# xaskasdf/ntransformer

Measured on AMD Instinct MI355X. Metric: decode tokens/sec (Llama-3.1-8B Q8_0 class, resident weights, greedy, batch 1), higher is better.
Workload: dtype f32; 1 GPU; Llama-3.1-8B-shaped Q8_0 GGUF tensors (seed 20260925), resident in HBM, 16-token prompt, greedy decode; ctx=4096, replicas=1, hipgraph=True

## Files before the change

include/ntk_engine.h:

```cpp
#ifndef NTK_ENGINE_H
#define NTK_ENGINE_H

#include "ntk.h"

#if defined(__GNUC__)
#pragma GCC visibility push(default)
#endif
#ifdef __cplusplus
extern "C" {
#endif

int ntk_rope_kv_store(float* q, const float* k, const float* v, const int* positions, int seq_len, int n_heads, int n_kv_heads, int head_dim,
                      float theta_base, float freq_scale, int interleaved, void* k_cache, void* v_cache, int start_pos, int max_seq, void* stream);
int ntk_rope_tab(float* q, float* k, const int* positions, int batch_size, int seq_len, int n_heads, int n_kv_heads, int head_dim, float theta_base,
                 float freq_scale, int interleaved, const float* inv_freq, void* stream);
int ntk_rope_kv_store_tab(float* q, const float* k, const float* v, const int* positions, int seq_len, int n_heads, int n_kv_heads, int head_dim,
                          float theta_base, float freq_scale, int interleaved, void* k_cache, void* v_cache, int start_pos, int max_seq,
                          const float* inv_freq, void* stream);
typedef struct ntk_gemv_seg {
    const void* W;
    float*      y;
    int         rows;
    int         dtype;
} ntk_gemv_seg;

int ntk_gemv_fused(const ntk_gemv_seg* segs, int nseg, const float* x, int in_features, const float* norm_w,
                   float eps, const float* resid, int silu_pair, void* stream);

size_t ntk_q8l_bytes(int rows, int in_features);
int ntk_q8l_pack(void* dst, const void* raw, int rows, int in_features, void* stream);
int ntk_q8l_unpack(void* raw, const void* packed, int rows, int in_features, void* stream);

size_t ntk_rp_bytes(int dtype, int rows, int in_features);
int ntk_rp_pack(void* dst, const void* raw, int rows, int in_features, int dtype, void* stream);
int ntk_rp_dequant(float* out, const void* rp, int rows, int in_features, int dtype, void* stream);
int ntk_rp_unpack(void* raw, const void* rp, int rows, int in_features, int dtype, void* stream);
int ntk_gemv_rp(float* y, const void* rp, const float* x, int out_features, int in_features, int weight_dtype, void* stream);
int ntk_gemv_rp_fused(const ntk_gemv_seg* segs, int nseg, const float* x, int in_features, const float* norm_w, float eps,
                      const float* resid, int silu_pair, void* stream);
#define NTK_ARENA_HIDDEN 1
#define NTK_ARENA_ATTN_OUT 2
#define NTK_ARENA_GATE 3
#define NTK_ARENA_HIDDEN_FLOATS 8192
#define NTK_ARENA_ATTN_FLOATS 8192
#define NTK_ARENA_GATE_FLOATS 32768
int ntk_decode_arena_acquire(void);
void ntk_decode_arena_release(int device);
float* ntk_decode_arena_slot(int slot);
int ntk_debug_gemv_static_x(void);

int ntk_debug_rp_prologue(uint8_t* out, const float* x, const float* norm_w, float eps, int in_features, int nsub, int nwaves, void* stream);
int ntk_debug_mfma_i8_probe(int* D, const int8_t* A, const int8_t* B, void* stream);

int ntk_attention_decode_fused(float* output, const float* q, const float* k, const float* v, void* k_cache,
                               void* v_cache, const int* d_pos, const float* inv_freq, int n_heads, int n_kv_heads,
                               int head_dim, int max_seq, float scale, float theta_base, float freq_scale,
                               void* stream);

size_t ntk_attention_split_scratch_bytes(int n_heads, int head_dim, int nsplit);
int ntk_attention_decode_split(float* output, const float* q, const float* k, const float* v, void* k_cache,
                               void* v_cache, const int* d_pos, const float* inv_freq, int n_heads, int n_kv_heads,
                               int head_dim, int max_seq, float scale, float theta_base, float freq_scale, int nsplit,
                               float* scratch, void* stream);
int ntk_attention_split_scratch_init(float* scratch, int n_heads, void* stream);
int ntk_attention_decode_split_merged(float* output, const float* q, const float* k, const float* v, void* k_cache,
                                      void* v_cache, const int* d_pos, const float* inv_freq, int n_heads, int n_kv_heads,
                                      int head_dim, int max_seq, float scale, float theta_base, float freq_scale, int nsplit,
                                      float* scratch, void* stream);

#define NTK_ATTN_BATCH_MAX 16
typedef struct ntk_kv_batch {
    void* k[NTK_ATTN_BATCH_MAX];
    void* v[NTK_ATTN_BATCH_MAX];
} ntk_kv_batch;
int ntk_attention_decode_batch(float* output, const float* q, const float* k, const float* v, const ntk_kv_batch* caches, const int* positions,
                               int n_rows, const float* inv_freq, int n_heads, int n_kv_heads, int head_dim, int max_seq, float scale,
                               float theta_base, float freq_scale, int nsplit, float* scratch, void* stream);

typedef struct ntk_kv_segments {
    int   n_seg;
    int   row0[NTK_ATTN_BATCH_MAX];
    int   n_rows[NTK_ATTN_BATCH_MAX];
    int   start_pos[NTK_ATTN_BATCH_MAX];
    void* k[NTK_ATTN_BATCH_MAX];
    void* v[NTK_ATTN_BATCH_MAX];
} ntk_kv_segments;
int ntk_kv_segments_validate(const ntk_kv_segments* segs, int total_rows, int max_seq);
int ntk_rope_kv_store_segments(float* q, const float* k, const float* v, const ntk_kv_segments* segs, int n_heads, int n_kv_heads, int head_dim,
                               float theta_base, float freq_scale, int interleaved, int max_seq, void* stream);
int ntk_rope_kv_store_segments_tab(float* q, const float* k, const float* v, const ntk_kv_segments* segs, int n_heads, int n_kv_heads, int head_dim,
                                   float theta_base, float freq_scale, int interleaved, int max_seq, const float* inv_freq, void* stream);
int ntk_attention_prefill_segments(float* output, const float* Q, const ntk_kv_segments* segs, int n_heads, int n_kv_heads, int head_dim, int max_seq,
                                   float scale, void* stream);

size_t ntk_kv_q8_cache_bytes(int max_seq, int n_kv_heads, int head_dim);
int ntk_kv_store_q8(void* k_cache, void* v_cache, const float* k, const float* v, int seq_len, int n_kv_heads, int head_dim, int start_pos,
                    int max_seq, void* stream);
int ntk_rope_kv_store_q8(float* q, const float* k, const float* v, const int* positions, int seq_len, int n_heads, int n_kv_heads, int head_dim,
                         float theta_base, float freq_scale, int interleaved, void* k_cache, void* v_cache, int start_pos, int max_seq,
                         void* stream);
int ntk_rope_kv_store_q8_tab(float* q, const float* k, const float* v, const int* positions, int seq_len, int n_heads, int n_kv_heads, int head_dim,
                             float theta_base, float freq_scale, int interleaved, void* k_cache, void* v_cache, int start_pos, int max_seq,
                             const float* inv_freq, void* stream);
int ntk_attention_decode_q8(float* output, const float* q, const float* k, const float* v, void* k_cache, void* v_cache, const int* d_pos,
                            const float* inv_freq, int n_heads, int n_kv_heads, int head_dim, int max_seq, float scale, float theta_base,
                            float freq_scale, int nsplit, float* scratch, void* stream);
int ntk_kv_dequant_q8_f16(void* k_f16, void* v_f16, const void* k_cache, const void* v_cache, int n_rows, int n_kv_heads, int head_dim,
                          int max_seq, void* stream);
int ntk_attention_decode_q8_batch(float* output, const float* q, const float* k, const float* v, const ntk_kv_batch* caches, const int* positions,
                                  int n_rows, const float* inv_freq, int n_heads, int n_kv_heads, int head_dim, int max_seq, float scale,
                                  float theta_base, float freq_scale, int nsplit, float* scratch, void* stream);

int ntk_kv_shift(uint16_t* k_cache, uint16_t* v_cache, int n_layers, int max_seq, int n_kv_heads, int head_dim, int src0, int dst0, int n_rows,
                 const float* inv_freq, float theta_base, float freq_scale, int interleaved, void* stream);
int ntk_kv_shift_q8(void* k_cache_q8, void* v_cache_q8, int n_layers, int max_seq, int n_kv_heads, int head_dim, int src0, int dst0, int n_rows,
                    const float* inv_freq, float theta_base, float freq_scale, int interleaved, void* stream);

int ntk_debug_gemv_fused_form(const ntk_gemv_seg* segs, int nseg, const float* x, int in_features, const float* norm_w, float eps,
                              const float* resid, int silu_pair, int integer_activations, void* stream);

size_t   ntk_tp_comm_bytes(size_t max_floats);
void*    ntk_tp_comm_alloc(size_t bytes);
int      ntk_tp_comm_reset(void* comm, void* stream);
float*   ntk_tp_slot(void* comm, size_t max_floats, unsigned call_index);
int      ntk_tp_allreduce_add(float* hidden, void* const* peers, int rank, int world, size_t max_floats, unsigned call_index, int n, void* stream);
int      ntk_tp_advance_epoch(void* comm, void* stream);
unsigned ntk_tp_error(void* comm);
int      ntk_ipc_export(void* devptr, void* handle64);
int      ntk_ipc_open(const void* handle64, void** devptr);
int      ntk_ipc_close(void* devptr);

int ntk_gemm_quant(float* Y, const void* W, const float* X, int n_tokens, int out_features, int in_features,
                   int weight_dtype, const float* resid, void* stream);

typedef struct ntk_gemm_partials {
    const float* part[3];
    float*       y[3];
    int          rows[3];
    int          nseg, n_tokens, nsplit;
} ntk_gemm_partials;
typedef struct ntk_gemm_desc {
    const ntk_gemv_seg* segs;
    int                 nseg;
    const float*        X;
    int                 n_tokens, in_features;
    const float*        resid;
    void*               workspace;
    size_t              workspace_bytes;
    int                 reuse_x;
    const float*        row_max;
    ntk_gemm_partials*  partials;
    int                 weights_repacked;
    int                 full_form;
} ntk_gemm_desc;
size_t ntk_gemm_quant_workspace_bytes(int in_features, int out_features);
int ntk_gemm_quant_f16(const ntk_gemm_desc* desc, void* stream);
int ntk_reduce_rmsnorm_rowmax(float* hidden, const ntk_gemm_partials* partials, const float* weight, float eps, float* x_out, float* row_max,
                              float* zero_tokens, void* stream);
int ntk_reduce_silu_mul_rowmax(float* output, const ntk_gemm_partials* partials, float* row_max, void* stream);
int ntk_rmsnorm_rowmax(float* output, const float* input, const float* weight, int n_tokens, int hidden_size, float eps, float* row_max,
                       float* zero_tokens, void* stream);
int ntk_silu_mul_rowmax(float* output, const float* gate, const float* up, int n_tokens, int width, float* row_max, void* stream);
int ntk_gemm_prepare_x(const float* X, int n_tokens, int in_features, void* workspace, void* stream);
int ntk_rmsnorm_prepare_x(float* output, const float* input, const float* weight, int n_tokens, int hidden_size, float eps, void* workspace, void* stream);
int ntk_reduce_rmsnorm_prepare_x(float* hidden, const ntk_gemm_partials* partials, const float* weight, float eps, float* x_out, void* workspace, void* stream);
int ntk_silu_mul_prepare_x(float* output, const float* gate, const float* up, int n_tokens, int width, void* workspace, void* stream);
int ntk_reduce_silu_mul_prepare_x(float* output, const ntk_gemm_partials* partials, void* workspace, void* stream);

size_t ntk_gemm_dense16_workspace_bytes(int in_features, int out_features, int dtype);
int ntk_gemm_dense16(const ntk_gemm_desc* desc, void* stream);

int ntk_embed_rows(float* out, const void* table, const int* tokens, int n_tokens, int hidden, int dtype,
                   void* stream);

int ntk_argmax(const float* logits, int n, int* d_out_token, int* h_mirror, float* scratch, void* stream);

int ntk_logprob_rows(const float* logits, int n_rows, int vocab, int ld, const int* targets, float* logprob, int* top1, void* stream);

size_t ntk_sample_scratch_bytes(int n);
int ntk_sample_top_k(float* logits, int n, const int* d_recent, int n_recent, float repeat_penalty, float temperature,
                     int top_k, float top_p, float r, int* d_out_token, int* h_mirror, void* scratch, void* stream);
int ntk_repeat_penalty(float* logits, int n, const int* d_recent, int n_recent, float repeat_penalty, void* stream);

#define NTK_SAMPLE_ROWS_MAX 16
typedef struct ntk_sample_rows {
    float temperature[NTK_SAMPLE_ROWS_MAX], top_p[NTK_SAMPLE_ROWS_MAX], repeat_penalty[NTK_SAMPLE_ROWS_MAX], r[NTK_SAMPLE_ROWS_MAX];
    int   top_k[NTK_SAMPLE_ROWS_MAX], n_recent[NTK_SAMPLE_ROWS_MAX];
} ntk_sample_rows;
size_t ntk_sample_rows_scratch_bytes(int n_rows, int vocab);
int ntk_sample_rows_top_k(float* logits, int n_rows, int vocab, int ld, const int* d_recent, int recent_ld, const ntk_sample_rows* rows, int* d_out,
                          int* h_mirror, void* scratch, void* stream);

int ntk_argmax_advance(const float* logits, int n, int* d_out_token, int* h_mirror, unsigned long long* h_ring4, int* d_pos,
                       float* scratch, void* stream);

int ntk_debug_sclk(unsigned long long* d_out2, void* stream);
int ntk_debug_sclk_begin(unsigned* d_flag, unsigned long long* d_out2, void* side_stream);
int ntk_debug_sclk_end(unsigned* d_flag, void* other_stream);

void ntk_debug_malloc_budget(long long bytes);

int ntk_advance_pos(int* d_pos, void* stream);

int ntk_qkv_bias(float* q, float* k, float* v, const float* bq, const float* bk, const float* bv, int n_rows, int q_dim, int kv_dim, void* stream);

int ntk_qk_norm(float* q, float* k, const float* wq, const float* wk, int n_rows, int n_heads, int n_kv_heads, int head_dim, float eps, void* stream);

#ifdef __cplusplus
}
#endif
#if defined(__GNUC__)
#pragma GCC visibility pop
#endif
#endif
```

ntransformer_amd/_lib.py:

```python
from __future__ import annotations

import ctypes as C
import os

_HERE = os.path.dirname(os.path.abspath(__file__))
LIB_PATH = os.environ.get("NTK_LIB_PATH") or os.path.join(_HERE, "libntransformer_hip.so")

NTK_OK = 0
_STATUS = {0: "ok", -1: "unsupported dtype", -2: "bad shape", -3: "HIP launch/runtime error", -4: "misaligned pointer",
           -5: "null pointer", -6: "no usable GPU", -7: "out of memory", -8: "I/O error", -9: "malformed GGUF"}


class NtkError(RuntimeError):
    def __init__(self, status: int, what: str = ""):
        self.status = status
        super().__init__("ntk status %d (%s)%s" % (status, _STATUS.get(status, "?"), (": " + what) if what else ""))


def check(status: int, what: str = "") -> None:
    if status != NTK_OK:
        raise NtkError(status, what)


class KvBatch(C.Structure):
    _fields_ = [("k", C.c_void_p * 16), ("v", C.c_void_p * 16)]


class KvSegments(C.Structure):
    _fields_ = [("n_seg", C.c_int), ("row0", C.c_int * 16), ("n_rows", C.c_int * 16), ("start_pos", C.c_int * 16), ("k", C.c_void_p * 16),
                ("v", C.c_void_p * 16)]


class SampleRows(C.Structure):
    _fields_ = [("temperature", C.c_float * 16), ("top_p", C.c_float * 16), ("repeat_penalty", C.c_float * 16), ("r", C.c_float * 16),
                ("top_k", C.c_int * 16), ("n_recent", C.c_int * 16)]


class GemvSeg(C.Structure):
    _fields_ = [("W", C.c_void_p), ("y", C.c_void_p), ("rows", C.c_int), ("dtype", C.c_int)]


class GemmPartials(C.Structure):
    _fields_ = [("part", C.c_void_p * 3), ("y", C.c_void_p * 3), ("rows", C.c_int * 3), ("nseg", C.c_int), ("n_tokens", C.c_int), ("nsplit", C.c_int)]


class GemmDesc(C.Structure):
    _fields_ = [("segs", C.POINTER(GemvSeg)), ("nseg", C.c_int), ("X", C.c_void_p), ("n_tokens", C.c_int), ("in_features", C.c_int), ("resid", C.c_void_p),
                ("workspace", C.c_void_p), ("workspace_bytes", C.c_size_t), ("reuse_x", C.c_int), ("row_max", C.c_void_p),
                ("partials", C.POINTER(GemmPartials)), ("weights_repacked", C.c_int), ("full_form", C.c_int)]


_lib = None


def lib() -> C.CDLL:
    global _lib
    if _lib is not None:
        return _lib
    if not os.path.exists(LIB_PATH):
        raise ImportError("%s is missing: run `python -c 'import __graft_entry__ as g; g.build()'` "
                          "(hipcc --offload-arch=gfx950); there is no CPU fallback" % LIB_PATH)
    L = C.CDLL(LIB_PATH, mode=C.RTLD_GLOBAL)
    vp, i, f, sz = C.c_void_p, C.c_int, C.c_float, C.c_size_t
    sig = {
        "ntk_abi_version": (i, []),
        "ntk_status_string": (C.c_char_p, [i]),
        "ntk_row_bytes": (sz, [i, C.c_int64]),
        "ntk_device_count": (i, []),
        "ntk_device_init": (i, [i]),
        "ntk_device_name": (i, [C.c_char_p, sz]),
        "ntk_device_mem_info": (i, [C.POINTER(sz), C.POINTER(sz)]),
        "ntk_stream": (vp, [i]),
        "ntk_stream_synchronize": (i, [vp]),
        "ntk_device_synchronize": (i, []),
        "ntk_event_create": (vp, []),
        "ntk_event_destroy": (i, [vp]),
        "ntk_event_record": (i, [vp, vp]),
        "ntk_event_synchronize": (i, [vp]),
        "ntk_event_elapsed_ms": (i, [vp, vp, C.POINTER(f)]),
        "nt_hip_malloc": (vp, [sz]), "nt_hip_free": (None, [vp]),
        "nt_hip_memcpy_h2d": (None, [vp, vp, sz]), "nt_hip_memcpy_d2h": (None, [vp, vp, sz]),
        "nt_hip_memcpy_d2d": (None, [vp, vp, sz]), "nt_hip_memset": (None, [vp, i, sz]),
        "nt_hip_malloc_host": (vp, [sz]), "nt_hip_free_host": (None, [vp]),
        "ntk_memcpy_h2d_async": (i, [vp, vp, sz, vp]), "ntk_memcpy_d2h_async": (i, [vp, vp, sz, vp]),
        "nt_cuda_malloc": (vp, [sz]), "nt_cuda_free": (None, [vp]),
        "nt_cuda_memcpy_h2d": (None, [vp, vp, sz]), "nt_cuda_memcpy_d2h": (None, [vp, vp, sz]),
        "nt_cuda_memcpy_d2d": (None, [vp, vp, sz]), "nt_cuda_memset": (None, [vp, i, sz]),
        "nt_cuda_malloc_host": (vp, [sz]), "nt_cuda_free_host": (None, [vp]),
        "ntk_rmsnorm": (i, [vp, vp, vp, i, i, f, vp]),
        "ntk_rmsnorm_f16": (i, [vp, vp, vp, i, i, f, vp]),
        "ntk_rope": (i, [vp, vp, vp, i, i, i, i, i, f, f, i, vp]),
        "ntk_softmax": (i, [vp, vp, i, i, vp]),
        "ntk_masked_softmax": (i, [vp, vp, vp, i, i, vp]),
        "ntk_gemv": (i, [vp, vp, vp, i, i, i, vp]),
        "ntk_gemv_add": (i, [vp, vp, vp, i, i, i, vp]),
        "ntk_gemm_f32": (i, [vp, vp, vp, i, i, i, vp]),
        "ntk_silu_mul": (i, [vp, vp, vp, i, vp]),
        "ntk_rmsnorm_rowmax": (i, [vp, vp, vp, i, i, f, vp, vp, vp]),
        "ntk_rope_kv_store": (i, [vp, vp, vp, vp, i, i, i, i, f, f, i, vp, vp, i, i, vp]),
        "ntk_silu_mul_rowmax": (i, [vp, vp, vp, i, i, vp, vp]),
        "ntk_add_bias": (i, [vp, vp, i, vp]),
        "ntk_attention_decode": (i, [vp, vp, vp, vp, i, i, i, i, i, f, vp]),
        "ntk_attention_prefill": (i, [vp, vp, vp, vp, i, i, i, i, i, i, f, vp]),
        "ntk_copy_to_kv_cache": (i, [vp, vp, vp, vp, i, i, i, i, i, vp]),
        "ntk_add": (i, [vp, vp, vp, i, vp]),
        "ntk_add_inplace": (i, [vp, vp, i, vp]),
        "ntk_copy": (i, [vp, vp, i, vp]),
        "ntk_cosine_similarity": (i, [vp, vp, vp, i, vp]),
        "ntk_gemv_fused": (i, [C.POINTER(GemvSeg), i, vp, i, vp, f, vp, i, vp]),
        "ntk_debug_gemv_fused_form": (i, [C.POINTER(GemvSeg), i, vp, i, vp, f, vp, i, i, vp]),
        "ntk_q8l_bytes": (sz, [i, i]),
        "ntk_q8l_pack": (i, [vp, vp, i, i, vp]),
        "ntk_q8l_unpack": (i, [vp, vp, i, i, vp]),
        "ntk_rp_bytes": (sz, [i, i, i]),
        "ntk_rp_pack": (i, [vp, vp, i, i, i, vp]),
        "ntk_rp_dequant": (i, [vp, vp, i, i, i, vp]),
        "ntk_rp_unpack": (i, [vp, vp, i, i, i, vp]),
        "ntk_gemv_rp": (i, [vp, vp, vp, i, i, i, vp]),
        "ntk_gemv_rp_fused": (i, [C.POINTER(GemvSeg), i, vp, i, vp, f, vp, i, vp]),
        "ntk_decode_arena_acquire": (i, []), "ntk_decode_arena_release": (None, [i]),
        "ntk_decode_arena_slot": (vp, [i]), "ntk_debug_gemv_static_x": (i, []),
        "ntk_debug_rp_prologue": (i, [vp, vp, vp, f, i, i, i, vp]),
        "ntk_debug_mfma_i8_probe": (i, [vp, vp, vp, vp]),
        "ntk_gemm_quant": (i, [vp, vp, vp, i, i, i, i, vp, vp]),
        "ntk_gemm_dense16_workspace_bytes": (sz, [i, i, i]),
        "ntk_gemm_dense16": (i, [C.POINTER(GemmDesc), vp]),
        "ntk_attention_decode_split": (i, [vp, vp, vp, vp, vp, vp, vp, vp, i, i, i, i, f, f, f, i, vp, vp]),
        "ntk_attention_split_scratch_bytes": (C.c_size_t, [i, i, i]),
        "ntk_attention_split_scratch_init": (i, [vp, i, vp]),
        "ntk_attention_decode_split_merged": (i, [vp, vp, vp, vp, vp, vp, vp, vp, i, i, i, i, f, f, f, i, vp, vp]),
        "ntk_attention_decode_fused": (i, [vp, vp, vp, vp, vp, vp, vp, vp, i, i, i, i, f, f, f, vp]),
        "ntk_attention_decode_batch": (i, [vp, vp, vp, vp, vp, vp, i, vp, i, i, i, i, f, f, f, i, vp, vp]),
        "ntk_kv_segments_validate": (i, [vp, i, i]),
        "ntk_rope_kv_store_segments": (i, [vp, vp, vp, vp, i, i, i, f, f, i, i, vp]),
        "ntk_attention_prefill_segments": (i, [vp, vp, vp, i, i, i, i, f, vp]),
        "ntk_rope_tab": (i, [vp, vp, vp, i, i, i, i, i, f, f, i, vp, vp]),
        "ntk_rope_kv_store_tab": (i, [vp, vp, vp, vp, i, i, i, i, f, f, i, vp, vp, i, i, vp, vp]),
        "ntk_rope_kv_store_segments_tab": (i, [vp, vp, vp, vp, i, i, i, f, f, i, i, vp, vp]),
        "ntk_rope_kv_store_q8_tab": (i, [vp, vp, vp, vp, i, i, i, i, f, f, i, vp, vp, i, i, vp, vp]),
        "ntk_kv_q8_cache_bytes": (C.c_size_t, [i, i, i]),
        "ntk_kv_store_q8": (i, [vp, vp, vp, vp, i, i, i, i, i, vp]),
        "ntk_rope_kv_store_q8": (i, [vp, vp, vp, vp, i, i, i, i, f, f, i, vp, vp, i, i, vp]),
        "ntk_attention_decode_q8": (i, [vp, vp, vp, vp, vp, vp, vp, vp, i, i, i, i, f, f, f, i, vp, vp]),
        "ntk_kv_dequant_q8_f16": (i, [vp, vp, vp, vp, i, i, i, i, vp]),
        "ntk_attention_decode_q8_batch": (i, [vp, vp, vp, vp, vp, vp, i, vp, i, i, i, i, f, f, f, i, vp, vp]),
        "ntk_kv_shift": (i, [vp, vp, i, i, i, i, i, i, i, vp, f, f, i, vp]),
        "ntk_kv_shift_q8": (i, [vp, vp, i, i, i, i, i, i, i, vp, f, f, i, vp]),
        "ntk_embed_rows": (i, [vp, vp, vp, i, i, i, vp]),
        "ntk_argmax": (i, [vp, i, vp, vp, vp, vp]),
        "ntk_logprob_rows": (i, [vp, i, i, i, vp, vp, vp, vp]),
        "ntk_sample_rows_scratch_bytes": (C.c_size_t, [i, i]),
        "ntk_sample_rows_top_k": (i, [vp, i, i, i, vp, i, C.POINTER(SampleRows), vp, vp, vp, vp]),
        "ntk_advance_pos": (i, [vp, vp]),
        "ntk_qkv_bias": (i, [vp, vp, vp, vp, vp, vp, i, i, i, vp]),
        "ntk_qk_norm": (i, [vp, vp, vp, vp, i, i, i, i, f, vp]),
        "ntk_debug_sclk": (i, [vp, vp]),
        "ntk_debug_sclk_begin": (i, [vp, vp, vp]),
        "ntk_debug_sclk_end": (i, [vp, vp]),
    }
    for name, (res, args) in sig.items():
        fn = getattr(L, name)
        fn.restype = res
        fn.argtypes = args
    _lib = L
    return L


EXPORTS_NTK_H = None
```

ntransformer_amd/csrc/common.hip.h:

```cpp
#pragma once
#include <hip/hip_runtime.h>
#include <stdint.h>
#include "../../include/ntk_engine.h"

#define NTK_WAVE 64

#define NTK_HIP_TRY(expr)                                   \
    do {                                                    \
        hipError_t e__ = (expr);                            \
        if (e__ != hipSuccess) return NTK_E_LAUNCH;         \
    } while (0)

#define NTK_EXTRA_API extern "C" __attribute__((visibility("default")))
#ifdef NTK_TUNE
#include <cstdlib>
#define NTK_TUNE_ENV_INT(name, dflt) ([] { const char* e__ = getenv(name); return e__ ? atoi(e__) : (dflt); }())
#else
#define NTK_TUNE_ENV_INT(name, dflt) (dflt)
#endif

namespace ntk {

hipStream_t resolve_stream(void* s);
int         last_launch_status();
int         q8l_gemv_fused(const ntk_gemv_seg* segs, int nseg, const float* x, int in, const float* norm_w, float eps, const float* resid,
                           int silu_pair, hipStream_t st);
int         dense16_gemv_fused(const ntk_gemv_seg* segs, int nseg, const float* x, int in, const float* norm_w, float eps, const float* resid,
                               int silu_pair, hipStream_t st);

__device__ __forceinline__ float h2f(uint16_t bits) {
    _Float16 h;
    __builtin_memcpy(&h, &bits, 2);
    return (float)h;
}
__device__ __forceinline__ uint16_t f2h(float f) {
    _Float16 h = (_Float16)f;
    uint16_t bits;
    __builtin_memcpy(&bits, &h, 2);
    return bits;
}

__device__ __forceinline__ void rope_rotate(const float a, const float b, const float c, const float s, float& ra, float& rb) {
#pragma clang fp contract(off)
    ra = a * c - b * s;
    rb = b * c + a * s;
}

__device__ __forceinline__ float rope_freq(const float* __restrict__ inv_freq, const int i, const int head_dim, const float theta) {
    return inv_freq ? inv_freq[i] : 1.0f / (float)pow((double)theta, (double)((2.0f * i) / head_dim));
}

template <int CTRL, int ROW_MASK>
__device__ __forceinline__ float dpp_or_zero(float v) {
    return __int_as_float(__builtin_amdgcn_update_dpp(0, __float_as_int(v), CTRL, ROW_MASK, 0xF, false));
}
template <int CTRL, int ROW_MASK>
__device__ __forceinline__ float dpp_or_self(float v) {
    return __int_as_float(__builtin_amdgcn_update_dpp(__float_as_int(v), __float_as_int(v), CTRL, ROW_MASK, 0xF, false));
}
constexpr int DPP_QUAD_1032 = 0xB1, DPP_QUAD_2301 = 0x4E, DPP_ROW_HALF_MIRROR = 0x141, DPP_ROW_MIRROR = 0x140,
              DPP_ROW_BCAST15 = 0x142, DPP_ROW_BCAST31 = 0x143;

__device__ __forceinline__ float wave_sum_lane63(float v) {
    v += dpp_or_zero<DPP_QUAD_1032, 0xF>(v);
    v += dpp_or_zero<DPP_QUAD_2301, 0xF>(v);
    v += dpp_or_zero<DPP_ROW_HALF_MIRROR, 0xF>(v);
    v += dpp_or_zero<DPP_ROW_MIRROR, 0xF>(v);
    v += dpp_or_zero<DPP_ROW_BCAST15, 0xA>(v);
    v += dpp_or_zero<DPP_ROW_BCAST31, 0xC>(v);
    return v;
}
__device__ __forceinline__ float wave_sum(float v) {
    return __int_as_float(__builtin_amdgcn_readlane(__float_as_int(wave_sum_lane63(v)), 63));
}
__device__ __forceinline__ float wave_max(float v) {
    v = fmaxf(v, dpp_or_self<DPP_QUAD_1032, 0xF>(v));
    v = fmaxf(v, dpp_or_self<DPP_QUAD_2301, 0xF>(v));
    v = fmaxf(v, dpp_or_self<DPP_ROW_HALF_MIRROR, 0xF>(v));
    v = fmaxf(v, dpp_or_self<DPP_ROW_MIRROR, 0xF>(v));
    v = fmaxf(v, dpp_or_self<DPP_ROW_BCAST15, 0xA>(v));
    v = fmaxf(v, dpp_or_self<DPP_ROW_BCAST31, 0xC>(v));
    return __int_as_float(__builtin_amdgcn_readlane(__float_as_int(v), 63));
}

template <int N>
__device__ __forceinline__ float group_sum(float v) {
    static_assert(N == 1 || N == 2 || N == 4 || N == 8 || N == 16 || N == 32, "group size");
    if constexpr (N >= 2) v += dpp_or_zero<DPP_QUAD_1032, 0xF>(v);
    if constexpr (N >= 4) v += dpp_or_zero<DPP_QUAD_2301, 0xF>(v);
    if constexpr (N >= 8) v += dpp_or_zero<DPP_ROW_HALF_MIRROR, 0xF>(v);
    if constexpr (N >= 16) v += dpp_or_zero<DPP_ROW_MIRROR, 0xF>(v);
    if constexpr (N >= 32) v += __shfl_xor(v, 16, 64);
    return v;
}

__device__ __forceinline__ float block_sum(float v, float* red) {
    const int lane = threadIdx.x & 63, wave = threadIdx.x >> 6, nw = (blockDim.x + 63) >> 6;
    v = wave_sum(v);
    __syncthreads();
    if (lane == 0) red[wave] = v;
    __syncthreads();
    float t = 0.0f;
    for (int i = 0; i < nw; ++i) t += red[i];
    return t;
}
__device__ __forceinline__ float block_max(float v, float* red) {
    const int lane = threadIdx.x & 63, wave = threadIdx.x >> 6, nw = (blockDim.x + 63) >> 6;
    v = wave_max(v);
    __syncthreads();
    if (lane == 0) red[wave] = v;
    __syncthreads();
    float t = red[0];
    for (int i = 1; i < nw; ++i) t = fmaxf(t, red[i]);
    return t;
}

template <int N>
__device__ __forceinline__ void lds_read_dwords(uint32_t (&dst)[N], const uint8_t* base, int off) {
    const int a = off & ~3;
    const uint32_t sh = (uint32_t)(off & 3);
    uint32_t w[N + 1];
#pragma unroll
    for (int i = 0; i <= N; ++i) w[i] = *reinterpret_cast<const uint32_t*>(base + a + 4 * i);
#pragma unroll
    for (int i = 0; i < N; ++i) dst[i] = __builtin_amdgcn_alignbyte(w[i + 1], w[i], sh);
}
__device__ __forceinline__ uint16_t lds_u16_at(const uint8_t* base, int off) {
    return *reinterpret_cast<const uint16_t*>(base + off);
}

__device__ __forceinline__ float ub2f(uint32_t w, int k) { return (float)((w >> (8 * k)) & 0xFFu); }
__device__ __forceinline__ float sb2f(uint32_t w, int k) { return (float)(int)(int8_t)(w >> (8 * k)); }

__device__ __forceinline__ void kq_scale_min(uint32_t s0, uint32_t s1, uint32_t s2, int j, float& sc, float& mn) {
    const uint64_t lo = (uint64_t)s0 | ((uint64_t)s1 << 32);
    auto byte = [&](int n) -> uint32_t {
        return n < 8 ? (uint32_t)((lo >> (8 * n)) & 0xFFu) : ((s2 >> (8 * (n - 8))) & 0xFFu);
    };
    uint32_t s, m;
    if (j < 4) {
        s = byte(j) & 63u;
        m = byte(j + 4) & 63u;
    } else {
        s = (byte(j + 4) & 0xFu) | ((byte(j - 4) >> 6) << 4);
        m = (byte(j + 4) >> 4) | ((byte(j) >> 6) << 4);
    }
    sc = (float)s;
    mn = (float)m;
}

}
```

ntransformer_amd/csrc/gemv.hip:

```cpp
#include "gemv_core.hip.h"
#include <algorithm>
#include <atomic>
#include <cmath>
#include <cstddef>
#include <mutex>
#include <cstdio>
#include <cstdlib>

namespace ntk {

enum { NS_ANY = 0, NS_ONE = 1, NS_SPLIT = 2 };

enum { XS_NONE = 0, XS_HIDDEN = NTK_ARENA_HIDDEN, XS_ATTN = NTK_ARENA_ATTN_OUT, XS_GATE = NTK_ARENA_GATE };
struct DecodeArena {
    float hidden[NTK_ARENA_HIDDEN_FLOATS];
    float attn_out[NTK_ARENA_ATTN_FLOATS];
    float gate[NTK_ARENA_GATE_FLOATS];
};
__device__ __attribute__((aligned(256))) DecodeArena g_decode_arena;
template <int XS> struct XSlot { static constexpr int IN = XS == XS_GATE ? 14336 : 4096; };
template <int XS> __device__ __forceinline__ const float* xslot_ptr() {
    return XS == XS_HIDDEN ? g_decode_arena.hidden : XS == XS_ATTN ? g_decode_arena.attn_out : g_decode_arena.gate;
}

template <int DT, bool NORM, bool XFAST, bool A16, bool XI = false, bool LM = false, int NSF = NS_ANY, int XS = XS_NONE>
__device__ __forceinline__ void gemv_quant_body(const GemvParams& p, const int bid, const int nblk) {
    using F = Fmt<DT>;
    static_assert(!LM || (DT == NTK_DT_Q8_0 && !A16 && !XI), "lane-major rows: Q8_0");
    static_assert(NSF == NS_ANY || LM, "compile-time slice forms: the lane-major kernels");
    static_assert(XS == XS_NONE || (LM && XFAST && NSF != NS_ANY), "early-x forms: the lane-major kernels, fast prologue");
    constexpr int NL = LM ? 4 : F::NL;
    constexpr int STAGE = LM ? 0 : NL * 1024 + 64;
    extern __shared__ __attribute__((aligned(16))) uint8_t smem[];
#ifdef NTK_GEMV_TRACE
    unsigned long long gv_t[GT_EV] = {0, 0, 0, 0, 0, 0, 0, 0, 0, 0, 0, 0, 0, 0};
#endif
    GV_STAMP(0);
#ifndef NTK_GEMV_NO_KARG_PREFETCH
    const auto* ka = __builtin_amdgcn_kernarg_segment_ptr();
    unsigned d0, d1, d2, d3, d4;
    if constexpr (XS == XS_NONE) {
        asm volatile("s_load_dword %0, %5, 0x0\n\ts_load_dword %1, %5, 0x40\n\ts_load_dword %2, %5, 0x80\n\ts_load_dword %3, %5, 0xc0\n\t"
                     "s_load_dword %4, %5, 0x100\n\ts_waitcnt lgkmcnt(0)"
                     : "=&s"(d0), "=&s"(d1), "=&s"(d2), "=&s"(d3), "=&s"(d4) : "s"(ka) : "memory");
    } else {
        asm volatile("s_load_dword %0, %5, 0x0\n\ts_load_dword %1, %5, 0x40\n\ts_load_dword %2, %5, 0x80\n\ts_load_dword %3, %5, 0xc0\n\t"
                     "s_load_dword %4, %5, 0x100"
                     : "=&s"(d0), "=&s"(d1), "=&s"(d2), "=&s"(d3), "=&s"(d4) : "s"(ka) : "memory");
    }
    __builtin_amdgcn_sched_barrier(0);
#endif

    const int tid = threadIdx.x;
    constexpr int XIT = 8, WIT = 4;
    u32x4 xv[XIT], wv[WIT];
    if constexpr (XS != XS_NONE) {
        constexpr int IN = XSlot<XS>::IN, step0 = 512 * 4;
        const float* const xs = xslot_ptr<XS>();
#pragma unroll
        for (int i = 0; i < XIT; ++i) {
            xv[i] = u32x4{0u, 0u, 0u, 0u};
            if (i * step0 < IN) xv[i] = *reinterpret_cast<const u32x4*>(xs + min(tid * 4 + i * step0, IN - 4));
        }
        GV_STAMP(7);
        __builtin_amdgcn_sched_barrier(0);
#ifndef NTK_GEMV_NO_KARG_PREFETCH
        asm volatile("s_waitcnt lgkmcnt(0)" : "+s"(d0), "+s"(d1), "+s"(d2), "+s"(d3), "+s"(d4) : : "memory");
        __builtin_amdgcn_sched_barrier(0);
#endif
        if constexpr (NORM) {
#pragma unroll
            for (int i = 0; i < WIT; ++i) {
                wv[i] = u32x4{0u, 0u, 0u, 0u};
                if (i * step0 < IN) wv[i] = *reinterpret_cast<const u32x4*>(p.norm_w + min(tid * 4 + i * step0, IN - 4));
            }
        }
    } else
    if constexpr (XFAST) {
        const int step0 = (int)blockDim.x * 4;
#pragma unroll
        for (int i = 0; i < XIT; ++i) {
            xv[i] = u32x4{0u, 0u, 0u, 0u};
            if (i * step0 < p.in) xv[i] = *reinterpret_cast<const u32x4*>(p.x + min(tid * 4 + i * step0, p.in - 4));
        }
        if constexpr (NORM) {
#pragma unroll
            for (int i = 0; i < WIT; ++i) {
                wv[i] = u32x4{0u, 0u, 0u, 0u};
                if (i * step0 < p.in) wv[i] = *reinterpret_cast<const u32x4*>(p.norm_w + min(tid * 4 + i * step0, p.in - 4));
            }
        }
        GV_STAMP(7);
    }
    const int lane = tid & 63;
    const int wave = __builtin_amdgcn_readfirstlane(tid >> 6);
    const int ns = NSF == NS_ONE ? 1 : p.ns;
    const bool single = NSF == NS_ANY ? p.ns == 1 : NSF == NS_ONE;
    const int nwaves = ns * p.rw;
    const int s = wave % ns;
    const int g = wave / ns;
    constexpr bool norm = NORM;

    const size_t image_bytes = (size_t)std::min(ns, 4) * 64 * XPITCH * 4;
    const size_t stage0 = single ? image_bytes : 0;
    const size_t regionA = single ? image_bytes + (size_t)nwaves * STAGE : std::max((size_t)nwaves * STAGE, image_bytes);
    float* part = reinterpret_cast<float*>(smem + regionA);
    float* red = part + 2 * p.rw * ns * RB;
    const size_t lds_floats_total = regionA / 4 + (size_t)(2 * p.rw * ns * RB + 16 + 16);

    uint8_t* stage = smem + stage0 + (size_t)wave * STAGE;
    const int my_len = min(p.slice_cols, p.in - s * p.slice_cols);
    const int ncols = min(64, max(0, my_len - 64 * lane));
    const unsigned slice_byte0 = (unsigned)((size_t)s * p.slice_cols / F::BW * F::BB);
    const unsigned slice_bytes = (unsigned)(my_len / F::BW * F::BB);
    const int group = bid * p.rw + g;
    const int ngroups = nblk * p.rw;
    const int mats = p.silu_pair ? 2 : 1;
    const int n_my = (p.total_rows > group) ? ((p.total_rows - 1 - group) / ngroups + 1) * mats : 0;

    static_assert(MAX_SEG == 3, "locate / seg_y: unrolled for three segments");
    const int seg_rows0 = p.seg[0].rows, seg_rows1 = p.seg[1].rows;
    float* const seg_y0 = p.seg[0].y;
    float* const seg_y1 = p.seg[1].y;
    float* const seg_y2 = p.seg[2].y;
    auto locate = [&](int q, int& seg, int& row) {
        int r = group + (q >> (mats - 1)) * ngroups;
        if (p.silu_pair) { seg = q & 1; row = r; return; }
        seg = 0;
        if (p.nseg > 1 && r >= seg_rows0) {
            r -= seg_rows0; seg = 1;
            if (p.nseg > 2 && r >= seg_rows1) { r -= seg_rows1; seg = 2; }
        }
        row = r;
    };
    auto seg_y = [&](int seg) { return seg == 0 ? seg_y0 : seg == 1 ? seg_y1 : seg_y2; };
    int cu_seg = 0, cu_row = group, cu_rows = p.silu_pair ? 0x7fffffff : p.seg[0].rows;
    auto cursor_normalise = [&]() {
        while (cu_seg + 1 < p.nseg && cu_row >= cu_rows) { cu_row -= cu_rows; ++cu_seg; cu_rows = p.seg[cu_seg].rows; }
    };
    if (!p.silu_pair) cursor_normalise();
    auto cursor_advance = [&]() {
        if (p.silu_pair) {
            if (cu_seg == 0) { cu_seg = 1; } else { cu_seg = 0; cu_row += ngroups; }
        } else {
            cu_row += ngroups;
            cursor_normalise();
        }
    };

    u32x4 pf[NL], pf2[LM ? NL : 1];
    uint32_t pf_sc = 0u, pf2_sc = 0u;
    const int lm_nl = my_len >> 6, lm_lane = min(lane, max(lm_nl - 1, 0));
    unsigned pre_off[NL];
    if constexpr (A16) {
        const unsigned last0 = (slice_bytes - 1u) & ~15u;
#pragma unroll
        for (int j = 0; j < NL; ++j) pre_off[j] = min(16u * (unsigned)(lane + 64 * j), last0);
    }
    int pf_seg = 0, pf_row = 0, pf_shift = 0;
    float pf_res = 0.0f;
    auto issue = [&]() {
        pf_seg = cu_seg; pf_row = cu_row;
        if (p.resid != nullptr && single) {
            int idx = cu_row;
            asm volatile("" : "+v"(idx));
            pf_res = p.resid[idx];
        }
        if constexpr (LM) return;
        const unsigned rel = (unsigned)p.seg[cu_seg].delta + (unsigned)cu_row * p.row_bytes + slice_byte0;
        pf_shift = (int)(rel & 15u);
        const unsigned nbytes = (rel & 15u) + slice_bytes;
        const unsigned last = (nbytes - 1u) & ~15u;
        const uint8_t* a = p.seg[cu_seg].W + (rel & ~15u);
#pragma unroll
        for (int j = 0; j < NL; ++j) {
            unsigned off;
            if constexpr (A16) off = pre_off[j]; else off = min(16u * (unsigned)(lane + 64 * j), last);
            pf[j] = __builtin_nontemporal_load(reinterpret_cast<const u32x4*>(a + off));
        }
    };
    auto issue_lm = [&](u32x4 (&c)[NL], uint32_t& sc) {
        const uint8_t* a = p.seg[cu_seg].W + ((unsigned)cu_row * p.row_bytes + slice_byte0);
#pragma unroll
        for (int j = 0; j < NL; ++j)
            c[j] = __builtin_nontemporal_load(reinterpret_cast<const u32x4*>(a + 16u * (unsigned)(j * lm_nl + lm_lane)));
        sc = __builtin_nontemporal_load(reinterpret_cast<const uint32_t*>(a + 64u * (unsigned)lm_nl + 4u * (unsigned)lm_lane));
    };
    auto issue_first = [&]() { issue(); if constexpr (LM) issue_lm(pf, pf_sc); };
    if (n_my <= 0) { cu_seg = 0; cu_row = 0; }

    f32x2 x2[32];
    XInt xi;
    static_assert(!XI || (XFAST && ((DT == NTK_DT_Q4_K && A16) || DT == NTK_DT_Q6_K)), "integer activations: fast prologue, Q4_K (aligned rows) / Q6_K");
    {
        float* ximg = reinterpret_cast<float*>(smem);
        constexpr int GS = 4;
        auto img_index = [&](int c, int g0) {
            if (single) return (c >> 6) * XPITCH + (c & 63);
            const int sp = c / p.slice_cols, cc = c - sp * p.slice_cols;
            return ((sp - g0) * 64 + (cc >> 6)) * XPITCH + (cc & 63);
        };
        const int step = (int)blockDim.x * 4;
        const int dummy = (int)(lds_floats_total - 16);
        const bool have_lo = ncols > 0, have_hi = ncols > 32;
        auto read_own_row = [&](int g0) {
            const float* xrow = ximg + ((s - g0) * 64 + lane) * XPITCH;
            const float* xr0 = xrow, *xr1 = xrow + 32;
            if constexpr (DT == NTK_DT_Q6_K) {
                xr0 = ximg + ((s - g0) * 64 + (lane & ~1)) * XPITCH + 32 * (lane & 1);
                xr1 = xr0 + XPITCH;
            }
#pragma unroll
            for (int j = 0; j < 64; j += 4) {
                const float4 v = *reinterpret_cast<const float4*>((j < 32 ? xr0 : xr1 - 32) + j);
                const bool have = j < 32 ? have_lo : have_hi;
                x2[j / 2] = f32x2{have ? v.x : 0.0f, have ? v.y : 0.0f};
                x2[j / 2 + 1] = f32x2{have ? v.z : 0.0f, have ? v.w : 0.0f};
            }
        };
        if constexpr (XFAST) {
#ifndef NTK_GEMV_NO_XWAIT
            asm volatile("" : "+v"(xv[0]), "+v"(xv[1]), "+v"(xv[2]), "+v"(xv[3]), "+v"(xv[4]), "+v"(xv[5]), "+v"(xv[6]), "+v"(xv[7]));
            if constexpr (NORM) asm volatile("" : "+v"(wv[0]), "+v"(wv[1]), "+v"(wv[2]), "+v"(wv[3]));
#endif
            issue_first();
            GV_STAMP(8);
            __builtin_amdgcn_sched_barrier(0);
            GV_STAMP(1);
            float rms_inv = 1.0f;
            if constexpr (NORM) {
                float ssq = 0.0f;
#pragma unroll
                for (int i = 0; i < WIT; ++i) {
                    const float m = (tid * 4 + i * step < p.in) ? 1.0f : 0.0f;
                    const float x0 = __uint_as_float(xv[i].x), x1 = __uint_as_float(xv[i].y), x2_ = __uint_as_float(xv[i].z), x3 = __uint_as_float(xv[i].w);
                    ssq = fmaf(x0 * m, x0, ssq); ssq = fmaf(x1 * m, x1, ssq); ssq = fmaf(x2_ * m, x2_, ssq); ssq = fmaf(x3 * m, x3, ssq);
                }
                ssq = wave_sum(ssq);
                if (lane == 0) red[wave] = ssq;
                __syncthreads();
                float tot = 0.0f;
                for (int w = 0; w < nwaves; ++w) tot += red[w];
                rms_inv = 1.0f / sqrtf(tot / (float)p.in + p.eps);
#pragma unroll
                for (int i = 0; i < WIT; ++i) {
                    xv[i].x = __float_as_uint(__uint_as_float(xv[i].x) * rms_inv * __uint_as_float(wv[i].x));
                    xv[i].y = __float_as_uint(__uint_as_float(xv[i].y) * rms_inv * __uint_as_float(wv[i].y));
                    xv[i].z = __float_as_uint(__uint_as_float(xv[i].z) * rms_inv * __uint_as_float(wv[i].z));
                    xv[i].w = __float_as_uint(__uint_as_float(xv[i].w) * rms_inv * __uint_as_float(wv[i].w));
                }
            }
            if constexpr (XI) {
                uint8_t* dimg = smem;
                auto xi_store = [&](const u32x4 q, const int sp, const int cc, const bool live) {
                    const float v0 = live ? __uint_as_float(q.x) : 0.0f, v1 = live ? __uint_as_float(q.y) : 0.0f,
                                v2 = live ? __uint_as_float(q.z) : 0.0f, v3 = live ? __uint_as_float(q.w) : 0.0f;
                    float am = fmaxf(fmaxf(fabsf(v0), fabsf(v1)), fmaxf(fabsf(v2), fabsf(v3)));
                    am = fmaxf(am, dpp_or_self<DPP_QUAD_1032, 0xF>(am));
                    am = fmaxf(am, dpp_or_self<DPP_QUAD_2301, 0xF>(am));
                    am = fmaxf(am, dpp_or_self<DPP_ROW_HALF_MIRROR, 0xF>(am));
                    float sm = (v0 + v1) + (v2 + v3);
                    sm += dpp_or_zero<DPP_QUAD_1032, 0xF>(sm);
                    sm += dpp_or_zero<DPP_QUAD_2301, 0xF>(sm);
                    const int e = am > 0.0f ? __builtin_amdgcn_frexp_expf(am) : 0;
                    const float up = __builtin_ldexpf(1.0f, 22 - e), inv = __builtin_ldexpf(1.0f, e - 22);
                    const uint32_t x0 = __float_as_uint(fmaf(v0, up, 12582912.0f)) - 0x4B400000u, x1 = __float_as_uint(fmaf(v1, up, 12582912.0f)) - 0x4B400000u,
                                   x2i = __float_as_uint(fmaf(v2, up, 12582912.0f)) - 0x4B400000u, x3 = __float_as_uint(fmaf(v3, up, 12582912.0f)) - 0x4B400000u;
                    const uint32_t ta = __builtin_amdgcn_perm(x1, x0, 0x05010400u);
                    const uint32_t tb = __builtin_amdgcn_perm(x1, x0, 0x07030602u);
                    const uint32_t tc = __builtin_amdgcn_perm(x3, x2i, 0x05010400u);
                    const uint32_t td = __builtin_amdgcn_perm(x3, x2i, 0x07030602u);
                    const uint32_t p0 = __builtin_amdgcn_perm(tc, ta, 0x05040100u);
                    const uint32_t p1 = __builtin_amdgcn_perm(tc, ta, 0x07060302u);
                    const uint32_t p2 = __builtin_amdgcn_perm(td, tb, 0x05040100u);
                    if (live) {
                        uint8_t* row = dimg + (size_t)(sp * 64 + (cc >> 6)) * (XPITCH * 4);
                        *reinterpret_cast<uint32_t*>(row + (cc & 63)) = p0;
                        *reinterpret_cast<uint32_t*>(row + 64 + (cc & 63)) = p1;
                        *reinterpret_cast<uint32_t*>(row + 128 + (cc & 63)) = p2;
                        float* meta = reinterpret_cast<float*>(row + 192);
                        if ((cc & 31) == 0) meta[(cc >> 5) & 1] = inv;
                        if ((cc & 15) == 0) meta[2 + ((cc >> 4) & 3)] = sm;
                    }
                };
                auto xi_read = [&](const int g0) {
                    const bool have_lo_ = ncols > 0, have_hi_ = ncols > 32;
                    const uint8_t* rowA = dimg + (size_t)((s - g0) * 64 + lane) * (XPITCH * 4);
                    const uint8_t* rowB = rowA;
                    int offA = 0, offB = 32;
                    if constexpr (DT == NTK_DT_Q6_K) {
                        rowA = dimg + (size_t)((s - g0) * 64 + (lane & ~1)) * (XPITCH * 4);
                        rowB = rowA + XPITCH * 4;
                        offA = offB = 32 * (lane & 1);
                    }
#pragma unroll
                    for (int pl = 0; pl < 3; ++pl)
#pragma unroll
                        for (int k4 = 0; k4 < 4; ++k4) {
                            const uint8_t* src = (k4 < 2 ? rowA + offA : rowB + offB) + 64 * pl + 16 * (k4 & 1);
                            const u32x4 v = *reinterpret_cast<const u32x4*>(src);
                            const bool have = k4 < 2 ? have_lo_ : have_hi_;
                            xi.d[pl][4 * k4] = have ? v.x : 0u; xi.d[pl][4 * k4 + 1] = have ? v.y : 0u;
                            xi.d[pl][4 * k4 + 2] = have ? v.z : 0u; xi.d[pl][4 * k4 + 3] = have ? v.w : 0u;
                        }
                    const float* mA = reinterpret_cast<const float*>(rowA + 192);
                    const float* mB = reinterpret_cast<const float*>(rowB + 192);
                    xi.inv[0] = have_lo_ ? mA[offA >> 5] : 0.0f;
                    xi.inv[1] = have_hi_ ? mB[offB >> 5] : 0.0f;
                    xi.sx[0] = have_lo_ ? mA[2 + (offA >> 4)] : 0.0f; xi.sx[1] = have_lo_ ? mA[3 + (offA >> 4)] : 0.0f;
                    xi.sx[2] = have_hi_ ? mB[2 + (offB >> 4)] : 0.0f; xi.sx[3] = have_hi_ ? mB[3 + (offB >> 4)] : 0.0f;
                };
                int isp = 0, icc = tid * 4;
#pragma unroll
                for (int i = 0; i < XIT; ++i) {
                    if (i * step >= p.in) continue;
                    xi_store(xv[i], isp, icc, tid * 4 + i * step < p.in);
                    icc += step;
                    if (icc >= p.slice_cols) { icc -= p.slice_cols; ++isp; }
                }
                __syncthreads();
                xi_read(0);
            } else
            {
                const int cend = min(p.in, GS * p.slice_cols);
                int isp = 0, icc = tid * 4;
#pragma unroll
                for (int i = 0; i < XIT; ++i) {
                    if (i * step >= cend) continue;
                    const int c = tid * 4 + i * step;
                    *reinterpret_cast<u32x4*>(ximg + (c < cend ? (isp * 64 + (icc >> 6)) * XPITCH + (icc & 63) : dummy)) = xv[i];
                    icc += step;
                    if (icc >= p.slice_cols) { icc -= p.slice_cols; ++isp; }
                }
                for (int c = XIT * step + tid * 4; c < cend; c += step)
                    *reinterpret_cast<float4*>(ximg + img_index(c, 0)) = *reinterpret_cast<const float4*>(p.x + c);
                GV_STAMP(9);
                __syncthreads();
                GV_STAMP(10);
                if (s < GS) read_own_row(0);
#ifdef NTK_GEMV_TRACE
                asm volatile("s_waitcnt lgkmcnt(0)" ::: "memory");
                GV_STAMP(11);
#endif
            }
            if constexpr (!XI)
            for (int g0 = GS; g0 < ns; g0 += GS) {
                const int cbeg = g0 * p.slice_cols, cend = min(p.in, (g0 + GS) * p.slice_cols);
                __syncthreads();
                for (int c = cbeg + tid * 4; c < cend; c += step)
                    *reinterpret_cast<float4*>(ximg + img_index(c, g0)) = *reinterpret_cast<const float4*>(p.x + c);
                __syncthreads();
                if (s >= g0 && s < g0 + GS) read_own_row(g0);
            }
        } else {
            issue_first();
            float rms_inv = 1.0f;
            if (NORM && !(kAblate & 1)) {
                float ssq = 0.0f;
                for (int c = tid; c < p.in; c += blockDim.x) ssq = fmaf(p.x[c], p.x[c], ssq);
                ssq = wave_sum(ssq);
                if (lane == 0) red[wave] = ssq;
                __syncthreads();
                float tot = 0.0f;
                for (int w = 0; w < nwaves; ++w) tot += red[w];
                rms_inv = 1.0f / sqrtf(tot / (float)p.in + p.eps);
            }
            for (int g0 = 0; g0 < ns; g0 += GS) {
                const int cbeg = g0 * p.slice_cols, cend = min(p.in, (g0 + GS) * p.slice_cols);
                if (g0 > 0) __syncthreads();
                if (!(kAblate & 1)) {
                    for (int c = cbeg + tid; c < cend; c += blockDim.x)
                        ximg[img_index(c, g0)] = NORM ? p.x[c] * rms_inv * p.norm_w[c] : p.x[c];
                }
                __syncthreads();
                if (s >= g0 && s < g0 + GS) read_own_row(g0);
            }
        }
        if ((kAblate & 1) || XI) {
#pragma unroll
            for (int j = 0; j < 32; ++j) x2[j] = f32x2{1.0f, 1.0f};
        }
        if (!single && !LM) __syncthreads();
        GV_STAMP(2);
    }
    float sx16[4], sx32[2];
#pragma unroll
    for (int r = 0; r < 4; ++r) {
        float t = 0.0f;
#pragma unroll
        for (int j = 0; j < 8; ++j) t += x2[8 * r + j].x + x2[8 * r + j].y;
        sx16[r] = t;
    }
    sx32[0] = sx16[0] + sx16[1];
    sx32[1] = sx16[2] + sx16[3];
    if constexpr (DT == NTK_DT_Q4_K) {
#pragma unroll
        for (int j = 16; j < 32; ++j) x2[j] *= 0.0625f;
    }
    if constexpr (DT == NTK_DT_Q4_0) {
#pragma unroll
        for (int j = 0; j < 32; ++j) if ((j & 8) != 0) x2[j] *= 0.0625f;
    }
    float gate_carry = 0.0f;
    float pair_g = 0.0f, pair_u = 0.0f;
    auto silu_flush = [&](const int last_pair) {
        const int base = last_pair & ~63;
        if (lane <= last_pair - base) {
            const int row = group + (base + lane) * ngroups;
            p.seg[0].y[row] = pair_g / (1.0f + expf(-pair_g)) * pair_u;
        }
    };

    float res_pf = 0.0f;
    auto prefetch_resid = [&](int b) {
        if (p.resid == nullptr || s != 0 || lane >= RB || b * RB + lane >= n_my) return;
        int seg, row;
        locate(b * RB + lane, seg, row);
        res_pf = p.resid[row];
    };
    if (!single) prefetch_resid(0);
    auto combine = [&](int b, int cnt) {
        if (s != 0) return;
        const float* pg = part + (size_t)(b & 1) * p.rw * ns * RB + (size_t)(g * ns) * RB;
        float t = 0.0f;
        if (lane < cnt)
            for (int ss = 0; ss < ns; ++ss) t += pg[ss * RB + lane];
        const float nxt = __shfl_down(t, 1, 64);
        if (lane < cnt) {
            int seg, row;
            locate(b * RB + lane, seg, row);
            if (p.silu_pair) {
                if ((lane & 1) == 0) seg_y0[row] = t / (1.0f + expf(-t)) * nxt;
            } else {
                float v = t;
                if (p.resid != nullptr && seg == 0) v = res_pf + v;
                seg_y(seg)[row] = v;
            }
        }
        prefetch_resid(b + 1);
    };

    auto row_step = [&](const int q, u32x4 (&cur)[NL], uint32_t& cur_sc, u32x4 (&nxt)[LM ? NL : 1], uint32_t& nxt_sc) __attribute__((always_inline)) {
        const int seg = pf_seg, row = pf_row, shift = A16 ? 0 : pf_shift;
        const float res = pf_res;
        float acc;
        if constexpr (LM) {
            asm volatile("" : "+v"(cur[0]), "+v"(cur[1]), "+v"(cur[2]), "+v"(cur[3]), "+v"(cur_sc));
#ifdef NTK_GEMV_TRACE
            if (q == 0) GV_STAMP(3);
            if (q == n_my - 1) GV_STAMP(5);
#endif
            if (q + 1 < n_my) { cursor_advance(); issue(); issue_lm(nxt, nxt_sc); }
            __builtin_amdgcn_sched_barrier(0);
            acc = dot_q8_regs(cur, cur_sc, ncols, x2);
        } else {
#pragma unroll
            for (int j = 0; j < NL; ++j) {
                if (kAblate & 4) { asm volatile("" ::"v"(pf[j])); continue; }
                *reinterpret_cast<u32x4*>(stage + 16 * (lane + 64 * j)) = pf[j];
            }
            __builtin_amdgcn_wave_barrier();
#ifdef NTK_GEMV_TRACE
            if (q == 0) GV_STAMP(3);
            if (q == n_my - 1) GV_STAMP(5);
#endif
            if (q + 1 < n_my) { cursor_advance(); issue(); }
            if constexpr (XI && DT == NTK_DT_Q6_K) acc = DotI<DT>::run(stage, shift, lane, ncols, xi);
            else if constexpr (XI) acc = DotI<DT>::run(stage, lane, ncols, xi);
            else acc = (kAblate & 2) ? x2[0].x + (float)q : Dot<DT, A16>::run(stage, shift, lane, ncols, x2, sx16, sx32);
            __builtin_amdgcn_wave_barrier();
        }
        const float tot = wave_sum_lane63(acc);
#ifdef NTK_GEMV_TRACE
        if (q == 0) { asm volatile("" :: "v"(tot)); GV_STAMP(4); }
#endif

        if (single) {
            if (p.silu_pair) {
                const float t63 = __int_as_float(__builtin_amdgcn_readlane(__float_as_int(tot), 63));
                const int pi = (q >> 1) & 63;
                if ((q & 1) == 0) { if (lane == pi) pair_g = t63; }
                else {
                    if (lane == pi) pair_u = t63;
                    if (pi == 63 || q == n_my - 1) silu_flush(q >> 1);
                }
            } else if (lane == 63) {
                float v = tot;
                if (p.resid != nullptr && seg == 0) v = res + v;
                p.seg[seg].y[row] = v;
            }
        } else {
            const int b = q / RB, i = q % RB;
            if (lane == 63) part[(size_t)(b & 1) * p.rw * ns * RB + (size_t)(g * ns + s) * RB + i] = tot;
            if (i == RB - 1) {
                __syncthreads();
                combine(b, RB);
            }
        }
    };
    for (int q = 0; q < n_my; ++q) {
        row_step(q, pf, pf_sc, pf2, pf2_sc);
        if constexpr (LM) { if (++q < n_my) row_step(q, pf2, pf2_sc, pf, pf_sc); }
    }
    if (!single) {
        int done = n_my / RB;
        if (n_my % RB) {
            __syncthreads();
            combine(done, n_my % RB);
            ++done;
        }
        for (; done < p.nbatch; ++done) __syncthreads();
    }
#ifdef NTK_GEMV_TRACE
    GV_STAMP(6);
    if (tid == 0 && bid < GT_WG) {
        gv_t[13] = (unsigned long long)n_my;
        for (int e = 0; e < GT_EV; ++e) g_gemv_trace[p.trace_slot & (GT_SLOTS - 1)][bid][e] = gv_t[e];
    }
#endif
}

template <bool NORM, bool XFAST, int NSF, int XS = XS_NONE>
__global__ __launch_bounds__(512, Fmt<NTK_DT_Q8_0>::MINW) void gemv_q8l_kernel(const GemvParams p) {
    gemv_quant_body<NTK_DT_Q8_0, NORM, XFAST, false, false, true, NSF, XS>(p, (int)blockIdx.x, (int)gridDim.x);
}
template <bool UNPACK>
__global__ __launch_bounds__(256) void q8l_pack_kernel(uint8_t* __restrict__ dst, const uint8_t* __restrict__ src, const int rows, const int in,
                                                       const int slice_cols) {
    const int lanes_row = in >> 6;
    const size_t t = (size_t)blockIdx.x * blockDim.x + threadIdx.x;
    if (t >= (size_t)rows * lanes_row) return;
    const int row = (int)(t / lanes_row), gl = (int)(t % lanes_row);
    const int lanes_slice = slice_cols >> 6, sl = gl / lanes_slice, l = gl - sl * lanes_slice;
    const int nl = min(lanes_slice, lanes_row - sl * lanes_slice);
    const size_t row0 = (size_t)row * lanes_row * 68;
    uint32_t* file = reinterpret_cast<uint32_t*>(const_cast<uint8_t*>(UNPACK ? dst : src) + row0 + (size_t)gl * 68);
    uint8_t* slice = const_cast<uint8_t*>(UNPACK ? src : dst) + row0 + (size_t)sl * lanes_slice * 68;
    uint32_t w[17], q[16], sc;
    if constexpr (!UNPACK) {
#pragma unroll
        for (int k = 0; k < 17; ++k) w[k] = file[k];
#pragma unroll
        for (int k = 0; k < 8; ++k) { q[k] = (w[k] >> 16) | (w[k + 1] << 16); q[8 + k] = w[9 + k]; }
        sc = (w[0] & 0xFFFFu) | (w[8] & 0xFFFF0000u);
#pragma unroll
        for (int j = 0; j < 4; ++j) *reinterpret_cast<u32x4*>(slice + (size_t)(j * nl + l) * 16) = u32x4{q[4 * j], q[4 * j + 1], q[4 * j + 2], q[4 * j + 3]};
        *reinterpret_cast<uint32_t*>(slice + (size_t)64 * nl + 4 * l) = sc;
    } else {
#pragma unroll
        for (int j = 0; j < 4; ++j) {
            const u32x4 v = *reinterpret_cast<const u32x4*>(slice + (size_t)(j * nl + l) * 16);
            q[4 * j] = v.x; q[4 * j + 1] = v.y; q[4 * j + 2] = v.z; q[4 * j + 3] = v.w;
        }
        sc = *reinterpret_cast<const uint32_t*>(slice + (size_t)64 * nl + 4 * l);
        w[0] = (sc & 0xFFFFu) | (q[0] << 16);
#pragma unroll
        for (int k = 1; k < 8; ++k) w[k] = (q[k - 1] >> 16) | (q[k] << 16);
        w[8] = (q[7] >> 16) | (sc & 0xFFFF0000u);
#pragma unroll
        for (int k = 0; k < 8; ++k) w[9 + k] = q[8 + k];
#pragma unroll
        for (int k = 0; k < 17; ++k) file[k] = w[k];
    }
}

template <int DT, bool NORM, bool XFAST, bool A16>
__global__ __launch_bounds__(512, Fmt<DT>::MINW) void gemv_quant_kernel(const GemvParams p) {
    gemv_quant_body<DT, NORM, XFAST, A16>(p, (int)blockIdx.x, (int)gridDim.x);
}
template <int DT, bool NORM>
__global__ __launch_bounds__(512, Fmt<DT>::MINW) void gemv_quant_xi_kernel(const GemvParams p) {
    gemv_quant_body<DT, NORM, true, A16_OK<DT>, true>(p, (int)blockIdx.x, (int)gridDim.x);
}
template <int DTA, int DTB, bool NORM>
__global__ __launch_bounds__(512, 4) void gemv_quant_pair_kernel(const GemvParams pa, const GemvParams pb, const int split) {
    if ((int)blockIdx.x < split) gemv_quant_body<DTA, NORM, true, A16_OK<DTA>>(pa, (int)blockIdx.x, split);
    else gemv_quant_body<DTB, NORM, true, A16_OK<DTB>>(pb, (int)blockIdx.x - split, (int)gridDim.x - split);
}

template <bool BF> __device__ __forceinline__ float w16f(uint16_t bits) {
    if constexpr (BF) return __uint_as_float((uint32_t)bits << 16); else return h2f(bits);
}
template <typename T, bool ADD, bool BF = false>
__global__ __launch_bounds__(256) void gemv_dense_kernel(float* __restrict__ y, const T* __restrict__ W,
                                                         const float* __restrict__ x, int out, int in) {
    const int lane = threadIdx.x & 63;
    const int wave = blockIdx.x * (blockDim.x >> 6) + (threadIdx.x >> 6);
    const int nwaves = gridDim.x * (blockDim.x >> 6);
    constexpr int V = 16 / (int)sizeof(T);
    for (int r = wave; r < out; r += nwaves) {
        const T* w = W + (size_t)r * in;
        float acc = 0.0f;
        int done = 0;
        if ((reinterpret_cast<uintptr_t>(w) & 15) == 0 && (reinterpret_cast<uintptr_t>(x) & 15) == 0) {
            const int nv = in / V;
            for (int i = lane; i < nv; i += 64) {
                const u32x4 raw = __builtin_nontemporal_load(reinterpret_cast<const u32x4*>(w) + i);
                if constexpr (sizeof(T) == 4) {
                    const float4 xv = *reinterpret_cast<const float4*>(x + 4 * i);
                    acc = fmaf(__uint_as_float(raw.x), xv.x, acc); acc = fmaf(__uint_as_float(raw.y), xv.y, acc);
                    acc = fmaf(__uint_as_float(raw.z), xv.z, acc); acc = fmaf(__uint_as_float(raw.w), xv.w, acc);
                } else {
                    const float4 x0 = *reinterpret_cast<const float4*>(x + 8 * i);
                    const float4 x1 = *reinterpret_cast<const float4*>(x + 8 * i + 4);
                    acc = fmaf(w16f<BF>((uint16_t)(raw.x & 0xFFFF)), x0.x, acc); acc = fmaf(w16f<BF>((uint16_t)(raw.x >> 16)), x0.y, acc);
                    acc = fmaf(w16f<BF>((uint16_t)(raw.y & 0xFFFF)), x0.z, acc); acc = fmaf(w16f<BF>((uint16_t)(raw.y >> 16)), x0.w, acc);
                    acc = fmaf(w16f<BF>((uint16_t)(raw.z & 0xFFFF)), x1.x, acc); acc = fmaf(w16f<BF>((uint16_t)(raw.z >> 16)), x1.y, acc);
                    acc = fmaf(w16f<BF>((uint16_t)(raw.w & 0xFFFF)), x1.z, acc); acc = fmaf(w16f<BF>((uint16_t)(raw.w >> 16)), x1.w, acc);
                }
            }
            done = nv * V;
        }
        for (int i = done + lane; i < in; i += 64) {
            float wv;
            if constexpr (sizeof(T) == 4) wv = (float)w[i]; else wv = w16f<BF>((uint16_t)w[i]);
            acc = fmaf(wv, x[i], acc);
        }
        acc = wave_sum(acc);
        if (lane == 0) y[r] = ADD ? y[r] + acc : acc;
    }
}

static bool is_quant(int dt) {
    return dt == NTK_DT_Q8_0 || dt == NTK_DT_Q4_0 || dt == NTK_DT_Q4_K || dt == NTK_DT_Q5_K || dt == NTK_DT_Q6_K;
}

struct GemvLaunch {
    GemvParams p;
    int grid, nwaves;
    size_t lds;
    bool xfast, a16;
};

static bool raise_lds_limit(const void* fn) {
    return hipFuncSetAttribute(fn, hipFuncAttributeMaxDynamicSharedMemorySize, 160 * 1024) == hipSuccess;
}

template <int DT>
static int prepare_quant(const ntk_gemv_seg* segs, int nseg, const float* x, int in, const float* norm_w, float eps,
                         const float* resid, int silu_pair, int max_wg, GemvLaunch& L, bool lm = false) {
    using F = Fmt<DT>;
    if (in <= 0 || in % F::BW != 0) return NTK_E_SHAPE;
    GemvParams& p = L.p;
    p = GemvParams{};
    long total = 0;
    const size_t row_bytes = (size_t)in / F::BW * F::BB;
    for (int i = 0; i < nseg; ++i) {
        if (segs[i].rows < 0) return NTK_E_SHAPE;
        if (segs[i].rows > 0 && (!segs[i].W || !segs[i].y)) return NTK_E_NULL;
        if ((size_t)segs[i].rows * row_bytes > 0xFFFFFFF0ull) return NTK_E_SHAPE;
        const uintptr_t w = reinterpret_cast<uintptr_t>(segs[i].W);
        if (w & 1) return NTK_E_ALIGN;
        p.seg[i].W = reinterpret_cast<const uint8_t*>(w & ~(uintptr_t)15);
        p.seg[i].delta = (int)(w & 15);
        p.seg[i].y = segs[i].y;
        p.seg[i].rows = segs[i].rows;
        total += segs[i].rows;
    }
    if (silu_pair) {
        if (nseg != 2 || segs[0].rows != segs[1].rows || resid) return NTK_E_SHAPE;
        total = segs[0].rows;
    }
    p.nseg = nseg;
    p.total_rows = (int)total;
    p.x = x;
    p.in = in;
    if (!gemv_slices(in, F::BW == 256 ? 256 : 64, p.ns, p.slice_cols)) return NTK_E_SHAPE;
    static const int env_waves = std::max(1, NTK_TUNE_ENV_INT("NTK_GEMV_WAVES", 8));
    p.rw = std::max(1, env_waves / p.ns);
    L.nwaves = p.ns * p.rw;
    p.x_vec = ((reinterpret_cast<uintptr_t>(x) & 15) == 0 &&
               (!norm_w || (reinterpret_cast<uintptr_t>(norm_w) & 15) == 0) && (p.slice_cols % 4 == 0)) ? 1 : 0;
    p.norm_w = norm_w;
    p.eps = eps;
    p.resid = resid;
    p.silu_pair = silu_pair;
    p.row_bytes = (unsigned)row_bytes;
    const int mats = silu_pair ? 2 : 1;
    int grid = (int)std::min<long>((total + p.rw - 1) / p.rw, max_wg);
    grid = std::max(grid, 1);
    L.grid = grid;
    const long ngroups = (long)grid * p.rw;
    const long rows_per_group = (total + ngroups - 1) / ngroups;
    p.nbatch = (int)((rows_per_group * mats + RB - 1) / RB);
    const int STAGE = lm ? 0 : F::NL * 1024 + 64;
    const size_t image_bytes = (size_t)std::min(p.ns, 4) * 64 * XPITCH * 4;
    const size_t regionA = p.ns == 1 ? image_bytes + (size_t)L.nwaves * STAGE : std::max((size_t)L.nwaves * STAGE, image_bytes);
    L.lds = regionA + (size_t)(2 * p.rw * p.ns * RB + 16 + 16) * sizeof(float);
    L.xfast = p.x_vec && (in % 4 == 0) && in >= 4 && !(kAblate & 1) && (!norm_w || in <= 4 * 4 * 64 * L.nwaves) &&
              (p.ns == 1 || 4 * 64 * L.nwaves <= p.slice_cols);
    bool a16 = (DT == NTK_DT_Q4_K || DT == NTK_DT_Q5_K);
    for (int i = 0; i < nseg; ++i) a16 = a16 && p.seg[i].delta == 0;
    L.a16 = a16;
    return NTK_OK;
}

constexpr size_t kXiMinBytes = (size_t)48 << 20;
enum { XI_DEFAULT = -1, XI_NEVER = 0, XI_ALWAYS = 1 };

static int max_workgroups() {
    static const int max_wg = std::max(1, NTK_TUNE_ENV_INT("NTK_GEMV_MAX_WG", 512));
    return max_wg;
}

template <int DT>
static int launch_quant(const ntk_gemv_seg* segs, int nseg, const float* x, int in, const float* norm_w, float eps,
                        const float* resid, int silu_pair, hipStream_t st, int xi_mode = XI_DEFAULT) {
    GemvLaunch L;
    const int rc = prepare_quant<DT>(segs, nseg, x, in, norm_w, eps, resid, silu_pair, max_workgroups(), L);
    if (rc != NTK_OK) return rc;
    if (L.p.total_rows == 0) return NTK_OK;
    using KernelFn = void (*)(const GemvParams);
    static const KernelFn table[2][2][2] = {
        {{gemv_quant_kernel<DT, false, false, false>, gemv_quant_kernel<DT, false, false, A16_OK<DT>>},
         {gemv_quant_kernel<DT, false, true, false>, gemv_quant_kernel<DT, false, true, A16_OK<DT>>}},
        {{gemv_quant_kernel<DT, true, false, false>, gemv_quant_kernel<DT, true, false, A16_OK<DT>>},
         {gemv_quant_kernel<DT, true, true, false>, gemv_quant_kernel<DT, true, true, A16_OK<DT>>}}};
    if (L.lds > 64 * 1024) {
        static bool once = [] {
            bool ok = true;
            for (int a = 0; a < 2; ++a)
                for (int b = 0; b < 2; ++b)
                    for (int c = 0; c < 2; ++c)
                        ok = ok && hipFuncSetAttribute((const void*)table[a][b][c], hipFuncAttributeMaxDynamicSharedMemorySize,
                                                       160 * 1024) == hipSuccess;
            return ok;
        }();
        if (!once || L.lds > 160 * 1024) return NTK_E_SHAPE;
    }
    const dim3 g(L.grid), b(64 * L.nwaves);
#ifdef NTK_GEMV_TRACE
    static int trace_counter = 0;
    L.p.trace_slot = trace_counter++;
#endif
    if constexpr (DT == NTK_DT_Q4_K || DT == NTK_DT_Q6_K) {
        const size_t launch_bytes = (size_t)L.p.total_rows * (silu_pair ? 2 : 1) * L.p.row_bytes;
        const bool want = xi_mode == XI_ALWAYS || (xi_mode == XI_DEFAULT && launch_bytes >= kXiMinBytes);
        if (want && L.xfast && (L.a16 || DT == NTK_DT_Q6_K) && L.p.ns <= 2 && in <= 8 * 4 * 64 * L.nwaves) {
            using XFn = void (*)(const GemvParams);
            static const XFn xt[2] = {gemv_quant_xi_kernel<DT, false>, gemv_quant_xi_kernel<DT, true>};
            if (L.lds > 64 * 1024) {
                static bool once2 = hipFuncSetAttribute((const void*)xt[0], hipFuncAttributeMaxDynamicSharedMemorySize, 160 * 1024) == hipSuccess &&
                                    hipFuncSetAttribute((const void*)xt[1], hipFuncAttributeMaxDynamicSharedMemorySize, 160 * 1024) == hipSuccess;
                if (!once2) return NTK_E_SHAPE;
            }
            hipLaunchKernelGGL(xt[norm_w ? 1 : 0], g, b, L.lds, st, L.p);
            return last_launch_status();
        }
    }
    hipLaunchKernelGGL(table[norm_w ? 1 : 0][L.xfast ? 1 : 0][L.a16 ? 1 : 0], g, b, L.lds, st, L.p);
    return last_launch_status();
}

static size_t q8l_bytes(int rows, int in) {
    int ns, sc;
    return rows > 0 && q8l_layout(in, ns, sc) ? (size_t)rows * (size_t)(in / 32 * 34) : 0;
}

static int q8l_pack(void* dst, const void* raw, int rows, int in, bool unpack, hipStream_t st) {
    int ns, sc;
    if (rows <= 0 || !q8l_layout(in, ns, sc)) return NTK_E_SHAPE;
    if ((reinterpret_cast<uintptr_t>(unpack ? raw : dst) & 15) || (reinterpret_cast<uintptr_t>(unpack ? dst : raw) & 3)) return NTK_E_ALIGN;
    const size_t n = (size_t)rows * (in / 64);
    if ((n + 255) / 256 > 0x7FFFFFFFull) return NTK_E_SHAPE;
    const dim3 g((unsigned)((n + 255) / 256)), b(256);
    uint8_t* d = static_cast<uint8_t*>(dst);
    const uint8_t* r = static_cast<const uint8_t*>(raw);
    if (unpack) hipLaunchKernelGGL(q8l_pack_kernel<true>, g, b, 0, st, d, r, rows, in, sc);
    else hipLaunchKernelGGL(q8l_pack_kernel<false>, g, b, 0, st, d, r, rows, in, sc);
    return last_launch_status();
}

constexpr int kArenaDevices = 16;
struct ArenaDev {
    std::atomic<int> known{0};
    std::atomic<int> owned{0};
    const float* addr[4] = {nullptr, nullptr, nullptr, nullptr};
};
static ArenaDev g_arena_dev[kArenaDevices];
static std::mutex g_arena_mu;
static thread_local int t_last_static_x = XS_NONE;

static ArenaDev* arena_dev(bool lookup) {
    int dev = -1;
    if (hipGetDevice(&dev) != hipSuccess || dev < 0 || dev >= kArenaDevices) return nullptr;
    ArenaDev& a = g_arena_dev[dev];
    if (a.known.load(std::memory_order_acquire) == 0 && lookup) {
        std::lock_guard<std::mutex> lk(g_arena_mu);
        if (a.known.load(std::memory_order_relaxed) == 0) {
            void* base = nullptr;
            const bool ok = hipGetSymbolAddress(&base, HIP_SYMBOL(g_decode_arena)) == hipSuccess && base != nullptr;
            if (ok) {
                auto* f = static_cast<const float*>(base);
                a.addr[XS_HIDDEN] = f + offsetof(DecodeArena, hidden) / 4;
                a.addr[XS_ATTN] = f + offsetof(DecodeArena, attn_out) / 4;
                a.addr[XS_GATE] = f + offsetof(DecodeArena, gate) / 4;
            }
            a.known.store(ok ? 1 : -1, std::memory_order_release);
        }
    }
    return a.known.load(std::memory_order_acquire) == 1 ? &a : nullptr;
}
static int static_x_slot(const float* x, int in) {
    const ArenaDev* a = arena_dev(false);
    if (!a) return XS_NONE;
    if (x == a->addr[XS_HIDDEN] && in == XSlot<XS_HIDDEN>::IN) return XS_HIDDEN;
    if (x == a->addr[XS_ATTN] && in == XSlot<XS_ATTN>::IN) return XS_ATTN;
    if (x == a->addr[XS_GATE] && in == XSlot<XS_GATE>::IN) return XS_GATE;
    return XS_NONE;
}

int q8l_gemv_fused(const ntk_gemv_seg* segs, int nseg, const float* x, int in, const float* norm_w, float eps, const float* resid,
                   int silu_pair, hipStream_t st) {
    int ns, sc;
    t_last_static_x = XS_NONE;
    if (!q8l_layout(in, ns, sc)) return NTK_E_SHAPE;
    for (int i = 0; i < nseg; ++i)
        if (reinterpret_cast<uintptr_t>(segs[i].W) & 15) return NTK_E_ALIGN;
    GemvLaunch L;
    const int rc = prepare_quant<NTK_DT_Q8_0>(segs, nseg, x, in, norm_w, eps, resid, silu_pair, max_workgroups(), L, true);
    if (rc != NTK_OK) return rc;
    if (L.p.total_rows == 0) return NTK_OK;
    using KernelFn = void (*)(const GemvParams);
#define Q8L_FORMS(NORM, XFAST) {gemv_q8l_kernel<NORM, XFAST, NS_ONE>, gemv_q8l_kernel<NORM, XFAST, NS_SPLIT>}
    static const KernelFn table[2][2][2] = {{Q8L_FORMS(false, false), Q8L_FORMS(false, true)}, {Q8L_FORMS(true, false), Q8L_FORMS(true, true)}};
#undef Q8L_FORMS
    if (L.lds > 64 * 1024) {
        static const bool once = [] {
            bool ok = true;
            for (int a = 0; a < 2; ++a)
                for (int b = 0; b < 2; ++b)
                    for (int c = 0; c < 2; ++c) ok = ok && raise_lds_limit((const void*)table[a][b][c]);
            return ok;
        }();
        if (!once || L.lds > 160 * 1024) return NTK_E_SHAPE;
    }
#ifdef NTK_GEMV_TRACE
    static int trace_counter = 0;
    L.p.trace_slot = trace_counter++;
#endif
    KernelFn fn = table[norm_w ? 1 : 0][L.xfast ? 1 : 0][L.p.ns == 1 ? 0 : 1];
    if (L.xfast && L.nwaves == 8) {
        const int xs = static_x_slot(x, in);
        KernelFn early = nullptr;
        if (xs == XS_HIDDEN && L.p.ns == 1 && norm_w) early = gemv_q8l_kernel<true, true, NS_ONE, XS_HIDDEN>;
        else if (xs == XS_ATTN && L.p.ns == 1 && !norm_w) early = gemv_q8l_kernel<false, true, NS_ONE, XS_ATTN>;
        else if (xs == XS_GATE && L.p.ns > 1 && !norm_w) {
            static const bool raised = raise_lds_limit((const void*)gemv_q8l_kernel<false, true, NS_SPLIT, XS_GATE>);
            if (raised || L.lds <= 64 * 1024) early = gemv_q8l_kernel<false, true, NS_SPLIT, XS_GATE>;
        }
        if (early && L.lds <= 160 * 1024) { fn = early; t_last_static_x = xs; }
    }
    hipLaunchKernelGGL(fn, dim3(L.grid), dim3(64 * L.nwaves), L.lds, st, L.p);
    return last_launch_status();
}


template <int DTA, int DTB>
static int launch_pair(const ntk_gemv_seg* sa, int na, const ntk_gemv_seg* sb, int nb, const float* x, int in, const float* norm_w,
                       float eps, hipStream_t st) {
    const double ba = (double)Fmt<DTA>::BB / Fmt<DTA>::BW, bb = (double)Fmt<DTB>::BB / Fmt<DTB>::BW;
    long ra = 0, rb = 0;
    for (int i = 0; i < na; ++i) ra += sa[i].rows;
    for (int i = 0; i < nb; ++i) rb += sb[i].rows;
    if (ra <= 0 || rb <= 0) return NTK_E_SHAPE;
    const int total_wg = max_workgroups();
    int wa = (int)(total_wg * (ra * ba) / (ra * ba + rb * bb) + 0.5);
    wa = std::min(std::max(wa, 1), total_wg - 1);
    GemvLaunch A, B;
    int rc = prepare_quant<DTA>(sa, na, x, in, norm_w, eps, nullptr, 0, wa, A);
    if (rc == NTK_OK) rc = prepare_quant<DTB>(sb, nb, x, in, norm_w, eps, nullptr, 0, total_wg - wa, B);
    if (rc != NTK_OK) return rc;
    if (!A.xfast || !B.xfast || A.nwaves != B.nwaves || A.a16 != A16_OK<DTA> || B.a16 != A16_OK<DTB>) return NTK_E_ALIGN;
    for (int i = 0; i < na; ++i) if (A.p.seg[i].delta != 0 && A16_OK<DTA>) return NTK_E_ALIGN;
    using PairFn = void (*)(const GemvParams, const GemvParams, int);
    const size_t lds = std::max(A.lds, B.lds);
    static const PairFn table[2] = {gemv_quant_pair_kernel<DTA, DTB, false>, gemv_quant_pair_kernel<DTA, DTB, true>};
    if (lds > 64 * 1024) {
        static bool once = hipFuncSetAttribute((const void*)table[0], hipFuncAttributeMaxDynamicSharedMemorySize, 160 * 1024) == hipSuccess &&
                           hipFuncSetAttribute((const void*)table[1], hipFuncAttributeMaxDynamicSharedMemorySize, 160 * 1024) == hipSuccess;
        if (!once || lds > 160 * 1024) return NTK_E_SHAPE;
    }
    hipLaunchKernelGGL(table[norm_w ? 1 : 0], dim3(A.grid + B.grid), dim3(64 * A.nwaves), lds, st, A.p, B.p, A.grid);
    return last_launch_status();
}

static int dispatch_quant(int dt, const ntk_gemv_seg* segs, int nseg, const float* x, int in, const float* norm_w,
                          float eps, const float* resid, int silu_pair, hipStream_t st, int xi_mode = XI_DEFAULT) {
    switch (dt) {
        case NTK_DT_Q8_0: return launch_quant<NTK_DT_Q8_0>(segs, nseg, x, in, norm_w, eps, resid, silu_pair, st);
        case NTK_DT_Q4_0: return launch_quant<NTK_DT_Q4_0>(segs, nseg, x, in, norm_w, eps, resid, silu_pair, st);
        case NTK_DT_Q4_K: return launch_quant<NTK_DT_Q4_K>(segs, nseg, x, in, norm_w, eps, resid, silu_pair, st, xi_mode);
        case NTK_DT_Q5_K: return launch_quant<NTK_DT_Q5_K>(segs, nseg, x, in, norm_w, eps, resid, silu_pair, st);
        case NTK_DT_Q6_K: return launch_quant<NTK_DT_Q6_K>(segs, nseg, x, in, norm_w, eps, resid, silu_pair, st, xi_mode);
        default: return NTK_E_DTYPE;
    }
}

template <bool ADD>
static int launch_dense(float* y, const void* W, const float* x, int out, int in, int dt, hipStream_t st) {
    if (out == 0) return NTK_OK;
    const int grid = std::min((out + 3) / 4, 2048);
    if (dt == NTK_DT_F32)
        hipLaunchKernelGGL((gemv_dense_kernel<float, ADD>), dim3(grid), dim3(256), 0, st, y, (const float*)W, x, out, in);
    else if (dt == NTK_DT_BF16)
        hipLaunchKernelGGL((gemv_dense_kernel<uint16_t, ADD, true>), dim3(grid), dim3(256), 0, st, y, (const uint16_t*)W, x, out, in);
    else
        hipLaunchKernelGGL((gemv_dense_kernel<uint16_t, ADD>), dim3(grid), dim3(256), 0, st, y, (const uint16_t*)W, x, out, in);
    return last_launch_status();
}

}

extern "C" {

#ifdef NTK_GEMV_TRACE
NTK_EXTRA_API int ntk_debug_gemv_trace(unsigned long long* out, size_t n) {
    return hipMemcpyFromSymbol(out, HIP_SYMBOL(ntk::g_gemv_trace), n * sizeof(unsigned long long)) == hipSuccess ? 0 : -3;
}
#endif

int ntk_decode_arena_acquire(void) {
    ntk::ArenaDev* a = ntk::arena_dev(true);
    int free_ = 0;
    return a && a->owned.compare_exchange_strong(free_, 1) ? (int)(a - ntk::g_arena_dev) : -1;
}
void ntk_decode_arena_release(int device) {
    if (device >= 0 && device < ntk::kArenaDevices) ntk::g_arena_dev[device].owned.store(0);
}
float* ntk_decode_arena_slot(int slot) {
    const ntk::ArenaDev* a = ntk::arena_dev(true);
    return a && slot >= NTK_ARENA_HIDDEN && slot <= NTK_ARENA_GATE ? const_cast<float*>(a->addr[slot]) : nullptr;
}
int ntk_debug_gemv_static_x(void) { return ntk::t_last_static_x; }

size_t ntk_q8l_bytes(int rows, int in_features) { return ntk::q8l_bytes(rows, in_features); }
int ntk_q8l_pack(void* dst, const void* raw, int rows, int in_features, void* stream) {
    if (!dst || !raw) return NTK_E_NULL;
    return ntk::q8l_pack(dst, raw, rows, in_features, false, ntk::resolve_stream(stream));
}
int ntk_q8l_unpack(void* raw, const void* packed, int rows, int in_features, void* stream) {
    if (!raw || !packed) return NTK_E_NULL;
    return ntk::q8l_pack(raw, packed, rows, in_features, true, ntk::resolve_stream(stream));
}

int ntk_gemv(float* y, const void* W, const float* x, int out_features, int in_features, int weight_dtype, void* stream) {
    if (!y || !W || !x) return NTK_E_NULL;
    if (out_features < 0 || in_features <= 0) return NTK_E_SHAPE;
    hipStream_t st = ntk::resolve_stream(stream);
    if (weight_dtype == NTK_DT_F32 || weight_dtype == NTK_DT_F16 || weight_dtype == NTK_DT_BF16)
        return ntk::launch_dense<false>(y, W, x, out_features, in_features, weight_dtype, st);
    if (!ntk::is_quant(weight_dtype)) return NTK_E_DTYPE;
    ntk_gemv_seg seg{W, y, out_features, weight_dtype};
    return ntk::dispatch_quant(weight_dtype, &seg, 1, x, in_features, nullptr, 0.0f, nullptr, 0, st);
}

int ntk_gemv_add(float* y, const void* W, const float* x, int out_features, int in_features, int weight_dtype, void* stream) {
    if (!y || !W || !x) return NTK_E_NULL;
    if (out_features < 0 || in_features <= 0) return NTK_E_SHAPE;
    if (weight_dtype != NTK_DT_F16) return NTK_E_DTYPE;
    return ntk::launch_dense<true>(y, W, x, out_features, in_features, weight_dtype, ntk::resolve_stream(stream));
}


static int gemv_fused_form(const ntk_gemv_seg* segs, int nseg, const float* x, int in_features, const float* norm_w, float eps,
                           const float* resid, int silu_pair, void* stream, int xi_mode) {
    if (!segs || !x) return NTK_E_NULL;
    if (nseg < 1 || nseg > ntk::MAX_SEG) return NTK_E_SHAPE;
    if (segs[0].dtype == NTK_DT_F16 || segs[0].dtype == NTK_DT_BF16) {
        for (int i = 1; i < nseg; ++i)
            if (segs[i].dtype != segs[0].dtype) return NTK_E_DTYPE;
        return ntk::dense16_gemv_fused(segs, nseg, x, in_features, norm_w, eps, resid, silu_pair, ntk::resolve_stream(stream));
    }
    ntk_gemv_seg a[3], b[3];
    int na = 0, nb = 0;
    for (int i = 0; i < nseg; ++i) {
        if (!ntk::is_quant(segs[i].dtype)) return NTK_E_DTYPE;
        if (segs[i].dtype == segs[0].dtype) a[na++] = segs[i];
        else if (nb == 0 || segs[i].dtype == b[0].dtype) b[nb++] = segs[i];
        else return NTK_E_DTYPE;
    }
    hipStream_t st = ntk::resolve_stream(stream);
    if (nb == 0) return ntk::dispatch_quant(segs[0].dtype, segs, nseg, x, in_features, norm_w, eps, resid, silu_pair, st, xi_mode);
    if (resid || silu_pair) return NTK_E_DTYPE;
    const int da = a[0].dtype, db = b[0].dtype;
    if (da == NTK_DT_Q4_K && db == NTK_DT_Q6_K) return ntk::launch_pair<NTK_DT_Q4_K, NTK_DT_Q6_K>(a, na, b, nb, x, in_features, norm_w, eps, st);
    if (da == NTK_DT_Q6_K && db == NTK_DT_Q4_K) return ntk::launch_pair<NTK_DT_Q4_K, NTK_DT_Q6_K>(b, nb, a, na, x, in_features, norm_w, eps, st);
    if (da == NTK_DT_Q4_K && db == NTK_DT_Q5_K) return ntk::launch_pair<NTK_DT_Q4_K, NTK_DT_Q5_K>(a, na, b, nb, x, in_features, norm_w, eps, st);
    if (da == NTK_DT_Q5_K && db == NTK_DT_Q4_K) return ntk::launch_pair<NTK_DT_Q4_K, NTK_DT_Q5_K>(b, nb, a, na, x, in_features, norm_w, eps, st);
    return NTK_E_DTYPE;
}

int ntk_gemv_fused(const ntk_gemv_seg* segs, int nseg, const float* x, int in_features, const float* norm_w, float eps,
                   const float* resid, int silu_pair, void* stream) {
    return gemv_fused_form(segs, nseg, x, in_features, norm_w, eps, resid, silu_pair, stream, ntk::XI_DEFAULT);
}
int ntk_debug_gemv_fused_form(const ntk_gemv_seg* segs, int nseg, const float* x, int in_features, const float* norm_w, float eps,
                              const float* resid, int silu_pair, int integer_activations, void* stream) {
    if (integer_activations < -1 || integer_activations > 1) return NTK_E_SHAPE;
    return gemv_fused_form(segs, nseg, x, in_features, norm_w, eps, resid, silu_pair, stream, integer_activations);
}

}
```

ntransformer_amd/csrc/gemv_core.hip.h:

```cpp
#pragma once
#include "common.hip.h"
#include <algorithm>

namespace ntk {

typedef uint32_t u32x4 __attribute__((ext_vector_type(4)));

constexpr int RB = 4;
constexpr int XPITCH = 68;
constexpr int MAX_SEG = 3;
#ifndef NTK_GEMV_ABLATE
#define NTK_GEMV_ABLATE 0
#endif
constexpr int kAblate = NTK_GEMV_ABLATE;

#ifdef NTK_GEMV_TRACE
constexpr int GT_SLOTS = 64, GT_WG = 512, GT_EV = 14;
__device__ unsigned long long g_gemv_trace[GT_SLOTS][GT_WG][GT_EV];
#define GV_STAMP(ev) do { asm volatile("" ::: "memory"); gv_t[ev] = __builtin_amdgcn_s_memrealtime(); asm volatile("" ::: "memory"); } while (0)
#else
#define GV_STAMP(ev) do {} while (0)
#endif

template <int DT> struct Fmt;
template <> struct Fmt<NTK_DT_Q8_0> { static constexpr int BW = 32, BB = 34, NL = 5, MINW = 4; };
template <> struct Fmt<NTK_DT_Q4_0> { static constexpr int BW = 32, BB = 18, NL = 3, MINW = 4; };
template <> struct Fmt<NTK_DT_Q4_K> { static constexpr int BW = 256, BB = 144, NL = 3, MINW = 4; };
template <> struct Fmt<NTK_DT_Q5_K> { static constexpr int BW = 256, BB = 176, NL = 3, MINW = 4; };
template <> struct Fmt<NTK_DT_Q6_K> { static constexpr int BW = 256, BB = 210, NL = 4, MINW = 4; };

inline bool gemv_slices(int in, int align, int& ns, int& slice_cols) {
    ns = (in + 4095) / 4096;
    slice_cols = ((in + ns - 1) / ns + align - 1) / align * align;
    return ns <= 8 && (long)(ns - 1) * slice_cols < in;
}
inline bool q8l_layout(int in, int& ns, int& slice_cols) {
    if (in <= 0 || in % 256 != 0 || !gemv_slices(in, 64, ns, slice_cols)) return false;
    return slice_cols % 256 == 0 && (in - (ns - 1) * slice_cols) % 256 == 0;
}
template <int DT> constexpr bool A16_OK = (DT == NTK_DT_Q4_K || DT == NTK_DT_Q5_K);

struct GemvSeg {
    const uint8_t* W;
    float* y;
    int rows;
    int delta;
};

struct GemvParams {
    GemvSeg seg[MAX_SEG];
    int nseg;
    int total_rows;
    const float* x;
    int in;
    int ns;
    int rw;
    int slice_cols;
    int nbatch;
    int x_vec;
    const float* norm_w;
    float eps;
    const float* resid;
    int silu_pair;
    unsigned row_bytes;
#ifdef NTK_GEMV_TRACE
    int trace_slot;
#endif
};

template <int DT, bool A16> struct Dot;

typedef float f32x2 __attribute__((ext_vector_type(2)));
__device__ __forceinline__ f32x2 pkfma(f32x2 a, f32x2 b, f32x2 c) { return __builtin_elementwise_fma(a, b, c); }
__device__ __forceinline__ uint32_t opaque(uint32_t v) { asm("" : "+v"(v)); return v; }
__device__ __forceinline__ f32x2 ub01(uint32_t w) { return f32x2{ub2f(w, 0), ub2f(w, 1)}; }
__device__ __forceinline__ f32x2 ub23(uint32_t w) { return f32x2{ub2f(w, 2), ub2f(w, 3)}; }
__device__ __forceinline__ float hsum(f32x2 a, f32x2 b) { return (a.x + a.y) + (b.x + b.y); }


template <bool A16> struct Dot<NTK_DT_Q8_0, A16> {
    __device__ static float run(const uint8_t* st, int shift, int lane, int ncols, const f32x2 (&x2)[32],
                                const float (&)[4], const float (&)[2]) {
        float acc = 0.0f;
        const int o = shift + 68 * lane;
#pragma unroll
        for (int h = 0; h < 2; ++h) {
            if (ncols > 32 * h) {
                const int ob = o + 34 * h;
                const float d = h2f(lds_u16_at(st, ob));
                uint32_t q[8];
                lds_read_dwords<8>(q, st, ob + 2);
                f32x2 a0 = {0.0f, 0.0f}, a1 = {0.0f, 0.0f};
#pragma unroll
                for (int i = 0; i < 8; ++i) {
                    a0 = pkfma(f32x2{sb2f(q[i], 0), sb2f(q[i], 1)}, x2[16 * h + 2 * i], a0);
                    a1 = pkfma(f32x2{sb2f(q[i], 2), sb2f(q[i], 3)}, x2[16 * h + 2 * i + 1], a1);
                }
                acc = fmaf(d, hsum(a0, a1), acc);
            }
        }
        return acc;
    }
};

__device__ __forceinline__ float dot_q8_regs(const u32x4 (&c)[4], const uint32_t sc, const int ncols, const f32x2 (&x2)[32]) {
    float acc = 0.0f;
    if (ncols > 0) {
#pragma unroll
        for (int h = 0; h < 2; ++h) {
            const float d = h2f((uint16_t)(h ? sc >> 16 : sc & 0xFFFFu));
            const uint32_t q[8] = {c[2 * h].x, c[2 * h].y, c[2 * h].z, c[2 * h].w, c[2 * h + 1].x, c[2 * h + 1].y, c[2 * h + 1].z, c[2 * h + 1].w};
            f32x2 a0 = {0.0f, 0.0f}, a1 = {0.0f, 0.0f};
#pragma unroll
            for (int i = 0; i < 8; ++i) {
                a0 = pkfma(f32x2{sb2f(q[i], 0), sb2f(q[i], 1)}, x2[16 * h + 2 * i], a0);
                a1 = pkfma(f32x2{sb2f(q[i], 2), sb2f(q[i], 3)}, x2[16 * h + 2 * i + 1], a1);
            }
            acc = fmaf(d, hsum(a0, a1), acc);
        }
    }
    return acc;
}

template <bool A16> struct Dot<NTK_DT_Q4_0, A16> {
    __device__ static float run(const uint8_t* st, int shift, int lane, int ncols, const f32x2 (&x2)[32],
                                const float (&)[4], const float (&sx32)[2]) {
        float acc = 0.0f;
        const int o = shift + 36 * lane;
#pragma unroll
        for (int h = 0; h < 2; ++h) {
            if (ncols > 32 * h) {
                const int ob = o + 18 * h;
                const float d = h2f(lds_u16_at(st, ob));
                uint32_t q[4];
                lds_read_dwords<4>(q, st, ob + 2);
                f32x2 a0 = {0.0f, 0.0f}, a1 = {0.0f, 0.0f};
#pragma unroll
                for (int i = 0; i < 4; ++i) {
                    const uint32_t lo = opaque(q[i] & 0x0F0F0F0Fu), hi = opaque(q[i] & 0xF0F0F0F0u);
                    a0 = pkfma(ub01(lo), x2[16 * h + 2 * i], a0);
                    a1 = pkfma(ub23(lo), x2[16 * h + 2 * i + 1], a1);
                    a0 = pkfma(ub01(hi), x2[16 * h + 8 + 2 * i], a0);
                    a1 = pkfma(ub23(hi), x2[16 * h + 8 + 2 * i + 1], a1);
                }
                acc = fmaf(d, fmaf(-8.0f, sx32[h], hsum(a0, a1)), acc);
            }
        }
        return acc;
    }
};

template <bool A16>
__device__ __forceinline__ void kq_header(const uint8_t* st, int ob, int c, float& d1, float& m1, float& d2, float& m2) {
    uint32_t hd[4];
    if constexpr (A16) {
        const u32x4 v = *reinterpret_cast<const u32x4*>(st + ob);
        hd[0] = v.x; hd[1] = v.y; hd[2] = v.z; hd[3] = v.w;
    } else {
        lds_read_dwords<4>(hd, st, ob);
    }
    const float d = h2f((uint16_t)(hd[0] & 0xFFFFu)), dmin = h2f((uint16_t)(hd[0] >> 16));
    const uint32_t s0 = hd[1], s1 = hd[2], s2 = hd[3];
    const uint32_t sc_lo = s0 & 0x3F3F3F3Fu, mn_lo = s1 & 0x3F3F3F3Fu;
    const uint32_t sc_hi = (s2 & 0x0F0F0F0Fu) | ((s0 >> 2) & 0x30303030u);
    const uint32_t mn_hi = ((s2 >> 4) & 0x0F0F0F0Fu) | ((s1 >> 2) & 0x30303030u);
    const bool upper = c >= 2;
    const int sh = 16 * (c & 1);
    const uint32_t sc = (upper ? sc_hi : sc_lo) >> sh, mn = (upper ? mn_hi : mn_lo) >> sh;
    d1 = d * ub2f(sc, 0); m1 = dmin * ub2f(mn, 0);
    d2 = d * ub2f(sc, 1); m2 = dmin * ub2f(mn, 1);
}

template <int N, bool A16>
__device__ __forceinline__ void lds_read_q(uint32_t (&dst)[N], const uint8_t* st, int off) {
    if constexpr (A16) {
        static_assert(N % 4 == 0, "b128 reads");
#pragma unroll
        for (int i = 0; i < N / 4; ++i) {
            const u32x4 v = *reinterpret_cast<const u32x4*>(st + off + 16 * i);
            dst[4 * i] = v.x; dst[4 * i + 1] = v.y; dst[4 * i + 2] = v.z; dst[4 * i + 3] = v.w;
        }
    } else {
        lds_read_dwords<N>(dst, st, off);
    }
}

template <bool A16> struct Dot<NTK_DT_Q4_K, A16> {
    __device__ static float run(const uint8_t* st, int shift, int lane, int ncols, const f32x2 (&x2)[32],
                                const float (&)[4], const float (&sx32)[2]) {
        if (ncols <= 0) return 0.0f;
        const int c = lane & 3, ob = shift + 144 * (lane >> 2);
        float d1, m1, d2, m2;
        kq_header<A16>(st, ob, c, d1, m1, d2, m2);
        uint32_t q[8];
        lds_read_q<8, A16>(q, st, ob + 16 + 32 * c);
        f32x2 l0 = {0.0f, 0.0f}, l1 = {0.0f, 0.0f}, h0 = {0.0f, 0.0f}, h1 = {0.0f, 0.0f};
#pragma unroll
        for (int i = 0; i < 8; ++i) {
            const uint32_t lo = opaque(q[i] & 0x0F0F0F0Fu), hi = opaque(q[i] & 0xF0F0F0F0u);
            l0 = pkfma(ub01(lo), x2[2 * i], l0);
            l1 = pkfma(ub23(lo), x2[2 * i + 1], l1);
            h0 = pkfma(ub01(hi), x2[16 + 2 * i], h0);
            h1 = pkfma(ub23(hi), x2[16 + 2 * i + 1], h1);
        }
        float t = d1 * hsum(l0, l1);
        t = fmaf(-m1, sx32[0], t);
        t = fmaf(d2, hsum(h0, h1), t);
        t = fmaf(-m2, sx32[1], t);
        return t;
    }
};

struct XInt {
    uint32_t d[3][16];
    float inv[2];
    float sx[4];
};
template <int DT> struct DotI;

template <> struct DotI<NTK_DT_Q4_K> {
    __device__ static float run(const uint8_t* st, int lane, int ncols, const XInt& xi) {
        if (ncols <= 0) return 0.0f;
        const int c = lane & 3, ob = 144 * (lane >> 2);
        float d1, m1, d2, m2;
        kq_header<true>(st, ob, c, d1, m1, d2, m2);
        uint32_t q[8];
        lds_read_q<8, true>(q, st, ob + 16 + 32 * c);
        uint32_t a0 = 0, a1 = 0, b0 = 0, b1 = 0;
        int a2 = 0, b2 = 0;
#pragma unroll
        for (int i = 0; i < 8; ++i) {
            const uint32_t lo = q[i] & 0x0F0F0F0Fu, hi = (q[i] >> 4) & 0x0F0F0F0Fu;
            a0 = __builtin_amdgcn_udot4(lo, xi.d[0][i], a0, false);
            a1 = __builtin_amdgcn_udot4(lo, xi.d[1][i], a1, false);
            a2 = __builtin_amdgcn_sdot4((int)lo, (int)xi.d[2][i], a2, false);
            b0 = __builtin_amdgcn_udot4(hi, xi.d[0][8 + i], b0, false);
            b1 = __builtin_amdgcn_udot4(hi, xi.d[1][8 + i], b1, false);
            b2 = __builtin_amdgcn_sdot4((int)hi, (int)xi.d[2][8 + i], b2, false);
        }
        const float fa = (float)(int)(a0 + (a1 << 8) + ((uint32_t)a2 << 16)) * xi.inv[0];
        const float fb = (float)(int)(b0 + (b1 << 8) + ((uint32_t)b2 << 16)) * xi.inv[1];
        float t = d1 * fa;
        t = fmaf(-m1, xi.sx[0] + xi.sx[1], t);
        t = fmaf(d2, fb, t);
        t = fmaf(-m2, xi.sx[2] + xi.sx[3], t);
        return t;
    }
};

template <> struct DotI<NTK_DT_Q6_K> {
    __device__ static float run(const uint8_t* st, int shift, int lane, int ncols, const XInt& xi) {
        if (ncols <= 0) return 0.0f;
        const int t = lane & 1, hf = (lane >> 1) & 1, ob = shift + 210 * (lane >> 2);
        uint32_t scd[2];
        lds_read_dwords<2>(scd, st, ob + 192 + 8 * hf);
        const uint32_t sc_lo = scd[0] >> (16 * t), sc_hi = scd[1] >> (16 * t);
        const float d = h2f(lds_u16_at(st, ob + 208));
        float S[4];
#pragma unroll
        for (int is = 0; is < 2; ++is) {
            uint32_t A[4], H[4];
            lds_read_dwords<4>(A, st, ob + 64 * hf + 32 * t + 16 * is);
            lds_read_dwords<4>(H, st, ob + 128 + 32 * hf + 16 * is);
            uint32_t a0 = 0, a1 = 0, b0 = 0, b1 = 0;
            int a2 = 0, b2 = 0;
#pragma unroll
            for (int i = 0; i < 4; ++i) {
                const uint32_t hs = H[i] >> (2 * t);
                const uint32_t qa = (A[i] & 0x0F0F0F0Fu) | ((hs & 0x03030303u) << 4);
                const uint32_t qb = ((A[i] >> 4) & 0x0F0F0F0Fu) | (hs & 0x30303030u);
                a0 = __builtin_amdgcn_udot4(qa, xi.d[0][4 * is + i], a0, false);
                a1 = __builtin_amdgcn_udot4(qa, xi.d[1][4 * is + i], a1, false);
                a2 = __builtin_amdgcn_sdot4((int)qa, (int)xi.d[2][4 * is + i], a2, false);
                b0 = __builtin_amdgcn_udot4(qb, xi.d[0][8 + 4 * is + i], b0, false);
                b1 = __builtin_amdgcn_udot4(qb, xi.d[1][8 + 4 * is + i], b1, false);
                b2 = __builtin_amdgcn_sdot4((int)qb, (int)xi.d[2][8 + 4 * is + i], b2, false);
            }
            S[is] = fmaf(65536.0f, (float)a2, (float)(a0 + (a1 << 8))) * xi.inv[0];
            S[2 + is] = fmaf(65536.0f, (float)b2, (float)(b0 + (b1 << 8))) * xi.inv[1];
        }
        float bs = sb2f(sc_lo, 0) * fmaf(-32.0f, xi.sx[0], S[0]);
        bs = fmaf(sb2f(sc_lo, 1), fmaf(-32.0f, xi.sx[1], S[1]), bs);
        bs = fmaf(sb2f(sc_hi, 0), fmaf(-32.0f, xi.sx[2], S[2]), bs);
        bs = fmaf(sb2f(sc_hi, 1), fmaf(-32.0f, xi.sx[3], S[3]), bs);
        return d * bs;
    }
};

template <bool A16> struct Dot<NTK_DT_Q5_K, A16> {
    __device__ static float run(const uint8_t* st, int shift, int lane, int ncols, const f32x2 (&x2)[32],
                                const float (&)[4], const float (&sx32)[2]) {
        if (ncols <= 0) return 0.0f;
        const int c = lane & 3, ob = shift + 176 * (lane >> 2);
        float d1, m1, d2, m2;
        kq_header<A16>(st, ob, c, d1, m1, d2, m2);
        f32x2 l0 = {0.0f, 0.0f}, l1 = {0.0f, 0.0f}, h0 = {0.0f, 0.0f}, h1 = {0.0f, 0.0f};
#pragma unroll
        for (int hh = 0; hh < 2; ++hh) {
            uint32_t qh[4], ql[4];
            lds_read_q<4, A16>(qh, st, ob + 16 + 16 * hh);
            lds_read_q<4, A16>(ql, st, ob + 48 + 32 * c + 16 * hh);
#pragma unroll
            for (int i = 0; i < 4; ++i) {
                const uint32_t r = __builtin_amdgcn_alignbit(qh[i], qh[i], (uint32_t)((2 * c + 28) & 31));
                const uint32_t lo = opaque((ql[i] & 0x0F0F0F0Fu) | (r & 0x10101010u));
                const uint32_t hi = opaque(((ql[i] >> 4) & 0x0F0F0F0Fu) | ((r >> 1) & 0x10101010u));
                l0 = pkfma(ub01(lo), x2[8 * hh + 2 * i], l0);
                l1 = pkfma(ub23(lo), x2[8 * hh + 2 * i + 1], l1);
                h0 = pkfma(ub01(hi), x2[16 + 8 * hh + 2 * i], h0);
                h1 = pkfma(ub23(hi), x2[16 + 8 * hh + 2 * i + 1], h1);
            }
        }
        float t = d1 * hsum(l0, l1);
        t = fmaf(-m1, sx32[0], t);
        t = fmaf(d2, hsum(h0, h1), t);
        t = fmaf(-m2, sx32[1], t);
        return t;
    }
};

template <bool A16> struct Dot<NTK_DT_Q6_K, A16> {
    __device__ static float run(const uint8_t* st, int shift, int lane, int ncols, const f32x2 (&x2)[32],
                                const float (&sx16)[4], const float (&)[2]) {
        if (ncols <= 0) return 0.0f;
        const int t = lane & 1, hf = (lane >> 1) & 1, ob = shift + 210 * (lane >> 2);
        uint32_t scd[2];
        lds_read_dwords<2>(scd, st, ob + 192 + 8 * hf);
        const uint32_t sc_lo = scd[0] >> (16 * t), sc_hi = scd[1] >> (16 * t);
        const float d = h2f(lds_u16_at(st, ob + 208));
        float S[4];
#pragma unroll
        for (int is = 0; is < 2; ++is) {
            uint32_t A[4], H[4];
            lds_read_dwords<4>(A, st, ob + 64 * hf + 32 * t + 16 * is);
            lds_read_dwords<4>(H, st, ob + 128 + 32 * hf + 16 * is);
            f32x2 a0 = {0.0f, 0.0f}, a1 = {0.0f, 0.0f}, b0 = {0.0f, 0.0f}, b1 = {0.0f, 0.0f};
#pragma unroll
            for (int i = 0; i < 4; ++i) {
                const uint32_t hs = H[i] >> (2 * t);
                const uint32_t qa = opaque((A[i] & 0x0F0F0F0Fu) | ((hs & 0x03030303u) << 4));
                const uint32_t qb = opaque(((A[i] >> 4) & 0x0F0F0F0Fu) | (hs & 0x30303030u));
                a0 = pkfma(ub01(qa), x2[8 * is + 2 * i], a0);
// ... 18 lines not shown
```

ntransformer_amd/csrc/gemv_rp.hip:

```cpp
#include "common.hip.h"
#include <algorithm>
#include <cstdio>
#include <cstdlib>
#include <cstring>

namespace ntk {

typedef int v4i __attribute__((ext_vector_type(4)));
typedef uint32_t u4 __attribute__((ext_vector_type(4)));
typedef uint32_t u2 __attribute__((ext_vector_type(2)));

template <int DT> struct Rp;
template <> struct Rp<NTK_DT_Q4_K> { static constexpr int S1 = 1024, S2 = 320, BB = 144, NSUB = 8; };
template <> struct Rp<NTK_DT_Q5_K> { static constexpr int S1 = 1280, S2 = 320, BB = 176, NSUB = 8; };
template <> struct Rp<NTK_DT_Q6_K> { static constexpr int S1 = 1536, S2 = 288, BB = 210, NSUB = 16; };

static bool rp_supported(int dt) { return dt == NTK_DT_Q4_K || dt == NTK_DT_Q5_K || dt == NTK_DT_Q6_K; }
static size_t rp_s1(int dt) { return dt == NTK_DT_Q4_K ? 1024 : dt == NTK_DT_Q5_K ? 1280 : 1536; }
static size_t rp_s2(int dt) { return dt == NTK_DT_Q6_K ? 288 : 320; }

template <int DT> __device__ __forceinline__ int raw_q(const uint8_t* blk, int cc) {
    if constexpr (DT == NTK_DT_Q4_K || DT == NTK_DT_Q5_K) {
        const int chunk = cc >> 6, l = cc & 31, hi = (cc >> 5) & 1;
        const uint8_t* qs = blk + (DT == NTK_DT_Q4_K ? 16 : 48);
// ... 479 lines not shown
#pragma unroll
                for (int k = 0; k < 4; ++k) {
                    const uint32_t h0 = k < 2 ? (hh[0] << (4 - 2 * k)) : (hh[0] >> (2 * k - 4));
                    const uint32_t h1 = k < 2 ? (hh[1] << (4 - 2 * k)) : (hh[1] >> (2 * k - 4));
                    b0[k] = (int)((h0 & 0x30303030u) | (raw[k] & 0x0F0F0F0Fu));
                    b1[k] = (int)((h1 & 0x30303030u) | ((raw[k] >> 4) & 0x0F0F0F0Fu));
                }
            }
        }
        v4i bc;
        if constexpr (NSUB == 8) bc = v4i{kg == 0 ? (int)it.rec[2] : 0, kg == 0 ? (int)it.rec[3] : 0, 0, 0};
        else bc = v4i{kg == 0 ? (int)it.rec[0] : 0, kg == 0 ? (int)it.rec[1] : 0, kg == 0 ? (int)it.rec[2] : 0, kg == 0 ? (int)it.rec[3] : 0};
        const v4i a0 = *reinterpret_cast<const v4i*>(xa), a1 = *reinterpret_cast<const v4i*>(xa + 64);
        const v4i a2 = *reinterpret_cast<const v4i*>(xa + 128), a3 = *reinterpret_cast<const v4i*>(xa + 192);
        const v4i ac = *reinterpret_cast<const v4i*>(smem + cbase + cstride * (uint32_t)sbk);
        const float inv = invt[sbk];
        const v4i c0 = __builtin_amdgcn_mfma_i32_16x16x64_i8(a0, b[0], z4, 0, 0, 0);
        const v4i c1 = __builtin_amdgcn_mfma_i32_16x16x64_i8(a1, b[1], z4, 0, 0, 0);
        const v4i c2 = __builtin_amdgcn_mfma_i32_16x16x64_i8(a2, b[2], z4, 0, 0, 0);
        const v4i c3 = __builtin_amdgcn_mfma_i32_16x16x64_i8(a3, b[3], z4, 0, 0, 0);
        const v4i cc = __builtin_amdgcn_mfma_i32_16x16x64_i8(ac, bc, z4, 0, 0, 0);
        int s0, s1, s2, s3;
        if constexpr (NSUB == 8) {
            s0 = (int)__builtin_amdgcn_ubfe(it.rec[0], o0, 8u); s1 = (int)__builtin_amdgcn_ubfe(it.rec[0], o1, 8u);
            s2 = (int)__builtin_amdgcn_ubfe(it.rec[1], o0, 8u); s3 = (int)__builtin_amdgcn_ubfe(it.rec[1], o1, 8u);
        } else {
            s0 = __builtin_amdgcn_sbfe((int)it.rec[0], o0, 8u); s1 = __builtin_amdgcn_sbfe((int)it.rec[1], o0, 8u);
            s2 = __builtin_amdgcn_sbfe((int)it.rec[2], o0, 8u); s3 = __builtin_amdgcn_sbfe((int)it.rec[3], o0, 8u);
        }
        const int i0 = __mul24(c0[0], s0) + __mul24(c1[0], s1) + __mul24(c2[0], s2) + __mul24(c3[0], s3);
        const int i1 = __mul24(c0[1], s0) + __mul24(c1[1], s1) + __mul24(c2[1], s2) + __mul24(c3[1], s3);
        const int i2 = __mul24(c0[2], s0) + __mul24(c1[2], s1) + __mul24(c2[2], s2) + __mul24(c3[2], s3);
        const float d = h2f((uint16_t)(it.dd & 0xFFFFu));
        const float S = fmaf(fmaf((float)i2, 256.0f, (float)i1), 256.0f, (float)i0);
        racc = fmaf(S, d * inv, racc);
        const float corr = fmaf(fmaf(fmaf((float)cc[3], 256.0f, (float)cc[2]), 256.0f, (float)cc[1]), 256.0f, (float)cc[0]);
        float fneg;
        if constexpr (NSUB == 8) fneg = -h2f((uint16_t)(it.dd >> 16)) * inv; else fneg = -32.0f * d * inv;
        racc = fmaf(corr, fneg, racc);
    };

    while (p_idx + (2 * RP_DEPTH - 1) * NW < N) {
#pragma unroll
        for (int u = 0; u < RP_DEPTH; ++u) { process(ring[u]); load_item(ring[u]); }
    }
    RP_STAMP(4);
#pragma unroll
    for (int u = 0; u < RP_DEPTH; ++u)
        if (p_idx < N) { process(ring[u]); if (p_idx + (RP_DEPTH - 1) * NW < N) load_item(ring[u]); }
#pragma unroll
    for (int u = 0; u < RP_DEPTH; ++u)
        if (p_idx < N) process(ring[u]);
#ifdef NTK_GEMV_TRACE
    asm volatile("" :: "v"(racc));
#endif
    RP_STAMP(5);
#ifndef NTK_RP_RESID_EPILOGUE
    float res_late = 0.0f;
    {
        const bool res_l = !silu && p.resid != nullptr && sg.wg0 == p.seg[0].wg0;
        const int row_l = (u0 + (tid >> 4)) * 16 + (tid & 15);
        if (res_l && tid < ntl * 16 && row_l < sg.rows) res_late = p.resid[row_l];
    }
#endif
    while (p_tl < ntl) flush();
    __syncthreads();
    RP_STAMP(6);

    auto tile_sum = [&](const int tl, const int r) {
        const float* q = part + (size_t)tl * NW * 64 + r;
        float t = 0.0f;
        int w = 0;
#ifndef NTK_RP_EPILOGUE_ROLLED
        for (; w + 8 <= NW; w += 8) {
            float a[8][4];
#pragma unroll
            for (int k = 0; k < 8; ++k) { a[k][0] = q[(w + k) * 64]; a[k][1] = q[(w + k) * 64 + 16]; a[k][2] = q[(w + k) * 64 + 32]; a[k][3] = q[(w + k) * 64 + 48]; }
#pragma unroll
            for (int k = 0; k < 8; ++k) t += (a[k][0] + a[k][1]) + (a[k][2] + a[k][3]);
        }
#endif
        for (; w < NW; ++w) t += (q[w * 64] + q[w * 64 + 16]) + (q[w * 64 + 32] + q[w * 64 + 48]);
        return t;
    };
    if (silu) {
        for (int e = tid; e < (u1 - u0) * 16; e += (int)blockDim.x) {
            const int pl = e >> 4, r = e & 15, row = (u0 + pl) * 16 + r;
            if (row < sg.rows) {
                const float gv = tile_sum(2 * pl, r), uv = tile_sum(2 * pl + 1, r);
                sg.y[row] = gv / (1.0f + expf(-gv)) * uv;
            }
        }
    } else {
        const bool res = p.resid != nullptr && sg.wg0 == p.seg[0].wg0;
        for (int e = tid; e < ntl * 16; e += (int)blockDim.x) {
            const int tl = e >> 4, r = e & 15, row = (u0 + tl) * 16 + r;
            if (row < sg.rows) {
                float v = tile_sum(tl, r);
#ifndef NTK_RP_RESID_EPILOGUE
                if (res) v = (e == tid ? res_late : p.resid[row]) + v;
#else
                if (res) v = p.resid[row] + v;
#endif
                sg.y[row] = v;
            }
        }
    }
    RP_STAMP(7);
#ifdef NTK_GEMV_TRACE
    if (tid == 0 && bid < RT_WG) {
        rp_t[8] = (unsigned long long)N; rp_t[9] = (unsigned long long)NW;
        for (int e = 0; e < RT_EV; ++e) g_rp_trace[p.trace_slot & (RT_SLOTS - 1)][bid][e] = rp_t[e];
    }
#endif
}

template <int DTA, int DTB, bool NORM>
__global__ __launch_bounds__(1024) void rp_gemv_kernel(const RpParams p) {
    extern __shared__ __attribute__((aligned(16))) uint8_t rp_smem[];
#ifndef NTK_RP_NO_KERNARG_TOUCH
    {
        const auto* ka = __builtin_amdgcn_kernarg_segment_ptr();
        unsigned d0, d1, d2, d3;
        asm volatile("s_load_dword %0, %4, 0x0\n\ts_load_dword %1, %4, 0x40\n\ts_load_dword %2, %4, 0x80\n\ts_load_dword %3, %4, 0xc0\n\t"
                     "s_waitcnt lgkmcnt(0)"
                     : "=&s"(d0), "=&s"(d1), "=&s"(d2), "=&s"(d3) : "s"(ka) : "memory");
        __builtin_amdgcn_sched_barrier(0);
    }
#endif
    if constexpr (DTA == DTB) {
        rp_body<DTA, NORM>(p, 0, p.nseg, rp_smem);
    } else {
        if ((int)blockIdx.x < p.seg[p.nseg_a].wg0) rp_body<DTA, NORM>(p, 0, p.nseg_a, rp_smem);
        else rp_body<DTB, NORM>(p, p.nseg_a, p.nseg, rp_smem);
    }
}

template <int NSUB, bool NORM>
__global__ __launch_bounds__(1024) void rp_prologue_dump_kernel(uint8_t* out, const float* x, const float* norm_w, float eps, int in, int nsb) {
    extern __shared__ __attribute__((aligned(16))) uint8_t rp_smem[];
    const int tid = threadIdx.x, lane = tid & 63, wave = tid >> 6, NW = blockDim.x >> 6;
    float* red = reinterpret_cast<float*>(rp_smem + 4 * (size_t)in + 68 * (size_t)nsb);
    float rms_inv = 1.0f;
    if (NORM) {
        float ssq = 0.0f;
        for (int c = tid; c < in; c += blockDim.x) ssq = fmaf(x[c], x[c], ssq);
        ssq = wave_sum(ssq);
        if (lane == 0) red[wave] = ssq;
        __syncthreads();
        float tot = 0.0f;
        for (int w = 0; w < NW; ++w) tot += red[w];
        rms_inv = 1.0f / sqrtf(tot / (float)in + eps);
    }
    for (int sb = wave; sb < nsb; sb += NW) {
        float4 v = *reinterpret_cast<const float4*>(x + 256 * sb + 4 * lane);
        if (NORM) {
            const float4 w = *reinterpret_cast<const float4*>(norm_w + 256 * sb + 4 * lane);
            v.x = v.x * rms_inv * w.x; v.y = v.y * rms_inv * w.y; v.z = v.z * rms_inv * w.z; v.w = v.w * rms_inv * w.w;
        }
        rp_convert_quad<NSUB>(rp_smem, in, nsb, sb, lane, v.x, v.y, v.z, v.w);
    }
    __syncthreads();
    const size_t n = 4 * (size_t)in + 68 * (size_t)nsb;
    for (size_t k = tid; k < n; k += blockDim.x) out[k] = rp_smem[k];
}

__global__ __launch_bounds__(64) void rp_mfma_probe_kernel(int* D, const int8_t* A, const int8_t* B) {
    const int lane = threadIdx.x, i = lane & 15, kg = lane >> 4;
    v4i a, b;
    int8_t ta[16], tb[16];
    for (int k = 0; k < 16; ++k) { ta[k] = A[i * 64 + 16 * kg + k]; tb[k] = B[(16 * kg + k) * 16 + i]; }
    __builtin_memcpy(&a, ta, 16);
    __builtin_memcpy(&b, tb, 16);
    const v4i z = {0, 0, 0, 0};
    const v4i c = __builtin_amdgcn_mfma_i32_16x16x64_i8(a, b, z, 0, 0, 0);
    for (int r = 0; r < 4; ++r) D[(4 * kg + r) * 16 + i] = c[r];
}

struct RpPlan { int nw, grid; size_t lds; int nwg[3]; };

static bool rp_plan_try(const int* tiles, const int* dts, int nsegw, int mult, int nsb, int in, int nw, int per_cu, RpPlan& out, int* max_cu_units) {
    if ((nsb + nw - 1) / nw > RP_MAXQ || per_cu < 1 || per_cu * nw > 16) return false;
    const int gmax = 256 * per_cu;
    double wsum = 0.0;
    for (int i = 0; i < nsegw; ++i) wsum += (double)tiles[i] * (double)(2 * rp_s1(dts[i]) + rp_s2(dts[i]));
    int grid = 0, max_ntl = 0, kmax = 0;
    for (int i = 0; i < nsegw; ++i) {
        const double wi = (double)tiles[i] * (double)(2 * rp_s1(dts[i]) + rp_s2(dts[i]));
        int gi = std::max(1, (int)(gmax * wi / wsum));
        gi = std::min(gi, tiles[i]);
        const int k = (tiles[i] + gi - 1) / gi;
        gi = (tiles[i] + k - 1) / k;
        out.nwg[i] = gi;
        grid += gi;
        kmax = std::max(kmax, k);
        max_ntl = std::max(max_ntl, k * mult);
    }
    if (grid > gmax) return false;
    const size_t lds = rp_lds_bytes(in, nsb, nw, max_ntl);
    if (lds > 160 * 1024 || (size_t)per_cu * lds > 160 * 1024) return false;
    out.nw = nw; out.grid = grid; out.lds = lds;
    *max_cu_units = kmax * ((grid + 255) / 256);
    return true;
}

static bool rp_plan(const int* tiles, const int* dts, int nseg, int nsb, int in, int silu_pair, int force_nw, int force_per_cu, RpPlan& best) {
    const int mult = silu_pair ? 2 : 1;
    const int nsegw = silu_pair ? 1 : nseg;
    double bytes = 0.0;
    for (int i = 0; i < nsegw; ++i) bytes += (double)tiles[i] * mult * nsb * (double)(2 * rp_s1(dts[i]) + rp_s2(dts[i]));
    int m = 0;
    if (force_nw > 0 || force_per_cu > 0) {
        for (int nw : {16, 14, 12, 10, 8, 7, 6, 5, 4}) for (int pc = 4; pc >= 1; --pc) {
            if ((force_nw > 0 && nw != force_nw) || (force_per_cu > 0 && pc != force_per_cu)) continue;
            if (rp_plan_try(tiles, dts, nsegw, mult, nsb, in, nw, pc, best, &m)) return true;
        }
        return false;
    }
    const int nw = nsb > 32 ? 16 : 8;
    RpPlan one, two;
    int m1 = 0, m2 = 0;
    const bool ok1 = rp_plan_try(tiles, dts, nsegw, mult, nsb, in, nw, 1, one, &m1);
    const bool ok2 = nw == 8 && rp_plan_try(tiles, dts, nsegw, mult, nsb, in, nw, 2, two, &m2);
    if (ok1 && ok2) { best = (m2 <= m1 && one.grid < 240 && bytes >= 48e6) ? two : one; return true; }
    if (ok1) { best = one; return true; }
    if (ok2) { best = two; return true; }
    for (int w : {16, 14, 12, 10, 8, 7, 6, 5, 4}) for (int pc = 1; pc <= 4; ++pc)
        if (rp_plan_try(tiles, dts, nsegw, mult, nsb, in, w, pc, best, &m)) return true;
    return false;
}

static int g_rp_force_nw = 0, g_rp_force_per_cu = 0;
static int g_rp_last_nw = 0, g_rp_last_grid = 0, g_rp_last_lds = 0;

using RpFn = void (*)(const RpParams);
template <int DTA, int DTB> static RpFn rp_fn(bool norm) {
    static const RpFn t[2] = {rp_gemv_kernel<DTA, DTB, false>, rp_gemv_kernel<DTA, DTB, true>};
    static const bool ok = hipFuncSetAttribute((const void*)t[0], hipFuncAttributeMaxDynamicSharedMemorySize, 160 * 1024) == hipSuccess &&
                           hipFuncSetAttribute((const void*)t[1], hipFuncAttributeMaxDynamicSharedMemorySize, 160 * 1024) == hipSuccess;
    return ok ? t[norm ? 1 : 0] : nullptr;
}

}

extern "C" {

size_t ntk_rp_bytes(int dtype, int rows, int in_features) {
    if (!ntk::rp_supported(dtype) || rows <= 0 || in_features <= 0 || in_features % 256 != 0) return 0;
    const size_t tiles = ((size_t)rows + 15) / 16, nsb = (size_t)in_features / 256;
    return tiles * nsb * (2 * ntk::rp_s1(dtype) + ntk::rp_s2(dtype));
}

int ntk_rp_pack(void* dst, const void* raw, int rows, int in_features, int dtype, void* stream) {
    if (!dst || !raw) return NTK_E_NULL;
    if (!ntk::rp_supported(dtype)) return NTK_E_DTYPE;
    if (rows <= 0 || in_features <= 0 || in_features % 256 != 0) return NTK_E_SHAPE;
    if (reinterpret_cast<uintptr_t>(dst) & 15) return NTK_E_ALIGN;
    const int tiles = (rows + 15) / 16, nsb = in_features / 256;
    if ((long)tiles * nsb > 0x7FFFFFFFl) return NTK_E_SHAPE;
    const size_t p2 = (size_t)tiles * nsb * 2 * ntk::rp_s1(dtype);
    hipStream_t st = ntk::resolve_stream(stream);
    const dim3 g((unsigned)(tiles * nsb)), b(128);
    uint8_t* d = static_cast<uint8_t*>(dst);
    const uint8_t* r = static_cast<const uint8_t*>(raw);
    if (dtype == NTK_DT_Q4_K) hipLaunchKernelGGL(ntk::rp_pack_kernel<NTK_DT_Q4_K>, g, b, 0, st, d, r, rows, nsb, p2);
    else if (dtype == NTK_DT_Q5_K) hipLaunchKernelGGL(ntk::rp_pack_kernel<NTK_DT_Q5_K>, g, b, 0, st, d, r, rows, nsb, p2);
    else hipLaunchKernelGGL(ntk::rp_pack_kernel<NTK_DT_Q6_K>, g, b, 0, st, d, r, rows, nsb, p2);
    return ntk::last_launch_status();
}

int ntk_rp_unpack(void* raw, const void* rp, int rows, int in_features, int dtype, void* stream) {
    if (!raw || !rp) return NTK_E_NULL;
    if (!ntk::rp_supported(dtype)) return NTK_E_DTYPE;
    if (rows <= 0 || in_features <= 0 || in_features % 256 != 0) return NTK_E_SHAPE;
    if ((reinterpret_cast<uintptr_t>(rp) & 15) || (reinterpret_cast<uintptr_t>(raw) & (dtype == NTK_DT_Q6_K ? 1 : 3))) return NTK_E_ALIGN;
    const int tiles = (rows + 15) / 16, nsb = in_features / 256;
    if ((long)tiles * nsb > 0x7FFFFFFFl) return NTK_E_SHAPE;
    const size_t p2 = (size_t)tiles * nsb * 2 * ntk::rp_s1(dtype);
    hipStream_t st = ntk::resolve_stream(stream);
    const dim3 g((unsigned)(tiles * nsb)), b(256);
    uint8_t* d = static_cast<uint8_t*>(raw);
    const uint8_t* r = static_cast<const uint8_t*>(rp);
    if (dtype == NTK_DT_Q4_K) hipLaunchKernelGGL(ntk::rp_unpack_kernel<NTK_DT_Q4_K>, g, b, 0, st, d, r, rows, nsb, p2);
    else if (dtype == NTK_DT_Q5_K) hipLaunchKernelGGL(ntk::rp_unpack_kernel<NTK_DT_Q5_K>, g, b, 0, st, d, r, rows, nsb, p2);
    else hipLaunchKernelGGL(ntk::rp_unpack_kernel<NTK_DT_Q6_K>, g, b, 0, st, d, r, rows, nsb, p2);
    return ntk::last_launch_status();
}

int ntk_rp_dequant(float* out, const void* rp, int rows, int in_features, int dtype, void* stream) {
    if (!out || !rp) return NTK_E_NULL;
    if (!ntk::rp_supported(dtype)) return NTK_E_DTYPE;
    if (rows <= 0 || in_features <= 0 || in_features % 256 != 0) return NTK_E_SHAPE;
    const int tiles = (rows + 15) / 16, nsb = in_features / 256;
    const size_t p2 = (size_t)tiles * nsb * 2 * ntk::rp_s1(dtype);
    hipStream_t st = ntk::resolve_stream(stream);
    const dim3 g((unsigned)rows), b(256);
    const uint8_t* r = static_cast<const uint8_t*>(rp);
    if (dtype == NTK_DT_Q4_K) hipLaunchKernelGGL(ntk::rp_dequant_kernel<NTK_DT_Q4_K>, g, b, 0, st, out, r, rows, in_features, nsb, p2);
    else if (dtype == NTK_DT_Q5_K) hipLaunchKernelGGL(ntk::rp_dequant_kernel<NTK_DT_Q5_K>, g, b, 0, st, out, r, rows, in_features, nsb, p2);
    else hipLaunchKernelGGL(ntk::rp_dequant_kernel<NTK_DT_Q6_K>, g, b, 0, st, out, r, rows, in_features, nsb, p2);
    return ntk::last_launch_status();
}

int ntk_gemv_rp_fused(const ntk_gemv_seg* segs, int nseg, const float* x, int in_features, const float* norm_w, float eps,
                      const float* resid, int silu_pair, void* stream) {
    using namespace ntk;
    if (!segs || !x) return NTK_E_NULL;
    if (nseg < 1 || nseg > 3) return NTK_E_SHAPE;
    if (in_features <= 0 || in_features % 256 != 0 || in_features > 32768) return NTK_E_SHAPE;
    if ((reinterpret_cast<uintptr_t>(x) & 15) || (norm_w && (reinterpret_cast<uintptr_t>(norm_w) & 15))) return NTK_E_ALIGN;
    if (silu_pair && (nseg != 2 || segs[0].rows != segs[1].rows || segs[0].dtype != segs[1].dtype || resid)) return NTK_E_SHAPE;
    {
        bool q8 = true;
        for (int i = 0; i < nseg; ++i) q8 = q8 && segs[i].dtype == NTK_DT_Q8_0;
        if (q8) {
            for (int i = 0; i < nseg; ++i) {
                if (segs[i].rows <= 0) return NTK_E_SHAPE;
                if (!segs[i].W || !segs[i].y) return NTK_E_NULL;
            }
            return q8l_gemv_fused(segs, nseg, x, in_features, norm_w, eps, resid, silu_pair, resolve_stream(stream));
        }
    }
    ntk_gemv_seg ord[3];
    int na = 0, nb = 0, dtb = -1;
    for (int i = 0; i < nseg; ++i) {
        if (!rp_supported(segs[i].dtype)) return NTK_E_DTYPE;
        if (segs[i].rows <= 0) return NTK_E_SHAPE;
        if (!segs[i].W || !segs[i].y) return NTK_E_NULL;
        if (reinterpret_cast<uintptr_t>(segs[i].W) & 15) return NTK_E_ALIGN;
    }
    for (int i = 0; i < nseg; ++i) if (segs[i].dtype == segs[0].dtype) ord[na++] = segs[i];
    for (int i = 0; i < nseg; ++i) if (segs[i].dtype != segs[0].dtype) {
        if (dtb < 0) dtb = segs[i].dtype; else if (segs[i].dtype != dtb) return NTK_E_DTYPE;
        ord[na + nb++] = segs[i];
    }
    if (resid && ord[0].W != segs[0].W) return NTK_E_SHAPE;
    const int dta = segs[0].dtype;
    if (dtb < 0) dtb = dta;
    RpParams p;
    memset(&p, 0, sizeof p);
    const int nsb = in_features / 256;
    int tiles[3] = {0, 0, 0}, dts[3] = {0, 0, 0};
    for (int i = 0; i < nseg; ++i) { tiles[i] = (ord[i].rows + 15) / 16; dts[i] = ord[i].dtype; }
    RpPlan plan;
    if (!rp_plan(tiles, dts, nseg, nsb, in_features, silu_pair, g_rp_force_nw, g_rp_force_per_cu, plan)) return NTK_E_SHAPE;
    int wg = 0;
    for (int i = 0; i < nseg; ++i) {
        RpSeg& s = p.seg[i];
        s.rp = static_cast<const uint8_t*>(ord[i].W);
        s.y = ord[i].y;
        s.rows = ord[i].rows;
        s.tiles = tiles[i];
        s.p2_off = (size_t)tiles[i] * nsb * 2 * rp_s1(dts[i]);
        if (s.p2_off + (size_t)tiles[i] * nsb * rp_s2(dts[i]) > 0xFFFFFFF0ull) return NTK_E_SHAPE;
        if (silu_pair && i == 1) { const RpSeg& g0 = p.seg[0]; s.wg0 = g0.wg0; s.nwg = g0.nwg; s.kb = g0.kb; s.krem = g0.krem; continue; }
        s.wg0 = wg; s.nwg = plan.nwg[i];
        s.kb = tiles[i] / s.nwg; s.krem = tiles[i] % s.nwg;
        wg += plan.nwg[i];
    }
    p.nseg = nseg; p.nseg_a = na;
    p.x = x; p.in = in_features; p.nsb = nsb;
    p.norm_w = norm_w; p.eps = eps; p.resid = resid; p.silu_pair = silu_pair;
    RpFn fn = nullptr;
    const bool nm = norm_w != nullptr;
    if (dta == dtb) {
        fn = dta == NTK_DT_Q4_K ? rp_fn<NTK_DT_Q4_K, NTK_DT_Q4_K>(nm) : dta == NTK_DT_Q5_K ? rp_fn<NTK_DT_Q5_K, NTK_DT_Q5_K>(nm) : rp_fn<NTK_DT_Q6_K, NTK_DT_Q6_K>(nm);
    } else if (dta == NTK_DT_Q4_K && dtb == NTK_DT_Q6_K) fn = rp_fn<NTK_DT_Q4_K, NTK_DT_Q6_K>(nm);
    else if (dta == NTK_DT_Q4_K && dtb == NTK_DT_Q5_K) fn = rp_fn<NTK_DT_Q4_K, NTK_DT_Q5_K>(nm);
    else if (dta == NTK_DT_Q6_K && dtb == NTK_DT_Q4_K) fn = rp_fn<NTK_DT_Q6_K, NTK_DT_Q4_K>(nm);
    else if (dta == NTK_DT_Q5_K && dtb == NTK_DT_Q4_K) fn = rp_fn<NTK_DT_Q5_K, NTK_DT_Q4_K>(nm);
    else return NTK_E_DTYPE;
    if (!fn) return NTK_E_LAUNCH;
#ifdef NTK_TUNE
    g_rp_last_nw = plan.nw; g_rp_last_grid = plan.grid; g_rp_last_lds = (int)plan.lds;
#endif
#ifdef NTK_GEMV_TRACE
    static int trace_counter = 0;
    p.trace_slot = trace_counter++;
#endif
    hipLaunchKernelGGL(fn, dim3((unsigned)plan.grid), dim3((unsigned)(64 * plan.nw)), plan.lds, resolve_stream(stream), p);
    return last_launch_status();
}

int ntk_gemv_rp(float* y, const void* rp, const float* x, int out_features, int in_features, int weight_dtype, void* stream) {
    if (!ntk::rp_supported(weight_dtype)) return NTK_E_DTYPE;
    ntk_gemv_seg seg{rp, y, out_features, weight_dtype};
    return ntk_gemv_rp_fused(&seg, 1, x, in_features, nullptr, 0.0f, nullptr, 0, stream);
}

#ifdef NTK_TUNE
NTK_EXTRA_API void ntk_tune_rp_plan(int nw, int per_cu) { ntk::g_rp_force_nw = nw; ntk::g_rp_force_per_cu = per_cu; }
NTK_EXTRA_API void ntk_tune_rp_waves(int nw) { ntk_tune_rp_plan(nw, 0); }
NTK_EXTRA_API void ntk_tune_rp_last_plan(int* out3) { out3[0] = ntk::g_rp_last_nw; out3[1] = ntk::g_rp_last_grid; out3[2] = ntk::g_rp_last_lds; }
#endif

#ifdef NTK_GEMV_TRACE
NTK_EXTRA_API int ntk_debug_rp_trace(unsigned long long* out, size_t n) {
    return hipMemcpyFromSymbol(out, HIP_SYMBOL(ntk::g_rp_trace), n * sizeof(unsigned long long)) == hipSuccess ? 0 : -3;
}
#endif

int ntk_debug_rp_prologue(uint8_t* out, const float* x, const float* norm_w, float eps, int in_features, int nsub, int nwaves, void* stream) {
    if (!out || !x) return NTK_E_NULL;
    if (in_features <= 0 || in_features % 256 != 0 || (nsub != 8 && nsub != 16) || nwaves < 1 || nwaves > 16) return NTK_E_SHAPE;
    const int nsb = in_features / 256;
    const size_t lds = ntk::rp_lds_bytes(in_features, nsb, nwaves, 1);
    if (lds > 160 * 1024) return NTK_E_SHAPE;
    using Fn = void (*)(uint8_t*, const float*, const float*, float, int, int);
    Fn fn = nsub == 8 ? (norm_w ? ntk::rp_prologue_dump_kernel<8, true> : ntk::rp_prologue_dump_kernel<8, false>)
                      : (norm_w ? ntk::rp_prologue_dump_kernel<16, true> : ntk::rp_prologue_dump_kernel<16, false>);
    if (hipFuncSetAttribute((const void*)fn, hipFuncAttributeMaxDynamicSharedMemorySize, 160 * 1024) != hipSuccess) return NTK_E_LAUNCH;
    hipLaunchKernelGGL(fn, dim3(1), dim3((unsigned)(64 * nwaves)), lds, ntk::resolve_stream(stream), out, x, norm_w, eps, in_features, nsb);
    return ntk::last_launch_status();
}

int ntk_debug_mfma_i8_probe(int* D, const int8_t* A, const int8_t* B, void* stream) {
    if (!D || !A || !B) return NTK_E_NULL;
    hipLaunchKernelGGL(ntk::rp_mfma_probe_kernel, dim3(1), dim3(64), 0, ntk::resolve_stream(stream), D, A, B);
    return ntk::last_launch_status();
}

}
```

ntransformer_amd/ops.py:

```python
from __future__ import annotations

import ctypes as C
from typing import Optional, Sequence

import numpy as np

from . import _lib
from ._lib import GemvSeg, check


class DeviceBuffer:

    def __init__(self, nbytes: int):
        self.nbytes = int(nbytes)
        self.ptr = _lib.lib().nt_hip_malloc(max(self.nbytes, 1))
        if not self.ptr:
            raise _lib.NtkError(-7, "hipMalloc(%d)" % nbytes)

    @classmethod
    def from_numpy(cls, a: np.ndarray) -> "DeviceBuffer":
        a = np.ascontiguousarray(a)
        b = cls(a.nbytes)
        if a.nbytes:
            _lib.lib().nt_hip_memcpy_h2d(b.ptr, a.ctypes.data_as(C.c_void_p), a.nbytes)
        return b

    @classmethod
    def zeros(cls, nbytes: int) -> "DeviceBuffer":
        b = cls(nbytes)
        _lib.lib().nt_hip_memset(b.ptr, 0, nbytes)
        return b

    def upload(self, a: np.ndarray, offset: int = 0) -> None:
        a = np.ascontiguousarray(a)
        assert offset + a.nbytes <= self.nbytes
        _lib.lib().nt_hip_memcpy_h2d(self.ptr + offset, a.ctypes.data_as(C.c_void_p), a.nbytes)

    def numpy(self, dtype=np.float32, count: Optional[int] = None, offset: int = 0) -> np.ndarray:
        dt = np.dtype(dtype)
        n = (self.nbytes - offset) // dt.itemsize if count is None else count
        out = np.empty(n, dt)
        check(_lib.lib().ntk_stream_synchronize(None), "stream sync")
        if n:
            _lib.lib().nt_hip_memcpy_d2h(out.ctypes.data_as(C.c_void_p), self.ptr + offset, out.nbytes)
        return out

    def at(self, byte_offset: int) -> int:
        return self.ptr + byte_offset

    def free(self) -> None:
        if self.ptr:
            _lib.lib().nt_hip_free(self.ptr)
            self.ptr = None

    def __del__(self):
        try:
            self.free()
        except Exception:
            pass


def _p(x) -> Optional[int]:
    if x is None:
        return None
    return x.ptr if isinstance(x, DeviceBuffer) else int(x)


def init(device_id: int = 0) -> None:
    check(_lib.lib().ntk_device_init(device_id), "ntk_device_init")


def synchronize(stream=None) -> None:
    check(_lib.lib().ntk_stream_synchronize(stream), "stream sync")


def launch_rmsnorm(output, input, weight, batch_size, hidden_size, eps, stream=None):
    check(_lib.lib().ntk_rmsnorm(_p(output), _p(input), _p(weight), batch_size, hidden_size, eps, stream), "rmsnorm")


def launch_rmsnorm_f16(output, input, weight, batch_size, hidden_size, eps, stream=None):
    check(_lib.lib().ntk_rmsnorm_f16(_p(output), _p(input), _p(weight), batch_size, hidden_size, eps, stream), "rmsnorm_f16")


def launch_rope(q, k, positions, batch_size, seq_len, n_heads, n_kv_heads, head_dim, theta_base, freq_scale,
                interleaved, stream=None):
    check(_lib.lib().ntk_rope(_p(q), _p(k), _p(positions), batch_size, seq_len, n_heads, n_kv_heads, head_dim,
                              theta_base, freq_scale, int(bool(interleaved)), stream), "rope")


def rope_tab(q, k, positions, seq_len, n_heads, n_kv_heads, head_dim, theta_base, freq_scale, interleaved, inv_freq=None, stream=None):
    check(_lib.lib().ntk_rope_tab(_p(q), _p(k), _p(positions), 1, seq_len, n_heads, n_kv_heads, head_dim, theta_base, freq_scale,
                                  int(bool(interleaved)), _p(inv_freq), stream), "rope_tab")


def launch_softmax(output, input, rows, cols, stream=None):
    check(_lib.lib().ntk_softmax(_p(output), _p(input), rows, cols, stream), "softmax")


def launch_masked_softmax(output, input, mask, rows, cols, stream=None):
    check(_lib.lib().ntk_masked_softmax(_p(output), _p(input), _p(mask), rows, cols, stream), "masked_softmax")


def launch_gemv(y, W, x, out_features, in_features, weight_dtype, stream=None):
    check(_lib.lib().ntk_gemv(_p(y), _p(W), _p(x), out_features, in_features, int(weight_dtype), stream), "gemv")


def launch_gemv_add(y, W, x, out_features, in_features, weight_dtype, stream=None):
    check(_lib.lib().ntk_gemv_add(_p(y), _p(W), _p(x), out_features, in_features, int(weight_dtype), stream), "gemv_add")


def launch_gemm_f32(Cm, A, B, M, N, K, stream=None):
    check(_lib.lib().ntk_gemm_f32(_p(Cm), _p(A), _p(B), M, N, K, stream), "gemm_f32")


def launch_silu_mul(output, gate, up, size, stream=None):
    check(_lib.lib().ntk_silu_mul(_p(output), _p(gate), _p(up), size, stream), "silu_mul")


def launch_add_bias(y, bias, size, stream=None):
    check(_lib.lib().ntk_add_bias(_p(y), _p(bias), size, stream), "add_bias")


def launch_attention_decode(output, q, k_cache, v_cache, seq_len, n_heads, n_kv_heads, head_dim, max_seq, scale, stream=None):
    check(_lib.lib().ntk_attention_decode(_p(output), _p(q), _p(k_cache), _p(v_cache), seq_len, n_heads, n_kv_heads,
                                          head_dim, max_seq, scale, stream), "attention_decode")


def launch_attention_prefill(output, Q, k_cache, v_cache, seq_len, start_pos, n_heads, n_kv_heads, head_dim, max_seq,
                             scale, stream=None):
    check(_lib.lib().ntk_attention_prefill(_p(output), _p(Q), _p(k_cache), _p(v_cache), seq_len, start_pos, n_heads,
                                           n_kv_heads, head_dim, max_seq, scale, stream), "attention_prefill")


def launch_copy_to_kv_cache(k_cache, v_cache, k, v, seq_len, n_kv_heads, head_dim, start_pos, max_seq, stream=None):
    check(_lib.lib().ntk_copy_to_kv_cache(_p(k_cache), _p(v_cache), _p(k), _p(v), seq_len, n_kv_heads, head_dim,
                                          start_pos, max_seq, stream), "copy_to_kv_cache")


def launch_add(out, a, b, size, stream=None):
    check(_lib.lib().ntk_add(_p(out), _p(a), _p(b), size, stream), "add")


def launch_add_inplace(a, b, size, stream=None):
    check(_lib.lib().ntk_add_inplace(_p(a), _p(b), size, stream), "add_inplace")


def launch_copy(dst, src, size, stream=None):
    check(_lib.lib().ntk_copy(_p(dst), _p(src), size, stream), "copy")


def launch_cosine_similarity(result, a, b, size, stream=None):
    check(_lib.lib().ntk_cosine_similarity(_p(result), _p(a), _p(b), size, stream), "cosine_similarity")


def gemv_fused(segs: Sequence[tuple], x, in_features, norm_w=None, eps=0.0, resid=None, silu_pair=False, stream=None,
               integer_activations=None):
    arr = (GemvSeg * len(segs))()
    for i, (W, y, rows, dt) in enumerate(segs):
        arr[i].W, arr[i].y, arr[i].rows, arr[i].dtype = _p(W), _p(y), rows, int(dt)
    if integer_activations is None:
        check(_lib.lib().ntk_gemv_fused(arr, len(segs), _p(x), in_features, _p(norm_w), eps, _p(resid), int(silu_pair),
                                        stream), "gemv_fused")
    else:
        check(_lib.lib().ntk_debug_gemv_fused_form(arr, len(segs), _p(x), in_features, _p(norm_w), eps, _p(resid), int(silu_pair),
                                                   1 if integer_activations else 0, stream), "gemv_fused_form")


def qkv_bias(q, k, v, bq, bk, bv, n_rows, q_dim, kv_dim, stream=None):
    check(_lib.lib().ntk_qkv_bias(_p(q), _p(k), _p(v), _p(bq), _p(bk), _p(bv), n_rows, q_dim, kv_dim, stream), "qkv_bias")


def qk_norm(q, k, wq, wk, n_rows, n_heads, n_kv_heads, head_dim, eps, stream=None):
    check(_lib.lib().ntk_qk_norm(_p(q), _p(k), _p(wq), _p(wk), n_rows, n_heads, n_kv_heads, head_dim, eps, stream), "qk_norm")


def q8l_bytes(rows, in_features) -> int:
    return int(_lib.lib().ntk_q8l_bytes(rows, in_features))


def q8l_pack(raw, rows, in_features, stream=None) -> "DeviceBuffer":
    n = q8l_bytes(rows, in_features)
    if n == 0:
        raise _lib.NtkError(-2, "q8l_pack: shape without a lane-major form")
    dst = DeviceBuffer(n + 256)
    check(_lib.lib().ntk_q8l_pack(_p(dst), _p(raw), rows, in_features, stream), "q8l_pack")
    synchronize(stream)
    return dst


def q8l_unpack(packed, rows, in_features, nbytes, stream=None) -> "DeviceBuffer":
    dst = DeviceBuffer(nbytes + 256)
    check(_lib.lib().ntk_q8l_unpack(_p(dst), _p(packed), rows, in_features, stream), "q8l_unpack")
    synchronize(stream)
    return dst


def rp_bytes(dtype, rows, in_features) -> int:
    return int(_lib.lib().ntk_rp_bytes(int(dtype), rows, in_features))


def rp_pack(raw, rows, in_features, dtype, stream=None) -> "DeviceBuffer":
    n = rp_bytes(dtype, rows, in_features)
    if n == 0:
        raise _lib.NtkError(-1, "rp_pack: dtype / shape without a repacked form")
    dst = DeviceBuffer(n + 256)
    check(_lib.lib().ntk_rp_pack(_p(dst), _p(raw), rows, in_features, int(dtype), stream), "rp_pack")
    synchronize(stream)
    return dst


def rp_unpack(rp, rows, in_features, dtype, nbytes, stream=None) -> "DeviceBuffer":
    dst = DeviceBuffer(nbytes + 256)
    check(_lib.lib().ntk_rp_unpack(_p(dst), _p(rp), rows, in_features, int(dtype), stream), "rp_unpack")
    synchronize(stream)
    return dst


def gemv_rp_fused(segs: Sequence[tuple], x, in_features, norm_w=None, eps=0.0, resid=None, silu_pair=False, stream=None):
    arr = (GemvSeg * len(segs))()
    for i, (W, y, rows, dt) in enumerate(segs):
        arr[i].W, arr[i].y, arr[i].rows, arr[i].dtype = _p(W), _p(y), rows, int(dt)
    check(_lib.lib().ntk_gemv_rp_fused(arr, len(segs), _p(x), in_features, _p(norm_w), eps, _p(resid), int(silu_pair),
                                       stream), "gemv_rp_fused")


ARENA_HIDDEN, ARENA_ATTN_OUT, ARENA_GATE = 1, 2, 3


def decode_arena_slot(slot: int) -> int:
    p = _lib.lib().ntk_decode_arena_slot(int(slot))
    if not p:
        raise _lib.NtkError(-1, "ntk_decode_arena_slot(%d)" % slot)
    return int(p)


def upload_to(ptr: int, a: np.ndarray) -> None:
    a = np.ascontiguousarray(a)
    _lib.lib().nt_hip_memcpy_h2d(ptr, a.ctypes.data_as(C.c_void_p), a.nbytes)


def gemv_static_x() -> int:
    return int(_lib.lib().ntk_debug_gemv_static_x())


def _gemm_quant_f16(segs, X, n_tokens, in_features, resid=None, row_max=None, partials=None, stream=None, keep=None, repacked=False, workspace=None,
                    reuse_x=0, full_form=False):
    L = _lib.lib()
    L.ntk_gemm_quant_workspace_bytes.restype = C.c_size_t
    n = int(L.ntk_gemm_quant_workspace_bytes(C.c_int(in_features), C.c_int(sum(r for _, _, r, _ in segs))))
    ws = workspace if workspace is not None else DeviceBuffer(n)
    arr = (GemvSeg * len(segs))()
    for i, (W, y, rows, dt) in enumerate(segs):
        arr[i].W, arr[i].y, arr[i].rows, arr[i].dtype = _p(W), _p(y), rows, int(dt)
    d = _lib.GemmDesc()
    d.segs, d.nseg, d.X, d.n_tokens, d.in_features, d.resid = arr, len(segs), _p(X), n_tokens, in_features, _p(resid)
    d.workspace, d.workspace_bytes, d.reuse_x, d.row_max = ws.ptr, n, int(reuse_x), _p(row_max)
    d.partials = C.pointer(partials) if partials is not None else None
    d.weights_repacked = 1 if repacked else 0
    d.full_form = 1 if full_form else 0
    L.ntk_gemm_quant_f16.argtypes = [C.POINTER(_lib.GemmDesc), C.c_void_p]
    st = L.ntk_gemm_quant_f16(C.byref(d), stream)
    if keep is not None:
        keep.append(ws)
    else:
        synchronize()
    return st


def gemm_quant_f16_prepared(segs, X, n_tokens, in_features, resid=None, row_max=None, stream=None):
    L = _lib.lib()
    L.ntk_gemm_quant_workspace_bytes.restype = C.c_size_t
    n = int(L.ntk_gemm_quant_workspace_bytes(C.c_int(in_features), C.c_int(sum(r for _, _, r, _ in segs))))
    ws = DeviceBuffer(n)
    arr = (GemvSeg * len(segs))()
    for i, (W, y, rows, dt) in enumerate(segs):
        arr[i].W, arr[i].y, arr[i].rows, arr[i].dtype = _p(W), _p(y), rows, int(dt)
    d = _lib.GemmDesc()
    d.segs, d.nseg, d.X, d.n_tokens, d.in_features, d.resid = arr, len(segs), _p(X), n_tokens, in_features, _p(resid)
    d.workspace, d.workspace_bytes, d.reuse_x, d.row_max = ws.ptr, n, 0, _p(row_max)
    L.ntk_gemm_quant_f16.argtypes = [C.POINTER(_lib.GemmDesc), C.c_void_p]

    def call(_keep=(ws, arr, d)):
        return L.ntk_gemm_quant_f16(C.byref(d), stream)
    return call


def gemm_dense16_workspace(in_features, rows, dtype) -> "DeviceBuffer":
    n = int(_lib.lib().ntk_gemm_dense16_workspace_bytes(in_features, rows, int(dtype)))
    if n == 0:
        raise _lib.NtkError(-1, "ntk_gemm_dense16_workspace_bytes: not a 16-bit dtype")
    return DeviceBuffer(n)


def gemm_dense16(segs, X, n_tokens, in_features, resid=None, workspace=None, reuse_x=0, repacked=False, stream=None) -> int:
    ws = workspace if workspace is not None else DeviceBuffer(max(int(_lib.lib().ntk_gemm_dense16_workspace_bytes(in_features, sum(r for _, _, r, _ in segs), int(segs[0][3]))), 256))
    arr = (GemvSeg * len(segs))()
    for i, (W, y, rows, dt) in enumerate(segs):
        arr[i].W, arr[i].y, arr[i].rows, arr[i].dtype = _p(W), _p(y), rows, int(dt)
    d = _lib.GemmDesc()
    d.segs, d.nseg, d.X, d.n_tokens, d.in_features, d.resid = arr, len(segs), _p(X), n_tokens, in_features, _p(resid)
    d.workspace, d.workspace_bytes, d.reuse_x = _p(ws), ws.nbytes if isinstance(ws, DeviceBuffer) else (1 << 40), int(reuse_x)
    d.weights_repacked = 1 if repacked else 0
    st = _lib.lib().ntk_gemm_dense16(C.byref(d), stream)
    synchronize()
    return st


def gemm_quant_ws_multi(segs, X, n_tokens, in_features, stream=None, repacked=False):
    return _gemm_quant_f16(segs, X, n_tokens, in_features, stream=stream, repacked=repacked)


def gemm_quant_ws(Y, W, X, n_tokens, out_features, in_features, dtype, resid=None, stream=None, repacked=False):
    st = _gemm_quant_f16([(W, Y, out_features, dtype)], X, n_tokens, in_features, resid=resid, stream=stream, repacked=repacked)
    synchronize()
    return st


def gemm_quant_ws_rm(Y, W, X, n_tokens, out_features, in_features, dtype, row_max, resid=None, stream=None):
    st = _gemm_quant_f16([(W, Y, out_features, dtype)], X, n_tokens, in_features, resid=resid, row_max=row_max, stream=stream)
    synchronize()
    return st


def gemm_deferred_then_consumer(kind, W, X, n_tokens, rows, in_features, dtype, row_max=None, **kw):
    L = _lib.lib()
    pt = _lib.GemmPartials()
    keep = []
    if kind == "norm":
        y = DeviceBuffer(n_tokens * rows * 4)
        in_place = kw.get("in_place", True)
        check(_gemm_quant_f16([(W, kw["hidden"] if in_place else y, rows, dtype)], X, n_tokens, in_features, resid=kw["hidden"] if in_place else None,
                              row_max=row_max, partials=pt, keep=keep), "gemm deferred")
        L.ntk_reduce_rmsnorm_rowmax.argtypes = [C.c_void_p, C.POINTER(_lib.GemmPartials), C.c_void_p, C.c_float, C.c_void_p, C.c_void_p, C.c_void_p, C.c_void_p]
        check(L.ntk_reduce_rmsnorm_rowmax(_p(kw["hidden"]), C.byref(pt), _p(kw["weight"]), kw["eps"], _p(kw["x_out"]), _p(kw["row_max_out"]), _p(kw.get("zero")), None),
              "reduce_rmsnorm_rowmax")
    else:
        yg, yu = DeviceBuffer(n_tokens * rows * 4), DeviceBuffer(n_tokens * rows * 4)
        check(_gemm_quant_f16([(W[0], yg, rows, dtype), (W[1], yu, rows, dtype)], X, n_tokens, in_features, row_max=row_max, partials=pt, keep=keep),
              "gemm multi deferred")
        L.ntk_reduce_silu_mul_rowmax.argtypes = [C.c_void_p, C.POINTER(_lib.GemmPartials), C.c_void_p, C.c_void_p]
        check(L.ntk_reduce_silu_mul_rowmax(_p(kw["output"]), C.byref(pt), _p(kw["row_max_out"]), None), "reduce_silu_mul_rowmax")
    synchronize()
    return int(pt.nsplit)


def rope_kv_store(q, k, v, positions, seq_len, n_heads, n_kv_heads, head_dim, theta_base, freq_scale, interleaved, k_cache, v_cache, start_pos, max_seq):
    check(_lib.lib().ntk_rope_kv_store(_p(q), _p(k), _p(v), _p(positions), seq_len, n_heads, n_kv_heads, head_dim, theta_base, freq_scale,
                                       int(bool(interleaved)), _p(k_cache), _p(v_cache), start_pos, max_seq, None), "rope_kv_store")


def rope_kv_store_tab(q, k, v, positions, seq_len, n_heads, n_kv_heads, head_dim, theta_base, freq_scale, interleaved, k_cache, v_cache, start_pos, max_seq,
                      inv_freq=None):
    check(_lib.lib().ntk_rope_kv_store_tab(_p(q), _p(k), _p(v), _p(positions), seq_len, n_heads, n_kv_heads, head_dim, theta_base, freq_scale,
                                           int(bool(interleaved)), _p(k_cache), _p(v_cache), start_pos, max_seq, _p(inv_freq), None), "rope_kv_store_tab")


def gemm_workspace(in_features, rows):
    L = _lib.lib()
    L.ntk_gemm_quant_workspace_bytes.restype = C.c_size_t
    return DeviceBuffer(int(L.ntk_gemm_quant_workspace_bytes(C.c_int(in_features), C.c_int(rows))))


def prepare_x(kind, workspace, n_tokens, width, **kw):
    L = _lib.lib()
    vp, i, f = C.c_void_p, C.c_int, C.c_float
    if kind == "x":
        L.ntk_gemm_prepare_x.argtypes = [vp, i, i, vp, vp]
        st = L.ntk_gemm_prepare_x(_p(kw["X"]), n_tokens, width, workspace.ptr, None)
    elif kind == "rmsnorm":
        L.ntk_rmsnorm_prepare_x.argtypes = [vp, vp, vp, i, i, f, vp, vp]
        st = L.ntk_rmsnorm_prepare_x(_p(kw["output"]), _p(kw["input"]), _p(kw["weight"]), n_tokens, width, kw["eps"], workspace.ptr, None)
    elif kind == "silu":
        L.ntk_silu_mul_prepare_x.argtypes = [vp, vp, vp, i, i, vp, vp]
        st = L.ntk_silu_mul_prepare_x(_p(kw["output"]), _p(kw["gate"]), _p(kw["up"]), n_tokens, width, workspace.ptr, None)
    elif kind == "reduce_rmsnorm":
        L.ntk_reduce_rmsnorm_prepare_x.argtypes = [vp, C.POINTER(_lib.GemmPartials), vp, f, vp, vp, vp]
        st = L.ntk_reduce_rmsnorm_prepare_x(_p(kw["hidden"]), C.byref(kw["partials"]), _p(kw["weight"]), kw["eps"], _p(kw["x_out"]), workspace.ptr, None)
    else:
        L.ntk_reduce_silu_mul_prepare_x.argtypes = [vp, C.POINTER(_lib.GemmPartials), vp, vp]
        st = L.ntk_reduce_silu_mul_prepare_x(_p(kw["output"]), C.byref(kw["partials"]), workspace.ptr, None)
    synchronize()
    return st


def launch_rmsnorm_rowmax(output, input, weight, n_tokens, hidden_size, eps, row_max, zero_tokens=None, stream=None):
    check(_lib.lib().ntk_rmsnorm_rowmax(_p(output), _p(input), _p(weight), n_tokens, hidden_size, eps, _p(row_max), _p(zero_tokens), stream), "rmsnorm_rowmax")


def launch_silu_mul_rowmax(output, gate, up, n_tokens, width, row_max, stream=None):
    check(_lib.lib().ntk_silu_mul_rowmax(_p(output), _p(gate), _p(up), n_tokens, width, _p(row_max), stream), "silu_mul_rowmax")


def sample_top_k(logits, n, recent, n_recent, repeat_penalty, temperature, top_k, top_p, r, d_out, stream=None):
    L = _lib.lib()
    L.ntk_sample_scratch_bytes.restype = C.c_size_t
    scratch = DeviceBuffer(int(L.ntk_sample_scratch_bytes(C.c_int(n))))
    L.ntk_sample_top_k.argtypes = [C.c_void_p, C.c_int, C.c_void_p, C.c_int, C.c_float, C.c_float, C.c_int, C.c_float, C.c_float,
                                   C.c_void_p, C.c_void_p, C.c_void_p, C.c_void_p]
    st = L.ntk_sample_top_k(_p(logits), n, _p(recent), n_recent, repeat_penalty, temperature, top_k, top_p, r, _p(d_out), None,
                            _p(scratch), stream)
    synchronize()
    return st


def sample_rows_top_k(logits, n_rows, vocab, ld, recent, recent_ld, rows, d_out, stream=None, null=()):
    L = _lib.lib()
    if not isinstance(rows, _lib.SampleRows):
        sr = _lib.SampleRows()
        for b, (temperature, top_k, top_p, repeat_penalty, r, n_recent) in enumerate(rows):
            sr.temperature[b], sr.top_k[b], sr.top_p[b], sr.repeat_penalty[b], sr.r[b], sr.n_recent[b] = temperature, top_k, top_p, repeat_penalty, r, n_recent
        rows = sr
    scratch = DeviceBuffer(int(L.ntk_sample_rows_scratch_bytes(min(max(n_rows, 1), 16), min(max(vocab, 1), 1 << 20))))
    arg = lambda name, v: None if name in null else v
    st = L.ntk_sample_rows_top_k(arg("logits", _p(logits)), n_rows, vocab, ld, _p(recent), recent_ld, arg("rows", C.pointer(rows)), arg("d_out", _p(d_out)), None,
                                 arg("scratch", _p(scratch)), stream)
    synchronize()
    return st


def gemm_quant(Y, W, X, n_tokens, out_features, in_features, dtype, resid=None, stream=None):
    check(_lib.lib().ntk_gemm_quant(_p(Y), _p(W), _p(X), n_tokens, out_features, in_features, int(dtype), _p(resid),
                                    stream), "gemm_quant")


def attention_decode_fused(output, q, k, v, k_cache, v_cache, d_pos, n_heads, n_kv_heads, head_dim, max_seq, scale,
                           theta_base, freq_scale=1.0, inv_freq=None, stream=None):
    check(_lib.lib().ntk_attention_decode_fused(_p(output), _p(q), _p(k), _p(v), _p(k_cache), _p(v_cache), _p(d_pos),
                                                _p(inv_freq), n_heads, n_kv_heads, head_dim, max_seq, scale, theta_base,
                                                freq_scale, stream), "attention_decode_fused")


def attention_decode_split(output, q, k, v, k_cache, v_cache, d_pos, n_heads, n_kv_heads, head_dim, max_seq, scale,
                           theta_base, nsplit, freq_scale=1.0, inv_freq=None, stream=None):
    scratch = DeviceBuffer(int(_lib.lib().ntk_attention_split_scratch_bytes(n_heads, head_dim, nsplit)))
    check(_lib.lib().ntk_attention_decode_split(_p(output), _p(q), _p(k), _p(v), _p(k_cache), _p(v_cache), _p(d_pos),
                                                _p(inv_freq), n_heads, n_kv_heads, head_dim, max_seq, scale, theta_base,
                                                freq_scale, nsplit, _p(scratch), stream), "attention_decode_split")
    synchronize()
    return None


def attention_decode_split_merged(output, q, k, v, k_cache, v_cache, d_pos, n_heads, n_kv_heads, head_dim, max_seq, scale,
                                  theta_base, nsplit, freq_scale=1.0, inv_freq=None, stream=None, launches=1):
    scratch = DeviceBuffer(int(_lib.lib().ntk_attention_split_scratch_bytes(n_heads, head_dim, nsplit)))
    check(_lib.lib().ntk_attention_split_scratch_init(_p(scratch), n_heads, stream), "attention_split_scratch_init")
    for _ in range(launches):
        check(_lib.lib().ntk_attention_decode_split_merged(_p(output), _p(q), _p(k), _p(v), _p(k_cache), _p(v_cache), _p(d_pos),
                                                           _p(inv_freq), n_heads, n_kv_heads, head_dim, max_seq, scale, theta_base,
                                                           freq_scale, nsplit, _p(scratch), stream), "attention_decode_split_merged")
    synchronize()
    return None


def attention_decode_batch(output, q, k, v, k_caches, v_caches, positions, n_rows, n_heads, n_kv_heads, head_dim, max_seq, scale,
                           theta_base, nsplit=1, freq_scale=1.0, inv_freq=None, stream=None, table=True):
    L = _lib.lib()
    kv = _lib.KvBatch()
    for b, (kc, vc) in enumerate(zip(k_caches, v_caches)):
        kv.k[b], kv.v[b] = _p(kc), _p(vc)
    scratch = DeviceBuffer(max(n_rows, 1) * int(L.ntk_attention_split_scratch_bytes(n_heads, head_dim, nsplit)))
    check(L.ntk_attention_decode_batch(_p(output), _p(q), _p(k), _p(v), C.addressof(kv) if table else None, _p(positions), n_rows, _p(inv_freq),
                                       n_heads, n_kv_heads, head_dim, max_seq, scale, theta_base, freq_scale, nsplit, _p(scratch), stream),
          "attention_decode_batch")
    synchronize()
    return None


def kv_segments(segments, k_caches=None, v_caches=None, n_seg=None, row0=None):
    d = _lib.KvSegments()
    d.n_seg = len(segments) if n_seg is None else n_seg
    row = 0
    for s, (n, start) in enumerate(segments[:16]):
        d.row0[s], d.n_rows[s], d.start_pos[s] = (row if row0 is None else row0[s]), n, start
        row += n
        for side, caches in ((d.k, k_caches), (d.v, v_caches)):
            c = caches[s] if caches is not None else None
            side[s] = c if c is None or isinstance(c, int) else _p(c)
    return d


def kv_segments_validate(desc, total_rows, max_seq) -> int:
    return int(_lib.lib().ntk_kv_segments_validate(C.addressof(desc) if desc is not None else None, int(total_rows), int(max_seq)))


def rope_kv_store_segments(q, k, v, desc, n_heads, n_kv_heads, head_dim, theta_base, max_seq, freq_scale=1.0, interleaved=False, stream=None) -> int:
    return int(_lib.lib().ntk_rope_kv_store_segments(_p(q), _p(k), _p(v), C.addressof(desc) if desc is not None else None, n_heads, n_kv_heads, head_dim,
                                                     theta_base, freq_scale, int(interleaved), max_seq, stream))


def rope_kv_store_segments_tab(q, k, v, desc, n_heads, n_kv_heads, head_dim, theta_base, max_seq, freq_scale=1.0, interleaved=False, inv_freq=None,
                               stream=None) -> int:
    return int(_lib.lib().ntk_rope_kv_store_segments_tab(_p(q), _p(k), _p(v), C.addressof(desc) if desc is not None else None, n_heads, n_kv_heads,
                                                         head_dim, theta_base, freq_scale, int(interleaved), max_seq, _p(inv_freq), stream))


def attention_prefill_segments(output, Q, desc, n_heads, n_kv_heads, head_dim, max_seq, scale, stream=None) -> int:
    return int(_lib.lib().ntk_attention_prefill_segments(_p(output), _p(Q), C.addressof(desc) if desc is not None else None, n_heads, n_kv_heads, head_dim,
                                                         max_seq, scale, stream))


def embed_rows(out, table, tokens, n_tokens, hidden, dtype, stream=None, allow_unsupported=False):
    st = _lib.lib().ntk_embed_rows(_p(out), _p(table), _p(tokens), n_tokens, hidden, int(dtype), stream)
    if not (allow_unsupported and st == -1):
        check(st, "embed_rows")
    return st


def argmax(logits, n, d_out_token, scratch, h_mirror=None, stream=None):
    check(_lib.lib().ntk_argmax(_p(logits), n, _p(d_out_token), _p(h_mirror), _p(scratch), stream), "argmax")


def logprob_rows(logits, n_rows, vocab, ld, targets, logprob, top1=None, stream=None):
    check(_lib.lib().ntk_logprob_rows(_p(logits), n_rows, vocab, ld, _p(targets), _p(logprob), _p(top1), stream), "logprob_rows")


def advance_pos(d_pos, stream=None):
    check(_lib.lib().ntk_advance_pos(_p(d_pos), stream), "advance_pos")


def sclk_mhz(stream=None) -> float:
    import numpy as np
    b = DeviceBuffer.zeros(24)
    check(_lib.lib().ntk_debug_sclk(_p(b), stream), "sclk probe")
    synchronize(stream)
    v = b.numpy(np.uint64)
    return 100.0 * float(v[0]) / max(float(v[1]), 1.0)
# ... 22 lines not shown
```

Baseline: 560.5 tokens/s.

## Add six-wave canonical Q8 lane-major GEMV form chosen by an even-split planner

The GEMV launch planning moves into a shared gemv_plan helper. When eight waves do not divide the row count evenly but six do (for example, a fused QKV projection on a single slice), the planner now picks a six-wave layout. New canonical kernel instantiations (256/384/448 threads) emulate the 512-thread prologue by having each thread load two quads, for x and for the RMSNorm weights, at virtual-thread offsets. The goal is to remove tail imbalance across workgroups and waves. The cost is smaller workgroups, extra kernel variants and more complex prologue code. A debug entry point that forces a given wave count is also exposed.

```diff
diff --git a/include/ntk_engine.h b/include/ntk_engine.h
--- a/include/ntk_engine.h
+++ b/include/ntk_engine.h
@@ -118,6 +118,9 @@
 
 int ntk_debug_gemv_fused_form(const ntk_gemv_seg* segs, int nseg, const float* x, int in_features, const float* norm_w, float eps,
                               const float* resid, int silu_pair, int integer_activations, void* stream);
+
+int ntk_debug_gemv_rp_fused_waves(const ntk_gemv_seg* segs, int nseg, const float* x, int in_features, const float* norm_w, float eps,
+                                  const float* resid, int silu_pair, int waves, void* stream);
 
 size_t   ntk_tp_comm_bytes(size_t max_floats);
 void*    ntk_tp_comm_alloc(size_t bytes);
diff --git a/ntransformer_amd/_lib.py b/ntransformer_amd/_lib.py
--- a/ntransformer_amd/_lib.py
+++ b/ntransformer_amd/_lib.py
@@ -118,6 +118,7 @@
         "ntk_rp_unpack": (i, [vp, vp, i, i, i, vp]),
         "ntk_gemv_rp": (i, [vp, vp, vp, i, i, i, vp]),
         "ntk_gemv_rp_fused": (i, [C.POINTER(GemvSeg), i, vp, i, vp, f, vp, i, vp]),
+        "ntk_debug_gemv_rp_fused_waves": (i, [C.POINTER(GemvSeg), i, vp, i, vp, f, vp, i, i, vp]),
         "ntk_decode_arena_acquire": (i, []), "ntk_decode_arena_release": (None, [i]),
         "ntk_decode_arena_slot": (vp, [i]), "ntk_debug_gemv_static_x": (i, []),
         "ntk_debug_rp_prologue": (i, [vp, vp, vp, f, i, i, i, vp]),
diff --git a/ntransformer_amd/csrc/common.hip.h b/ntransformer_amd/csrc/common.hip.h
--- a/ntransformer_amd/csrc/common.hip.h
+++ b/ntransformer_amd/csrc/common.hip.h
@@ -24,7 +24,7 @@
 hipStream_t resolve_stream(void* s);
 int         last_launch_status();
 int         q8l_gemv_fused(const ntk_gemv_seg* segs, int nseg, const float* x, int in, const float* norm_w, float eps, const float* resid,
-                           int silu_pair, hipStream_t st);
+                           int silu_pair, hipStream_t st, int waves = 0);
 int         dense16_gemv_fused(const ntk_gemv_seg* segs, int nseg, const float* x, int in, const float* norm_w, float eps, const float* resid,
                                int silu_pair, hipStream_t st);
 
diff --git a/ntransformer_amd/csrc/gemv.hip b/ntransformer_amd/csrc/gemv.hip
--- a/ntransformer_amd/csrc/gemv.hip
+++ b/ntransformer_amd/csrc/gemv.hip
@@ -23,12 +23,14 @@
     return XS == XS_HIDDEN ? g_decode_arena.hidden : XS == XS_ATTN ? g_decode_arena.attn_out : g_decode_arena.gate;
 }
 
-template <int DT, bool NORM, bool XFAST, bool A16, bool XI = false, bool LM = false, int NSF = NS_ANY, int XS = XS_NONE>
+template <int DT, bool NORM, bool XFAST, bool A16, bool XI = false, bool LM = false, int NSF = NS_ANY, int XS = XS_NONE, int TC = 0>
 __device__ __forceinline__ void gemv_quant_body(const GemvParams& p, const int bid, const int nblk) {
     using F = Fmt<DT>;
     static_assert(!LM || (DT == NTK_DT_Q8_0 && !A16 && !XI), "lane-major rows: Q8_0");
     static_assert(NSF == NS_ANY || LM, "compile-time slice forms: the lane-major kernels");
     static_assert(XS == XS_NONE || (LM && XFAST && NSF != NS_ANY), "early-x forms: the lane-major kernels, fast prologue");
+    static_assert(TC == 0 || (LM && XFAST && NSF == NS_ONE && TC % 64 == 0 && TC < GV_VTHREADS && 2 * TC >= GV_VTHREADS), "canonical forms: lane-major rows of one slice, 256 .. 448 threads");
+    static_assert(TC == 0 || XS == XS_NONE || XSlot<XS>::IN <= GV_CANON_MAX_IN, "canonical forms: two quads per virtual thread");
     constexpr int NL = LM ? 4 : F::NL;
     constexpr int STAGE = LM ? 0 : NL * 1024 + 64;
     extern __shared__ __attribute__((aligned(16))) uint8_t smem[];
@@ -52,15 +54,29 @@
 #endif
 
     const int tid = threadIdx.x;
-    constexpr int XIT = 8, WIT = 4;
+    constexpr int XIT = GV_XIT, WIT = GV_WIT;
     u32x4 xv[XIT], wv[WIT];
+    constexpr int QV = TC ? 2 : XIT, QW = TC ? 2 : WIT;
+    static_assert(TC == 0 || (2 * QV <= XIT && 2 * QW <= WIT && QV == QW), "register budget of the fast prologue");
+    const bool vt2 = TC && tid + TC < GV_VTHREADS;
+    if constexpr (TC != 0) {
+#pragma unroll
+        for (int i = QV; i < XIT; ++i) xv[i] = u32x4{0u, 0u, 0u, 0u};
+#pragma unroll
+        for (int i = QW; i < WIT; ++i) wv[i] = u32x4{0u, 0u, 0u, 0u};
+    }
     if constexpr (XS != XS_NONE) {
-        constexpr int IN = XSlot<XS>::IN, step0 = 512 * 4;
+        constexpr int IN = XSlot<XS>::IN, step0 = GV_VTHREADS * 4;
         const float* const xs = xslot_ptr<XS>();
 #pragma unroll
-        for (int i = 0; i < XIT; ++i) {
+        for (int i = 0; i < QV; ++i) {
             xv[i] = u32x4{0u, 0u, 0u, 0u};
             if (i * step0 < IN) xv[i] = *reinterpret_cast<const u32x4*>(xs + min(tid * 4 + i * step0, IN - 4));
+        }
+        if constexpr (TC != 0) {
+#pragma unroll
+            for (int i = 0; i < QV; ++i)
+                if (i * step0 < IN && vt2) xv[QV + i] = *reinterpret_cast<const u32x4*>(xs + min((tid + TC) * 4 + i * step0, IN - 4));
         }
         GV_STAMP(7);
         __builtin_amdgcn_sched_barrier(0);
@@ -70,24 +86,39 @@
 #endif
         if constexpr (NORM) {
 #pragma unroll
-            for (int i = 0; i < WIT; ++i) {
+            for (int i = 0; i < QW; ++i) {
                 wv[i] = u32x4{0u, 0u, 0u, 0u};
                 if (i * step0 < IN) wv[i] = *reinterpret_cast<const u32x4*>(p.norm_w + min(tid * 4 + i * step0, IN - 4));
             }
+            if constexpr (TC != 0) {
+#pragma unroll
+                for (int i = 0; i < QW; ++i)
+                    if (i * step0 < IN && vt2) wv[QW + i] = *reinterpret_cast<const u32x4*>(p.norm_w + min((tid + TC) * 4 + i * step0, IN - 4));
+            }
         }
     } else
     if constexpr (XFAST) {
-        const int step0 = (int)blockDim.x * 4;
-#pragma unroll
-        for (int i = 0; i < XIT; ++i) {
+        const int step0 = TC ? GV_VTHREADS * 4 : (int)blockDim.x * 4;
+#pragma unroll
+        for (int i = 0; i < QV; ++i) {
             xv[i] = u32x4{0u, 0u, 0u, 0u};
             if (i * step0 < p.in) xv[i] = *reinterpret_cast<const u32x4*>(p.x + min(tid * 4 + i * step0, p.in - 4));
         }
+        if constexpr (TC != 0) {
+#pragma unroll
+            for (int i = 0; i < QV; ++i)
+                if (i * step0 < p.in && vt2) xv[QV + i] = *reinterpret_cast<const u32x4*>(p.x + min((tid + TC) * 4 + i * step0, p.in - 4));
+        }
         if constexpr (NORM) {
 #pragma unroll
-            for (int i = 0; i < WIT; ++i) {
+            for (int i = 0; i < QW; ++i) {
                 wv[i] = u32x4{0u, 0u, 0u, 0u};
                 if (i * step0 < p.in) wv[i] = *reinterpret_cast<const u32x4*>(p.norm_w + min(tid * 4 + i * step0, p.in - 4));
+            }
+            if constexpr (TC != 0) {
+#pragma unroll
+                for (int i = 0; i < QW; ++i)
+                    if (i * step0 < p.in && vt2) wv[QW + i] = *reinterpret_cast<const u32x4*>(p.norm_w + min((tid + TC) * 4 + i * step0, p.in - 4));
             }
         }
         GV_STAMP(7);
@@ -200,7 +231,7 @@
             const int sp = c / p.slice_cols, cc = c - sp * p.slice_cols;
             return ((sp - g0) * 64 + (cc >> 6)) * XPITCH + (cc & 63);
         };
-        const int step = (int)blockDim.x * 4;
+        const int step = TC ? GV_VTHREADS * 4 : (int)blockDim.x * 4;
         const int dummy = (int)(lds_floats_total - 16);
         const bool have_lo = ncols > 0, have_hi = ncols > 32;
         auto read_own_row = [&](int g0) {
@@ -231,16 +262,30 @@
             if constexpr (NORM) {
                 float ssq = 0.0f;
 #pragma unroll
-                for (int i = 0; i < WIT; ++i) {
+                for (int i = 0; i < QW; ++i) {
                     const float m = (tid * 4 + i * step < p.in) ? 1.0f : 0.0f;
                     const float x0 = __uint_as_float(xv[i].x), x1 = __uint_as_float(xv[i].y), x2_ = __uint_as_float(xv[i].z), x3 = __uint_as_float(xv[i].w);
                     ssq = fmaf(x0 * m, x0, ssq); ssq = fmaf(x1 * m, x1, ssq); ssq = fmaf(x2_ * m, x2_, ssq); ssq = fmaf(x3 * m, x3, ssq);
                 }
                 ssq = wave_sum(ssq);
                 if (lane == 0) red[wave] = ssq;
+                if constexpr (TC != 0) {
+                    if (wave + TC / 64 < GV_VTHREADS / 64) {
+                        float ssq2 = 0.0f;
+#pragma unroll
+                        for (int i = 0; i < QW; ++i) {
+                            const u32x4 q = xv[QV + i];
+                            const float m = ((tid + TC) * 4 + i * step < p.in) ? 1.0f : 0.0f;
+                            const float x0 = __uint_as_float(q.x), x1 = __uint_as_float(q.y), x2_ = __uint_as_float(q.z), x3 = __uint_as_float(q.w);
+                            ssq2 = fmaf(x0 * m, x0, ssq2); ssq2 = fmaf(x1 * m, x1, ssq2); ssq2 = fmaf(x2_ * m, x2_, ssq2); ssq2 = fmaf(x3 * m, x3, ssq2);
+                        }
+                        ssq2 = wave_sum(ssq2);
+                        if (lane == 0) red[wave + TC / 64] = ssq2;
+                    }
+                }
                 __syncthreads();
                 float tot = 0.0f;
-                for (int w = 0; w < nwaves; ++w) tot += red[w];
+                for (int w = 0; w < (TC ? GV_VTHREADS / 64 : nwaves); ++w) tot += red[w];
                 rms_inv = 1.0f / sqrtf(tot / (float)p.in + p.eps);
 #pragma unroll
                 for (int i = 0; i < WIT; ++i) {
@@ -323,6 +368,16 @@
             } else
             {
                 const int cend = min(p.in, GS * p.slice_cols);
+                if constexpr (TC != 0) {
+#pragma unroll
+                    for (int k = 0; k < 2; ++k)
+#pragma unroll
+                    for (int i = 0; i < QV; ++i) {
+                        if (i * step >= cend || (k > 0 && !vt2)) continue;
+                        const int c = (tid + k * TC) * 4 + i * step;
+                        *reinterpret_cast<u32x4*>(ximg + (c < cend ? (c >> 6) * XPITCH + (c & 63) : dummy)) = xv[k * QV + i];
+                    }
+                } else {
                 int isp = 0, icc = tid * 4;
 #pragma unroll
                 for (int i = 0; i < XIT; ++i) {
@@ -331,6 +386,7 @@
                     *reinterpret_cast<u32x4*>(ximg + (c < cend ? (isp * 64 + (icc >> 6)) * XPITCH + (icc & 63) : dummy)) = xv[i];
                     icc += step;
                     if (icc >= p.slice_cols) { icc -= p.slice_cols; ++isp; }
+                }
                 }
                 for (int c = XIT * step + tid * 4; c < cend; c += step)
                     *reinterpret_cast<float4*>(ximg + img_index(c, 0)) = *reinterpret_cast<const float4*>(p.x + c);
@@ -523,6 +579,10 @@
 template <bool NORM, bool XFAST, int NSF, int XS = XS_NONE>
 __global__ __launch_bounds__(512, Fmt<NTK_DT_Q8_0>::MINW) void gemv_q8l_kernel(const GemvParams p) {
     gemv_quant_body<NTK_DT_Q8_0, NORM, XFAST, false, false, true, NSF, XS>(p, (int)blockIdx.x, (int)gridDim.x);
+}
+template <bool NORM, int TC, int XS = XS_NONE>
+__global__ __launch_bounds__(512, Fmt<NTK_DT_Q8_0>::MINW) void gemv_q8l_canon_kernel(const GemvParams p) {
+    gemv_quant_body<NTK_DT_Q8_0, NORM, true, false, false, true, NS_ONE, XS, TC>(p, (int)blockIdx.x, (int)gridDim.x);
 }
 template <bool UNPACK>
 __global__ __launch_bounds__(256) void q8l_pack_kernel(uint8_t* __restrict__ dst, const uint8_t* __restrict__ src, const int rows, const int in,
@@ -630,6 +690,7 @@
     int grid, nwaves;
     size_t lds;
     bool xfast, a16;
+    bool canon;
 };
 
 static bool raise_lds_limit(const void* fn) {
@@ -638,7 +699,7 @@
 
 template <int DT>
 static int prepare_quant(const ntk_gemv_seg* segs, int nseg, const float* x, int in, const float* norm_w, float eps,
-                         const float* resid, int silu_pair, int max_wg, GemvLaunch& L, bool lm = false) {
+                         const float* resid, int silu_pair, int max_wg, GemvLaunch& L, bool lm = false, int waves = 0) {
     using F = Fmt<DT>;
     if (in <= 0 || in % F::BW != 0) return NTK_E_SHAPE;
     GemvParams& p = L.p;
@@ -665,30 +726,27 @@
     p.total_rows = (int)total;
     p.x = x;
     p.in = in;
-    if (!gemv_slices(in, F::BW == 256 ? 256 : 64, p.ns, p.slice_cols)) return NTK_E_SHAPE;
-    static const int env_waves = std::max(1, NTK_TUNE_ENV_INT("NTK_GEMV_WAVES", 8));
-    p.rw = std::max(1, env_waves / p.ns);
-    L.nwaves = p.ns * p.rw;
-    p.x_vec = ((reinterpret_cast<uintptr_t>(x) & 15) == 0 &&
-               (!norm_w || (reinterpret_cast<uintptr_t>(norm_w) & 15) == 0) && (p.slice_cols % 4 == 0)) ? 1 : 0;
+    const bool aligned = (reinterpret_cast<uintptr_t>(x) & 15) == 0 && (!norm_w || (reinterpret_cast<uintptr_t>(norm_w) & 15) == 0);
+    const int mats = silu_pair ? 2 : 1;
+    GemvShape shape{};
+    shape.total_rows = total; shape.mats = mats; shape.in = in;
+    shape.align = F::BW == 256 ? 256 : 64;
+    shape.stage = lm ? 0 : F::NL * 1024 + 64;
+    shape.lm = lm; shape.norm = norm_w != nullptr;
+    shape.x_ok = aligned && !(kAblate & 1);
+    static const int env_waves = std::max(0, NTK_TUNE_ENV_INT("NTK_GEMV_WAVES", 0));
+    const GemvPlan g = gemv_plan(shape, waves > 0 ? waves : env_waves, max_wg, waves > 0);
+    if (g.status != NTK_OK) return g.status;
+    p.ns = g.ns; p.slice_cols = g.slice_cols;
+    p.rw = g.rw;
+    p.nbatch = g.nbatch;
+    L.nwaves = g.nwaves; L.grid = g.grid; L.lds = g.lds; L.xfast = g.xfast; L.canon = g.canon;
+    p.x_vec = (aligned && (p.slice_cols % 4 == 0)) ? 1 : 0;
     p.norm_w = norm_w;
     p.eps = eps;
     p.resid = resid;
     p.silu_pair = silu_pair;
     p.row_bytes = (unsigned)row_bytes;
-    const int mats = silu_pair ? 2 : 1;
-    int grid = (int)std::min<long>((total + p.rw - 1) / p.rw, max_wg);
-    grid = std::max(grid, 1);
-    L.grid = grid;
-    const long ngroups = (long)grid * p.rw;
-    const long rows_per_group = (total + ngroups - 1) / ngroups;
-    p.nbatch = (int)((rows_per_group * mats + RB - 1) / RB);
-    const int STAGE = lm ? 0 : F::NL * 1024 + 64;
-    const size_t image_bytes = (size_t)std::min(p.ns, 4) * 64 * XPITCH * 4;
-    const size_t regionA = p.ns == 1 ? image_bytes + (size_t)L.nwaves * STAGE : std::max((size_t)L.nwaves * STAGE, image_bytes);
-    L.lds = regionA + (size_t)(2 * p.rw * p.ns * RB + 16 + 16) * sizeof(float);
-    L.xfast = p.x_vec && (in % 4 == 0) && in >= 4 && !(kAblate & 1) && (!norm_w || in <= 4 * 4 * 64 * L.nwaves) &&
-              (p.ns == 1 || 4 * 64 * L.nwaves <= p.slice_cols);
     bool a16 = (DT == NTK_DT_Q4_K || DT == NTK_DT_Q5_K);
     for (int i = 0; i < nseg; ++i) a16 = a16 && p.seg[i].delta == 0;
     L.a16 = a16;
@@ -811,14 +869,14 @@
 }
 
 int q8l_gemv_fused(const ntk_gemv_seg* segs, int nseg, const float* x, int in, const float* norm_w, float eps, const float* resid,
-                   int silu_pair, hipStream_t st) {
+                   int silu_pair, hipStream_t st, int waves) {
     int ns, sc;
     t_last_static_x = XS_NONE;
     if (!q8l_layout(in, ns, sc)) return NTK_E_SHAPE;
     for (int i = 0; i < nseg; ++i)
         if (reinterpret_cast<uintptr_t>(segs[i].W) & 15) return NTK_E_ALIGN;
     GemvLaunch L;
-    const int rc = prepare_quant<NTK_DT_Q8_0>(segs, nseg, x, in, norm_w, eps, resid, silu_pair, max_workgroups(), L, true);
+    const int rc = prepare_quant<NTK_DT_Q8_0>(segs, nseg, x, in, norm_w, eps, resid, silu_pair, max_workgroups(), L, true, waves);
     if (rc != NTK_OK) return rc;
     if (L.p.total_rows == 0) return NTK_OK;
     using KernelFn = void (*)(const GemvParams);
@@ -840,10 +898,19 @@
     L.p.trace_slot = trace_counter++;
 #endif
     KernelFn fn = table[norm_w ? 1 : 0][L.xfast ? 1 : 0][L.p.ns == 1 ? 0 : 1];
-    if (L.xfast && L.nwaves == 8) {
+    if (L.canon) {
+#define Q8L_CANON(TC) {gemv_q8l_canon_kernel<false, TC>, gemv_q8l_canon_kernel<true, TC>}
+        static const KernelFn canon[3][2] = {Q8L_CANON(256), Q8L_CANON(384), Q8L_CANON(448)};
+#undef Q8L_CANON
+        static_assert(gv_canon_waves(4) && gv_canon_waves(6) && gv_canon_waves(7) && !gv_canon_waves(5), "one instantiation per wave count of the plan");
+        fn = canon[L.nwaves == 4 ? 0 : L.nwaves == 6 ? 1 : 2][norm_w ? 1 : 0];
+    }
+    if (L.xfast && (L.nwaves == 8 || (L.canon && L.nwaves == 6))) {
         const int xs = static_x_slot(x, in);
         KernelFn early = nullptr;
-        if (xs == XS_HIDDEN && L.p.ns == 1 && norm_w) early = gemv_q8l_kernel<true, true, NS_ONE, XS_HIDDEN>;
+        if (xs == XS_HIDDEN && L.p.ns == 1 && norm_w)
+            early = L.nwaves == 8 ? gemv_q8l_kernel<true, true, NS_ONE, XS_HIDDEN> : gemv_q8l_canon_kernel<true, 384, XS_HIDDEN>;
+        else if (L.nwaves != 8) {}
         else if (xs == XS_ATTN && L.p.ns == 1 && !norm_w) early = gemv_q8l_kernel<false, true, NS_ONE, XS_ATTN>;
         else if (xs == XS_GATE && L.p.ns > 1 && !norm_w) {
             static const bool raised = raise_lds_limit((const void*)gemv_q8l_kernel<false, true, NS_SPLIT, XS_GATE>);
diff --git a/ntransformer_amd/csrc/gemv_core.hip.h b/ntransformer_amd/csrc/gemv_core.hip.h
--- a/ntransformer_amd/csrc/gemv_core.hip.h
+++ b/ntransformer_amd/csrc/gemv_core.hip.h
@@ -1,13 +1,12 @@
 #pragma once
 #include "common.hip.h"
+#include "gemv_plan.h"
 #include <algorithm>
 
 namespace ntk {
 
 typedef uint32_t u32x4 __attribute__((ext_vector_type(4)));
 
-constexpr int RB = 4;
-constexpr int XPITCH = 68;
 constexpr int MAX_SEG = 3;
 #ifndef NTK_GEMV_ABLATE
 #define NTK_GEMV_ABLATE 0
@@ -29,15 +28,6 @@
 template <> struct Fmt<NTK_DT_Q5_K> { static constexpr int BW = 256, BB = 176, NL = 3, MINW = 4; };
 template <> struct Fmt<NTK_DT_Q6_K> { static constexpr int BW = 256, BB = 210, NL = 4, MINW = 4; };
 
-inline bool gemv_slices(int in, int align, int& ns, int& slice_cols) {
-    ns = (in + 4095) / 4096;
-    slice_cols = ((in + ns - 1) / ns + align - 1) / align * align;
-    return ns <= 8 && (long)(ns - 1) * slice_cols < in;
-}
-inline bool q8l_layout(int in, int& ns, int& slice_cols) {
-    if (in <= 0 || in % 256 != 0 || !gemv_slices(in, 64, ns, slice_cols)) return false;
-    return slice_cols % 256 == 0 && (in - (ns - 1) * slice_cols) % 256 == 0;
-}
 template <int DT> constexpr bool A16_OK = (DT == NTK_DT_Q4_K || DT == NTK_DT_Q5_K);
 
 struct GemvSeg {
diff --git a/ntransformer_amd/csrc/gemv_plan.h b/ntransformer_amd/csrc/gemv_plan.h
--- /dev/null
+++ b/ntransformer_amd/csrc/gemv_plan.h
@@ -0,0 +1,82 @@
+#pragma once
+#include <stddef.h>
+#include <stdint.h>
+#include <algorithm>
+#include "../../include/ntk.h"
+
+namespace ntk {
+
+constexpr int RB = 4;
+constexpr int XPITCH = 68;
+constexpr int GV_WAVES = 8;
+constexpr int GV_MAX_WG = 512;
+constexpr int GV_XIT = 8, GV_WIT = 4, GV_VTHREADS = 512;
+constexpr int GV_CANON_MAX_IN = GV_VTHREADS * 4 * (GV_WIT / 2);
+constexpr int GV_CANON_MIN_WAVES = GV_VTHREADS / 2 / 64;
+
+inline bool gemv_slices(int in, int align, int& ns, int& slice_cols) {
+    ns = (in + 4095) / 4096;
+    slice_cols = ((in + ns - 1) / ns + align - 1) / align * align;
+    return ns <= 8 && (long)(ns - 1) * slice_cols < in;
+}
+inline bool q8l_layout(int in, int& ns, int& slice_cols) {
+    if (in <= 0 || in % 256 != 0 || !gemv_slices(in, 64, ns, slice_cols)) return false;
+    return slice_cols % 256 == 0 && (in - (ns - 1) * slice_cols) % 256 == 0;
+}
+
+struct GemvShape {
+    long total_rows;
+    int mats;
+    int in;
+    int align;
+    int stage;
+    bool lm;
+    bool norm;
+    bool x_ok;
+};
+struct GemvPlan {
+    int status;
+    int ns, slice_cols;
+    int rw, nwaves;
+    int grid, ngroups;
+    int rows_per_group;
+    int nbatch;
+    bool xfast;
+    bool canon;
+    size_t lds;
+};
+
+inline long gv_groups(long total_rows, int waves, int cap) { return std::max(1L, std::min<long>((total_rows + waves - 1) / waves, cap)); }
+inline bool gv_even(long total_rows, int waves, int cap) { return total_rows % (waves * gv_groups(total_rows, waves, cap)) == 0; }
+
+constexpr bool gv_canon_waves(int nwaves) { return nwaves == 4 || nwaves == 6 || nwaves == 7; }
+inline bool gv_canon_ok(const GemvShape& s, int ns, int nwaves) {
+    return s.lm && ns == 1 && s.in <= GV_CANON_MAX_IN && nwaves >= GV_CANON_MIN_WAVES && gv_canon_waves(nwaves);
+}
+
+inline GemvPlan gemv_plan(const GemvShape& s, int waves, int cap, bool strict = false) {
+    GemvPlan p{};
+    p.status = NTK_E_SHAPE;
+    if (s.in <= 0 || s.total_rows < 0 || cap < 1 || waves < 0 || !gemv_slices(s.in, s.align, p.ns, p.slice_cols)) return p;
+    const bool vec = s.x_ok && (p.slice_cols % 4 == 0) && (s.in % 4 == 0) && s.in >= 4;
+    int want = waves > 0 ? waves : GV_WAVES;
+    if (waves == 0 && vec && gv_canon_ok(s, p.ns, 6) && gv_even(s.total_rows, 6, cap) && !gv_even(s.total_rows, GV_WAVES, cap)) want = 6;
+    p.rw = std::max(1, want / p.ns);
+    p.nwaves = p.ns * p.rw;
+    if (p.nwaves > 8) return p;
+    p.canon = vec && gv_canon_ok(s, p.ns, p.nwaves);
+    if (strict && waves > 0 && waves != GV_WAVES && !p.canon) return p;
+    p.grid = (int)std::max(1L, std::min<long>((s.total_rows + p.rw - 1) / p.rw, cap));
+    p.ngroups = p.grid * p.rw;
+    p.rows_per_group = (int)((s.total_rows + p.ngroups - 1) / p.ngroups);
+    p.nbatch = (int)(((long)p.rows_per_group * s.mats + RB - 1) / RB);
+    const size_t image_bytes = (size_t)std::min(p.ns, 4) * 64 * XPITCH * 4;
+    const size_t regionA = p.ns == 1 ? image_bytes + (size_t)p.nwaves * s.stage : std::max((size_t)p.nwaves * s.stage, image_bytes);
+    p.lds = regionA + (size_t)(2 * p.rw * p.ns * RB + 16 + 16) * sizeof(float);
+    p.xfast = vec && (p.canon || ((!s.norm || s.in <= GV_WIT * 4 * 64 * p.nwaves) &&
+                                  (p.ns == 1 || 4 * 64 * p.nwaves <= p.slice_cols)));
+    p.status = NTK_OK;
+    return p;
+}
+
+}
diff --git a/ntransformer_amd/csrc/gemv_rp.hip b/ntransformer_amd/csrc/gemv_rp.hip
--- a/ntransformer_amd/csrc/gemv_rp.hip
+++ b/ntransformer_amd/csrc/gemv_rp.hip
@@ -805,8 +805,8 @@
     return ntk::last_launch_status();
 }
 
-int ntk_gemv_rp_fused(const ntk_gemv_seg* segs, int nseg, const float* x, int in_features, const float* norm_w, float eps,
-                      const float* resid, int silu_pair, void* stream) {
+static int gemv_rp_fused_waves(const ntk_gemv_seg* segs, int nseg, const float* x, int in_features, const float* norm_w, float eps,
+                               const float* resid, int silu_pair, int waves, void* stream) {
     using namespace ntk;
     if (!segs || !x) return NTK_E_NULL;
     if (nseg < 1 || nseg > 3) return NTK_E_SHAPE;
@@ -821,9 +821,10 @@
                 if (segs[i].rows <= 0) return NTK_E_SHAPE;
                 if (!segs[i].W || !segs[i].y) return NTK_E_NULL;
             }
-            return q8l_gemv_fused(segs, nseg, x, in_features, norm_w, eps, resid, silu_pair, resolve_stream(stream));
-        }
-    }
+            return q8l_gemv_fused(segs, nseg, x, in_features, norm_w, eps, resid, silu_pair, resolve_stream(stream), waves);
+        }
+    }
+    if (waves != 0) return NTK_E_SHAPE;
     ntk_gemv_seg ord[3];
     int na = 0, nb = 0, dtb = -1;
     for (int i = 0; i < nseg; ++i) {
@@ -885,6 +886,16 @@
     return last_launch_status();
 }
 
+int ntk_gemv_rp_fused(const ntk_gemv_seg* segs, int nseg, const float* x, int in_features, const float* norm_w, float eps,
+                      const float* resid, int silu_pair, void* stream) {
+    return gemv_rp_fused_waves(segs, nseg, x, in_features, norm_w, eps, resid, silu_pair, 0, stream);
+}
+int ntk_debug_gemv_rp_fused_waves(const ntk_gemv_seg* segs, int nseg, const float* x, int in_features, const float* norm_w, float eps,
+                                  const float* resid, int silu_pair, int waves, void* stream) {
+    if (waves != 0 && waves != 4 && waves != 6 && waves != 7 && waves != 8) return NTK_E_SHAPE;
+    return gemv_rp_fused_waves(segs, nseg, x, in_features, norm_w, eps, resid, silu_pair, waves, stream);
+}
+
 int ntk_gemv_rp(float* y, const void* rp, const float* x, int out_features, int in_features, int weight_dtype, void* stream) {
     if (!ntk::rp_supported(weight_dtype)) return NTK_E_DTYPE;
     ntk_gemv_seg seg{rp, y, out_features, weight_dtype};
diff --git a/ntransformer_amd/ops.py b/ntransformer_amd/ops.py
--- a/ntransformer_amd/ops.py
+++ b/ntransformer_amd/ops.py
@@ -216,12 +216,16 @@
     return dst
 
 
-def gemv_rp_fused(segs: Sequence[tuple], x, in_features, norm_w=None, eps=0.0, resid=None, silu_pair=False, stream=None):
+def gemv_rp_fused(segs: Sequence[tuple], x, in_features, norm_w=None, eps=0.0, resid=None, silu_pair=False, stream=None, waves=None):
     arr = (GemvSeg * len(segs))()
     for i, (W, y, rows, dt) in enumerate(segs):
         arr[i].W, arr[i].y, arr[i].rows, arr[i].dtype = _p(W), _p(y), rows, int(dt)
-    check(_lib.lib().ntk_gemv_rp_fused(arr, len(segs), _p(x), in_features, _p(norm_w), eps, _p(resid), int(silu_pair),
-                                       stream), "gemv_rp_fused")
+    if waves is None:
+        check(_lib.lib().ntk_gemv_rp_fused(arr, len(segs), _p(x), in_features, _p(norm_w), eps, _p(resid), int(silu_pair),
+                                           stream), "gemv_rp_fused")
+    else:
+        check(_lib.lib().ntk_debug_gemv_rp_fused_waves(arr, len(segs), _p(x), in_features, _p(norm_w), eps, _p(resid), int(silu_pair),
+                                                       int(waves), stream), "gemv_rp_fused_waves")
 
 
 ARENA_HIDDEN, ARENA_ATTN_OUT, ARENA_GATE = 1, 2, 3
```

After: 564.7 tokens/s, median of 6. Within noise of the previous version (+0.8%).
